# nv-tlabs/ChronoEdit

Measured on AMD Instinct MI355X. Metric: denoising-steps/sec, higher is better.
Workload: dtype bf16

## Files before the change

chronoedit_amd/csrc/ce_attn.hip:

```cpp
#include <cstdlib>

#include "ce_common.h"

namespace {

constexpr int HD = 128;
constexpr int QW = 32;
constexpr int KVB = 64;
constexpr int K_TILE_BYTES = KVB * HD * 2;
constexpr int VT_TILE_BYTES = HD * KVB * 2;
constexpr int BUF_BYTES = K_TILE_BYTES + VT_TILE_BYTES;
constexpr int OST_ROW = HD * 2 + 16;
constexpr int smem_bytes(int nwave, bool two_seg) {
  const int stage = nwave * QW * OST_ROW;
  return two_seg ? 2 * BUF_BYTES + stage : (stage > 2 * BUF_BYTES ? stage : 2 * BUF_BYTES);
}
constexpr float NEG_BIG = -1.0e30f;

__device__ __forceinline__ int vt_swz(int dv) {
  return ((((dv >> 2) & 7) << 1) | (((dv >> 1) ^ (dv >> 5)) & 1)) ^ (((dv >> 6) & 1) << 1);
}

struct KVSeg {
  const bf16* k;
  const bf16* v;
  int len;
  int ldk;
  int ldv;
};
struct BlkRows {
  int rows;
  int stride;
  uint32_t magic;
  int vt_cols;
  unsigned char* q8;
  unsigned char* s8;
  int ld8;
};

template <bool TWO_SEG, int NWAVE>
__global__ __launch_bounds__(NWAVE * 64, NWAVE == 8 ? 2 : 2) void attn_fwd_kernel(const bf16* __restrict__ Q, bf16* __restrict__ O, KVSeg seg0,
                                                       KVSeg seg1, int Nq, int H, int ldq, int ldo, int nqb,
                                                       float scale_log2e) {
  extern __shared__ __attribute__((aligned(16))) unsigned char smem[];
  {
    const size_t bz = blockIdx.y;
    Q += bz * Nq * ldq;
    O += bz * Nq * ldo;
    seg0.k += bz * seg0.len * seg0.ldk;
    seg0.v += bz * seg0.len * seg0.ldv;
    if (TWO_SEG) {
      seg1.k += bz * seg1.len * seg1.ldk;
      seg1.v += bz * seg1.len * seg1.ldv;
    }
  }
  const int tid = threadIdx.x, lane = tid & 63, wave = tid >> 6;
  const int l31 = lane & 31, hh = lane >> 5;

  int head, qb;
  if ((H & 7) == 0) {
    const int xcd = blockIdx.x & 7, local = blockIdx.x >> 3;
    head = xcd + 8 * (local / nqb);
    qb = local % nqb;
  } else {
    head = blockIdx.x / nqb;
    qb = blockIdx.x % nqb;
  }
  constexpr int QB = QW * NWAVE;
  constexpr int NT = NWAVE * 64;
  const int q0 = qb * QB + wave * QW;
  const int hoff = head * HD;

  bf16x8 qf[8];
  {
    const bf16* qrow = Q + (size_t)min(q0 + l31, Nq - 1) * ldq + hoff + 8 * hh;
#pragma unroll
    for (int ks = 0; ks < 8; ++ks) qf[ks] = *reinterpret_cast<const bf16x8*>(qrow + 16 * ks);
  }

  constexpr int KREP = 1024 / NT, KROWS = NT / 16;
  const int k_ck = tid & 15, k_row0 = tid >> 4;
  constexpr int VREP = 512 / NT, VKQ = NT / 32;
  const int v_dvq = tid & 31, v_kvq = tid >> 5;

  unsigned char* ost = smem + (TWO_SEG ? 2 * BUF_BYTES : 0) + (size_t)(wave * QW + l31) * OST_ROW;

#pragma unroll
  for (int sidx = 0; sidx < (TWO_SEG ? 2 : 1); ++sidx) {
    const KVSeg sg = sidx == 0 ? seg0 : seg1;
    const int ntiles = (sg.len + KVB - 1) / KVB;

    f32x16 oacc[4];
// ... 135 lines not shown
    const float l_tot = l_run + __shfl_xor(l_run, 32, 64);
    const float inv = 1.0f / l_tot;
#pragma unroll
    for (int m = 0; m < 4; ++m)
#pragma unroll
      for (int a = 0; a < 4; ++a) {
        uint32_t w0 = pack_bf16(oacc[m][4 * a + 0] * inv, oacc[m][4 * a + 1] * inv);
        uint32_t w1 = pack_bf16(oacc[m][4 * a + 2] * inv, oacc[m][4 * a + 3] * inv);
        u32x2* slot = reinterpret_cast<u32x2*>(ost + (32 * m + 8 * a + 4 * hh) * 2);
        if (TWO_SEG && sidx == 1) {
          const u32x2 pv = *slot;
          w0 = pack_bf16(bf16lo(pv[0]) + bf16lo(w0), bf16hi(pv[0]) + bf16hi(w0));
          w1 = pack_bf16(bf16lo(pv[1]) + bf16lo(w1), bf16hi(pv[1]) + bf16hi(w1));
        }
        u32x2 val = {w0, w1};
        *slot = val;
      }
  }

  __syncthreads();
#pragma unroll
  for (int i = 0; i < 8; ++i) {
    const int c = lane + 64 * i;
    const int rl = c >> 4, cc = c & 15;
    const int q = q0 + rl;
    if (q < Nq) {
      const u32x4 v = *reinterpret_cast<const u32x4*>(smem + (TWO_SEG ? 2 * BUF_BYTES : 0) + (size_t)(wave * QW + rl) * OST_ROW + cc * 16);
      *reinterpret_cast<u32x4*>(O + (size_t)q * ldo + hoff + cc * 8) = v;
    }
  }
}


#define CE_EPOCH_BARRIER()                          \
  asm volatile("s_waitcnt lgkmcnt(0)" ::: "memory"); \
  __builtin_amdgcn_s_barrier()
constexpr int PK_ROW = HD * 2 + 16;
constexpr int PV_ROW = KVB * 2 + 16;
constexpr int PK_TILE = KVB * PK_ROW;
constexpr int PV_TILE = HD * PV_ROW;
typedef __attribute__((ext_vector_type(4))) unsigned pp_u4;
typedef __attribute__((ext_vector_type(2))) unsigned pp_u2;

constexpr int K_GRP = 1088;
typedef __attribute__((address_space(3))) void lds_void;
#ifdef CE_DIAGNOSTICS
__device__ unsigned long long g_sp_exact_hits = 0ull;
#endif
constexpr float SP_SPEC_THR = 1024.0f;
constexpr int SP_V0 = 2 * PK_TILE;
constexpr int SP_TILE_BYTES = 2 * PK_TILE + 3 * PV_TILE;
constexpr int sp_smem_bytes(bool two_seg) { return two_seg ? SP_TILE_BYTES + 8 * QW * OST_ROW : SP_TILE_BYTES; }

template <bool TWO_SEG, bool VT = false, bool QOUT = false>
__global__ __launch_bounds__(512, 2) void attn_fwd_sp_kernel(const bf16* __restrict__ Q_, bf16* __restrict__ O_, KVSeg seg0_,
                                                              KVSeg seg1_, int Nq, int H, int ldq, int ldo, int nqb,
                                                              float scale_log2e, int batch, BlkRows blk) {
  extern __shared__ __attribute__((aligned(16))) unsigned char smem[];
  constexpr int NWAVE = 8, QB = QW * NWAVE;
  const int tid = threadIdx.x, lane = tid & 63;
  const int wave = __builtin_amdgcn_readfirstlane(tid >> 6);
  const int l31 = lane & 31, hh = lane >> 5;
  for (int item = blockIdx.x; item < nqb * H * batch; item += gridDim.x) {
  const bf16* Q = Q_;
  bf16* O = O_;
  KVSeg seg0 = seg0_, seg1 = seg1_;

  int head, qb, bz;
  {
    const int nqb_full = Nq / QB;
    if ((H & 7) == 0) {
      const int xcd = item & 7, local = item >> 3, hx_n = H >> 3;
      const int full = batch * hx_n * nqb_full;
      if (local < full) {
        bz = local / (hx_n * nqb_full);
        const int r = local % (hx_n * nqb_full);
        head = xcd + 8 * (r / nqb_full);
        qb = r % nqb_full;
      } else {
        const int l2 = local - full;
        bz = l2 / hx_n;
        head = xcd + 8 * (l2 % hx_n);
        qb = nqb_full;
      }
    } else {
      bz = item / (nqb * H);
      const int r = item % (nqb * H);
      head = r / nqb;
      qb = r % nqb;
    }
  }
  {
    if (VT && blk.rows > 0) {
      Q += (size_t)bz * blk.rows * ldq;
      O += (size_t)bz * blk.rows * ldo;
      seg0.k += (size_t)bz * blk.rows * seg0.ldk;
      seg0.v += (size_t)bz * blk.vt_cols;
    } else {
      Q += (size_t)bz * Nq * ldq;
      O += (size_t)bz * Nq * ldo;
      seg0.k += (size_t)bz * seg0.len * seg0.ldk;
      seg0.v += VT ? (size_t)bz * (TWO_SEG ? blk.vt_cols : seg0.len) : (size_t)bz * seg0.len * seg0.ldv;
    }
    if (TWO_SEG) {
      seg1.k += (size_t)bz * seg1.len * seg1.ldk;
      seg1.v += VT ? (size_t)bz * blk.stride : (size_t)bz * seg1.len * seg1.ldv;
    }
  }
  const int q0 = qb * QB + wave * QW;
  const int hoff = head * HD;
  const bool active = q0 < Nq;
  const int q0row = (VT && blk.rows > 0) ? (q0 / blk.rows) * blk.stride + q0 % blk.rows : q0;

  bf16x8 qf[8];
  {
    const bf16* qrow = Q + (size_t)(q0 + l31 < Nq ? q0row + l31 : 0) * ldq + hoff + 8 * hh;
#pragma unroll
    for (int ks = 0; ks < 8; ++ks) qf[ks] = *reinterpret_cast<const bf16x8*>(qrow + 16 * ks);
  }
  auto scale_q = [&]() __attribute__((always_inline)) {
#pragma unroll
  for (int ks = 0; ks < 8; ++ks) {
    const u32x4 w = __builtin_bit_cast(u32x4, qf[ks]);
    u32x4 o;
#pragma unroll
    for (int i = 0; i < 4; ++i) o[i] = pack_bf16(bf16lo(w[i]) * scale_log2e, bf16hi(w[i]) * scale_log2e);
    qf[ks] = __builtin_bit_cast(bf16x8, o);
  }
#pragma unroll
  for (int ks = 0; ks < 8; ++ks) asm volatile("" : "+v"(qf[ks]));

  };
  const int v_dvq = (tid & 1) | (((tid >> 4) & 15) << 1), v_kvq = ((tid >> 1) & 7) | (((tid >> 8) & 1) << 3);
  const int v_chunk = (v_kvq & ~3) | ((v_kvq & 1) << 1) | ((v_kvq >> 1) & 1);
  unsigned char* ost = smem + (TWO_SEG ? SP_TILE_BYTES : 0) + (size_t)(wave * QW + l31) * OST_ROW;
  const int k_w = l31 & 3;
  const unsigned char* k_rd = smem + (l31 >> 2) * K_GRP + k_w * 256 + ((hh ^ (k_w & 1)) << 4);
  const int k_eo[2] = {(k_w >> 1) << 5, ((k_w >> 1) ^ 1) << 5};
  const unsigned char* v_rd = smem + SP_V0 + l31 * PV_ROW + hh * 16;
  int vt_off[4];
#pragma unroll
  for (int s4 = 0; s4 < 4; ++s4) {
    const int x = (l31 >> 1) & 7;
    vt_off[s4] = l31 * 128 + ((2 * (s4 ^ (x >> 1)) + (hh ^ (x & 1))) << 4);
  }
  unsigned char* v_wr = smem + SP_V0 + (4 * v_dvq) * PV_ROW + v_chunk * 8;

#pragma unroll
  for (int sidx = 0; sidx < (TWO_SEG ? 2 : 1); ++sidx) {
    const KVSeg sg = sidx == 0 ? seg0 : seg1;
    const int ntiles = (sg.len + KVB - 1) / KVB;
    const int k_rows_span = (VT && blk.rows > 0) ? ((sg.len - 1) / blk.rows) * blk.stride + blk.rows : sg.len;
    const auto k_rsrc = __builtin_amdgcn_make_buffer_rsrc((void*)(sg.k + hoff), 0, (k_rows_span - 1) * sg.ldk * 2 + HD * 2, 0x00020000);
    const auto v_rsrc = VT ? __builtin_amdgcn_make_buffer_rsrc((void*)(sg.v + (size_t)hoff * sg.ldv), 0, ((HD - 1) * sg.ldv + ntiles * KVB) * 2, 0x00020000)
                           : __builtin_amdgcn_make_buffer_rsrc((void*)(sg.v + hoff), 0, (sg.len - 1) * sg.ldv * 2 + HD * 2, 0x00020000);
    int v_voff[4];
#pragma unroll
    for (int i = 0; i < 4; ++i) v_voff[i] = (4 * v_kvq + i) * sg.ldv * 2 + v_dvq * 8;
    const int k_tile_bytes = KVB * sg.ldk * 2, v_tile_bytes = KVB * sg.ldv * 2;

    f32x16 oacc[4];
#pragma unroll
    for (int m = 0; m < 4; ++m)
#pragma unroll
      for (int r = 0; r < 16; ++r) oacc[m][r] = 0.f;
    float l_run = 0.f, alpha_prev = 1.0f, mc = 0.f;
    f32x16 cinit;
#pragma unroll
    for (int r = 0; r < 16; ++r) cinit[r] = 0.f;
    u32x4 ppk[4];
#pragma unroll
    for (int s4 = 0; s4 < 4; ++s4) ppk[s4] = u32x4{0u, 0u, 0u, 0u};

// ... 822 lines not shown
    if (col < col_end) *reinterpret_cast<pp_u4*>(VT + (size_t)(head * HD + d) * ldvt + col) = v;
  }
}

}

#ifdef CE_DIAGNOSTICS
extern "C" int ce_diag_mx_exact_hits(unsigned long long* out, int reset);
CE_API int ce_diag_attention_exact_route_hits(unsigned long long* hits, int reset) {
  if (!hits) return CE_ERR_ARG;
  unsigned long long v = 0ull, z = 0ull;
  if (hipDeviceSynchronize() != hipSuccess) return CE_ERR_ARG;
  if (hipMemcpyFromSymbol(&v, HIP_SYMBOL(g_sp_exact_hits), sizeof(v)) != hipSuccess) return CE_ERR_ARG;
  if (reset && hipMemcpyToSymbol(HIP_SYMBOL(g_sp_exact_hits), &z, sizeof(z)) != hipSuccess) return CE_ERR_ARG;
  hits[0] = v;
  return ce_diag_mx_exact_hits(hits + 1, reset);
}
#endif
CE_KNOB g_attn_nwave = 0;
#ifdef CE_DIAGNOSTICS
CE_API int ce_set_attention_waves(int nwave) {
  const int old = g_attn_nwave;
  if (nwave == 0 || nwave == 4 || nwave == 8 || nwave == 16 || nwave == 64 || nwave == 128 || nwave == 129) g_attn_nwave = nwave;
  return old;
}
#endif

CE_API int ce_attention_batched_bf16(const void* Q, const void* K1, const void* V1, int len1, int ldk1, int ldv1,
                                         const void* K2, const void* V2, int len2, int ldk2, int ldv2, void* O, int Nq, int H,
                                         int head_dim, int ldq, int ldo, float softmax_scale, int batch, hipStream_t stream) {
  if (!Q || !K1 || !V1 || !O) return CE_ERR_ARG;
  if (head_dim != HD || Nq <= 0 || H <= 0 || len1 <= 0 || batch <= 0 || batch > 65535) return CE_ERR_SHAPE;
  if ((ldq & 7) || (ldo & 7) || (ldk1 & 7) || (ldv1 & 3)) return CE_ERR_ALIGN;
  const bool two = (K2 != nullptr && V2 != nullptr && len2 > 0);
  if (two && ((ldk2 & 7) || (ldv2 & 3))) return CE_ERR_ALIGN;
  KVSeg s0{(const bf16*)K1, (const bf16*)V1, len1, ldk1, ldv1};
  KVSeg s1{(const bf16*)K2, (const bf16*)V2, two ? len2 : 0, ldk2, ldv2};
  const float sl2 = softmax_scale * 1.4426950408889634f;
  const bool sp = g_attn_nwave == 64 || g_attn_nwave == 0 || g_attn_nwave >= 128;
  const int nwave = sp ? 8 : g_attn_nwave;
  const int nqb = (Nq + nwave * QW - 1) / (nwave * QW);
  dim3 grid(nqb * H, batch), block(nwave * 64);
  if (sp) {
#define CE_ATTN_SP(TWO)                                                                                              \
  do {                                                                                                               \
    static bool done_[CE_MAX_DEVICES] = {};                                                                          \
    bool& done = done_[ce_device_slot()];                                                                            \
    if (!done) {                                                                                                     \
      (void)hipFuncSetAttribute((const void*)attn_fwd_sp_kernel<TWO>, hipFuncAttributeMaxDynamicSharedMemorySize,    \
                                sp_smem_bytes(TWO));                                                                 \
      done = true;                                                                                                   \
    }                                                                                                                \
    hipLaunchKernelGGL((attn_fwd_sp_kernel<TWO>), dim3(nqb * H * batch), block, sp_smem_bytes(TWO), stream, (const bf16*)Q, \
                       (bf16*)O, s0, s1, Nq, H, ldq, ldo, nqb, sl2, batch, BlkRows{0, 0, 0u, 0});                    \
  } while (0)
    if (two) CE_ATTN_SP(true); else CE_ATTN_SP(false);
#undef CE_ATTN_SP
    return (int)hipGetLastError();
  }
#define CE_ATTN_LAUNCH(TWO, NW)                                                                                     \
  do {                                                                                                              \
    static bool done_[CE_MAX_DEVICES] = {};                                                                         \
    bool& done = done_[ce_device_slot()];                                                                           \
    if (!done) {                                                                                                    \
      (void)hipFuncSetAttribute((const void*)attn_fwd_kernel<TWO, NW>, hipFuncAttributeMaxDynamicSharedMemorySize,  \
                                smem_bytes(NW, TWO));                                                               \
      done = true;                                                                                                  \
    }                                                                                                               \
    hipLaunchKernelGGL((attn_fwd_kernel<TWO, NW>), grid, block, smem_bytes(NW, TWO), stream, (const bf16*)Q, (bf16*)O, \
                       s0, s1, Nq, H, ldq, ldo, nqb, sl2);                                                          \
  } while (0)
  if (two) {
    if (nwave == 8) CE_ATTN_LAUNCH(true, 8); else CE_ATTN_LAUNCH(true, 4);
  } else {
    if (nwave == 8) CE_ATTN_LAUNCH(false, 8); else CE_ATTN_LAUNCH(false, 4);
  }
#undef CE_ATTN_LAUNCH
  return (int)hipGetLastError();
}

CE_API int ce_attention_bf16(const void* Q, const void* K1, const void* V1, int len1, int ldk1, int ldv1, const void* K2,
                                 const void* V2, int len2, int ldk2, int ldv2, void* O, int Nq, int H, int head_dim, int ldq,
                                 int ldo, float softmax_scale, hipStream_t stream) {
  return ce_attention_batched_bf16(Q, K1, V1, len1, ldk1, ldv1, K2, V2, len2, ldk2, ldv2, O, Nq, H, head_dim, ldq, ldo,
                                   softmax_scale, 1, stream);
}

CE_API int ce_v_transpose_bf16(const void* v, int ldv, void* vt, int ldvt, int n_keys, int H, hipStream_t stream) {
  if (!v || !vt) return CE_ERR_ARG;
  if (n_keys <= 0 || H <= 0 || ldvt < n_keys) return CE_ERR_SHAPE;
  if ((ldv & 3) || (ldvt & 7)) return CE_ERR_ALIGN;
  hipLaunchKernelGGL(v_transpose_kernel, dim3((ldvt + KVB - 1) / KVB, H), dim3(256), 0, stream, (const bf16*)v, ldv, (bf16*)vt, ldvt, n_keys, 0, 0, 0);
  return (int)hipGetLastError();
}

CE_API int ce_v_transpose_blocked_bf16(const void* v, int ldv, void* vt, int ldvt, int n_keys, int H, int batch, int blk_rows, int blk_stride,
                                           int vt_sample_cols, hipStream_t stream) {
  if (!v || !vt) return CE_ERR_ARG;
  if (n_keys <= 0 || H <= 0 || batch <= 0 || blk_rows <= 0 || (blk_rows & 63) || blk_stride < batch * blk_rows || (vt_sample_cols & 63) ||
      vt_sample_cols < (n_keys + KVB - 1) / KVB * KVB || ldvt < batch * vt_sample_cols)
    return CE_ERR_SHAPE;
  if ((ldv & 3) || (ldvt & 7)) return CE_ERR_ALIGN;
  hipLaunchKernelGGL(v_transpose_kernel, dim3(vt_sample_cols / KVB, H, batch), dim3(256), 0, stream, (const bf16*)v, ldv, (bf16*)vt, ldvt, n_keys,
                     blk_rows, blk_stride, vt_sample_cols);
  return (int)hipGetLastError();
}

#ifdef CE_DIAGNOSTICS
extern "C" int ce_attn16_launch(const void* Q, const void* K, const void* Vt, int len, int ldk, int ldvt, void* O, int Nq, int H, int ldq, int ldo,
                                float sl2, int batch, int cus, hipStream_t stream);
#endif

static int attention_vt_launch(const void* Q, const void* K, const void* Vt, int len, int ldk, int ldvt, void* O, int Nq, int H, int head_dim,
                               int ldq, int ldo, float softmax_scale, int batch, int blk_rows, int blk_stride, int vt_sample_cols,
                               hipStream_t stream) {
  if (!Q || !K || !Vt || !O) return CE_ERR_ARG;
  if (head_dim != HD || Nq <= 0 || H <= 0 || len <= 0 || batch <= 0 || batch > 65535) return CE_ERR_SHAPE;
  const int ntiles_cols = (len + KVB - 1) / KVB * KVB;
  if (blk_rows == 0) {
    vt_sample_cols = len;
    if (ldvt < (batch - 1) * len + ntiles_cols) return CE_ERR_SHAPE;
  } else {
    if ((blk_rows & 63) || blk_stride < batch * blk_rows || (Nq % blk_rows) || vt_sample_cols < ntiles_cols ||
        ldvt < (batch - 1) * vt_sample_cols + ntiles_cols)
      return CE_ERR_SHAPE;
  }
  if ((ldq & 7) || (ldo & 7) || (ldk & 7) || (ldvt & 7) || (batch > 1 && (vt_sample_cols & 1))) return CE_ERR_ALIGN;
  KVSeg s0{(const bf16*)K, (const bf16*)Vt, len, ldk, ldvt};
  KVSeg s1{nullptr, nullptr, 0, 0, 0};
  BlkRows blk{blk_rows, blk_stride, 0u, vt_sample_cols};
  if (blk_rows > 0) {
    const uint32_t tps = (uint32_t)(blk_rows >> 6);
    blk.magic = tps == 1 ? 0u : (uint32_t)(((1ull << 32) + tps - 1) / tps);
  }
  const float sl2 = softmax_scale * 1.4426950408889634f;
  const int nqb = (Nq + 8 * QW - 1) / (8 * QW);
  static bool done_[CE_MAX_DEVICES] = {};
  bool& done = done_[ce_device_slot()];
  if (!done) {
    (void)hipFuncSetAttribute((const void*)attn_fwd_sp_kernel<false, true>, hipFuncAttributeMaxDynamicSharedMemorySize, sp_smem_bytes(false));
    done = true;
  }
  const int cus = ce_device_cus();
  const int items = nqb * H * batch;
#ifdef CE_DIAGNOSTICS
  if (g_attn_nwave == 16 && blk_rows == 0) {
    const int rc = ce_attn16_launch(Q, K, Vt, len, ldk, ldvt, O, Nq, H, ldq, ldo, sl2, batch, cus, stream);
    if (rc != CE_ERR_ALIGN) return rc;
  }
#endif
  if (g_attn_nwave == 128 || g_attn_nwave == 129) {
    static bool done4_[CE_MAX_DEVICES] = {};
    bool& done4 = done4_[ce_device_slot()];
    if (!done4) {
      (void)hipFuncSetAttribute((const void*)attn_fwd_w4_kernel, hipFuncAttributeMaxDynamicSharedMemorySize, W4_SMEM);
      done4 = true;
    }
    const int grid4 = (g_attn_nwave == 129 && items > cus) ? (cus & ~7) : items;
    hipLaunchKernelGGL(attn_fwd_w4_kernel, dim3(grid4), dim3(256), W4_SMEM, stream, (const bf16*)Q, (bf16*)O, s0, Nq, H, ldq, ldo, nqb,
                       sl2, batch, blk);
    return (int)hipGetLastError();
  }
  const int grid_vt = items <= 2 * cus ? items : ((2 * cus) & ~7);
  hipLaunchKernelGGL((attn_fwd_sp_kernel<false, true>), dim3(grid_vt), dim3(512), sp_smem_bytes(false), stream, (const bf16*)Q, (bf16*)O,
                     s0, s1, Nq, H, ldq, ldo, nqb, sl2, batch, blk);
  return (int)hipGetLastError();
}

CE_API int ce_attention_vt_bf16(const void* Q, const void* K, const void* Vt, int len, int ldk, int ldvt, void* O, int Nq, int H,
                                    int head_dim, int ldq, int ldo, float softmax_scale, int batch, hipStream_t stream) {
  return attention_vt_launch(Q, K, Vt, len, ldk, ldvt, O, Nq, H, head_dim, ldq, ldo, softmax_scale, batch, 0, 0, 0, stream);
}

CE_API int ce_attention_vt_blocked_bf16(const void* Q, const void* K, const void* Vt, int len, int ldk, int ldvt, void* O, int Nq, int H,
                                            int head_dim, int ldq, int ldo, float softmax_scale, int batch, int blk_rows, int blk_stride,
                                            int vt_sample_cols, hipStream_t stream) {
  if (blk_rows <= 0) return CE_ERR_SHAPE;
  return attention_vt_launch(Q, K, Vt, len, ldk, ldvt, O, Nq, H, head_dim, ldq, ldo, softmax_scale, batch, blk_rows, blk_stride, vt_sample_cols,
                             stream);
}


static int attention_2seg_vt_launch(const void* Q, const void* K1, const void* V1t, int len1, int ldk1, int ldv1t, int vt_cols1,
                                    const void* K2, const void* V2t, int len2, int ldk2, int ldv2t, int vt_cols2, void* O, int Nq,
                                    int H, int head_dim, int ldq, int ldo, float softmax_scale, int batch, void* O8, void* S8, int ldo8,
                                    hipStream_t stream) {
  if (!Q || !K1 || !V1t || !K2 || !V2t || (!O && !O8)) return CE_ERR_ARG;
  if (head_dim != HD || Nq <= 0 || H <= 0 || len1 <= 0 || len2 <= 0 || batch <= 0 || batch > 65535) return CE_ERR_SHAPE;
  const int c1 = (len1 + KVB - 1) / KVB * KVB, c2 = (len2 + KVB - 1) / KVB * KVB;
  if (vt_cols1 < len1 || vt_cols2 < len2 || ldv1t < (batch - 1) * vt_cols1 + c1 || ldv2t < (batch - 1) * vt_cols2 + c2) return CE_ERR_SHAPE;
  if ((ldq & 7) || (ldo & 7) || (ldk1 & 7) || (ldk2 & 7) || (ldv1t & 7) || (ldv2t & 7) || (vt_cols1 & 1) || (vt_cols2 & 1)) return CE_ERR_ALIGN;
  KVSeg s0{(const bf16*)K1, (const bf16*)V1t, len1, ldk1, ldv1t};
  KVSeg s1{(const bf16*)K2, (const bf16*)V2t, len2, ldk2, ldv2t};
  const float sl2 = softmax_scale * 1.4426950408889634f;
  const int nqb = (Nq + 8 * QW - 1) / (8 * QW);
  static bool done_[CE_MAX_DEVICES] = {};
  bool& done = done_[ce_device_slot()];
  if (!done) {
    (void)hipFuncSetAttribute((const void*)attn_fwd_sp_kernel<true, true>, hipFuncAttributeMaxDynamicSharedMemorySize, sp_smem_bytes(true));
    (void)hipFuncSetAttribute((const void*)attn_fwd_sp_kernel<true, true, true>, hipFuncAttributeMaxDynamicSharedMemorySize, sp_smem_bytes(true));
    done = true;
  }
  const BlkRows blk{0, vt_cols2, 0u, vt_cols1, (unsigned char*)O8, (unsigned char*)S8, ldo8};
  const int cus = ce_device_cus();
  const int items = nqb * H * batch;
  const int grid = items <= 2 * cus ? items : ((2 * cus) & ~7);
  if (O8)
    hipLaunchKernelGGL((attn_fwd_sp_kernel<true, true, true>), dim3(grid), dim3(512), sp_smem_bytes(true), stream, (const bf16*)Q,
                       (bf16*)O, s0, s1, Nq, H, ldq, ldo, nqb, sl2, batch, blk);
  else
    hipLaunchKernelGGL((attn_fwd_sp_kernel<true, true>), dim3(grid), dim3(512), sp_smem_bytes(true), stream, (const bf16*)Q, (bf16*)O,
                       s0, s1, Nq, H, ldq, ldo, nqb, sl2, batch, blk);
  return (int)hipGetLastError();
}

CE_API int ce_attention_2seg_vt_bf16(const void* Q, const void* K1, const void* V1t, int len1, int ldk1, int ldv1t, int vt_cols1,
                                         const void* K2, const void* V2t, int len2, int ldk2, int ldv2t, int vt_cols2, void* O, int Nq,
                                         int H, int head_dim, int ldq, int ldo, float softmax_scale, int batch, hipStream_t stream) {
  if (!O) return CE_ERR_ARG;
  return attention_2seg_vt_launch(Q, K1, V1t, len1, ldk1, ldv1t, vt_cols1, K2, V2t, len2, ldk2, ldv2t, vt_cols2, O, Nq, H, head_dim, ldq, ldo,
                                  softmax_scale, batch, nullptr, nullptr, 0, stream);
}

CE_API int ce_attention_2seg_vt_quant_bf16(const void* Q, const void* K1, const void* V1t, int len1, int ldk1, int ldv1t, int vt_cols1,
                                               const void* K2, const void* V2t, int len2, int ldk2, int ldv2t, int vt_cols2, void* o8,
                                               void* scale8, int Nq, int H, int head_dim, int ldq, int ldo8, float softmax_scale, int batch,
                                               hipStream_t stream) {
  if (!o8 || !scale8 || (ldo8 & 15) || ((H * head_dim) & 127)) return CE_ERR_ARG;
  return attention_2seg_vt_launch(Q, K1, V1t, len1, ldk1, ldv1t, vt_cols1, K2, V2t, len2, ldk2, ldv2t, vt_cols2, nullptr, Nq, H, head_dim, ldq,
                                  8, softmax_scale, batch, o8, scale8, ldo8, stream);
}
```

chronoedit_amd/csrc/ce_gemm.hip:

```cpp
#include <cmath>

#include "ce_common.h"

#define EPI_BIAS 0
#define EPI_BIAS_GELU 1
#define EPI_GATE_RES 2
#define EPI_BIAS_GELU_ERF 3
#define EPI_F32 4
#define EPI_BIAS_ROW 6
#define EPI_BIAS_T 7
#define EPI_MUL 5

namespace {

constexpr int BM = 128, BN = 128, BK = 64;
constexpr int TILE_BYTES = BM * BK * 2;
constexpr int LDC_BYTES = BN * 2 + 16;

__device__ __forceinline__ int swz_chunk(int row, int chunk) { return chunk ^ ((row >> 1) & 7); }

template <int EPI>
__global__ __launch_bounds__(256) void gemm_bf16_128(const bf16* __restrict__ A, const bf16* __restrict__ W,
                                                     bf16* __restrict__ C, const float* __restrict__ bias,
                                                     const float* __restrict__ gate, const bf16* __restrict__ res, int M,
                                                     int N, int K, int lda, int ldw, int ldc, int ldres, int gate_rows,
                                                     int tiles_m, int tiles_n, int batch0, long long sA0, long long sA1,
                                                     long long sW0, long long sW1, long long sC0, long long sC1,
                                                     int a_seg_tiles, long long a_seg_extra) {
  __shared__ __attribute__((aligned(16))) unsigned char smem[2 * 2 * TILE_BYTES];
  if (gridDim.y > 1) {
    const int z0 = blockIdx.y % batch0, z1 = blockIdx.y / batch0;
    A += z0 * sA0 + z1 * sA1;
    W += z0 * sW0 + z1 * sW1;
    const long long oc = z0 * sC0 + z1 * sC1;
    C = EPI == EPI_F32 ? reinterpret_cast<bf16*>(reinterpret_cast<float*>(C) + oc) : C + oc;
  }
  const int tid = threadIdx.x, lane = tid & 63, wave = tid >> 6;
  const int wm = wave >> 1, wn = wave & 1;

  const int nwg = tiles_m * tiles_n;
  const int wg = xcd_remap(blockIdx.x, nwg);
  constexpr int GROUP = 8;
  const int group_sz = GROUP * tiles_n;
  const int gid = wg / group_sz;
  const int first_m = gid * GROUP;
  const int gm = min(tiles_m - first_m, GROUP);
  const int tm = first_m + (wg % group_sz) % gm;
  const int tn = (wg % group_sz) / gm;
  const int m0 = tm * BM, n0 = tn * BN;

  const int st_row = tid >> 3, st_ck = tid & 7;
  const bf16* a_src[4];
  const bf16* w_src[4];
  int st_off[4];
#pragma unroll
  for (int i = 0; i < 4; ++i) {
    const int r = st_row + 32 * i;
    a_src[i] = A + (size_t)min(m0 + r, M - 1) * lda + st_ck * 8;
    w_src[i] = W + (size_t)min(n0 + r, N - 1) * ldw + st_ck * 8;
    st_off[i] = r * (BK * 2) + (swz_chunk(r, st_ck) << 4);
  }

  f32x4 acc[4][4];
#pragma unroll
// ... 39 lines not shown
        af[i] = *reinterpret_cast<const bf16x8*>(sA + r * (BK * 2) + (swz_chunk(r, fg + 4 * ks) << 4));
      }
#pragma unroll
      for (int j = 0; j < 4; ++j) {
        const int r = wn * 64 + j * 16 + fr;
        wf[j] = *reinterpret_cast<const bf16x8*>(sW + r * (BK * 2) + (swz_chunk(r, fg + 4 * ks) << 4));
      }
#pragma unroll
      for (int i = 0; i < 4; ++i)
#pragma unroll
        for (int j = 0; j < 4; ++j) acc[i][j] = __builtin_amdgcn_mfma_f32_16x16x32_bf16(af[i], wf[j], acc[i][j], 0, 0, 0);
    }
    if (kt + 1 < KT) {
      unsigned char* dA = smem + (cur ^ 1) * 2 * TILE_BYTES;
#pragma unroll
      for (int i = 0; i < 4; ++i) {
        *reinterpret_cast<u32x4*>(dA + st_off[i]) = ra[i];
        *reinterpret_cast<u32x4*>(dA + TILE_BYTES + st_off[i]) = rw[i];
      }
    }
    __syncthreads();
  }

  if (EPI == EPI_F32) {
    float* Cf = reinterpret_cast<float*>(C);
#pragma unroll
    for (int j = 0; j < 4; ++j) {
      const int n = n0 + wn * 64 + j * 16 + fr;
#pragma unroll
      for (int i = 0; i < 4; ++i)
#pragma unroll
        for (int r = 0; r < 4; ++r) {
          const int m = m0 + wm * 64 + i * 16 + fg * 4 + r;
          if (m < M && n < N) Cf[(size_t)m * ldc + n] = acc[i][j][r];
        }
    }
    return;
  }
#pragma unroll
  for (int j = 0; j < 4; ++j) {
    const int cl = wn * 64 + j * 16 + fr;
    const int n = n0 + cl;
    const float bv = (EPI != EPI_BIAS_ROW && bias != nullptr && n < N) ? bias[n] : 0.f;
#pragma unroll
    for (int i = 0; i < 4; ++i)
#pragma unroll
      for (int r = 0; r < 4; ++r) {
        const int rl = wm * 64 + i * 16 + fg * 4 + r;
        const float br = EPI == EPI_BIAS_ROW ? bias[min(m0 + rl, M - 1)] : bv;
        *reinterpret_cast<bf16*>(smem + rl * LDC_BYTES + cl * 2) = (bf16)(acc[i][j][r] + br);
      }
  }
  __syncthreads();
#pragma unroll
  for (int t = 0; t < 8; ++t) {
    const int c = tid + 256 * t;
    const int rl = c >> 4, cc = c & 15;
    const int m = m0 + rl, n = n0 + cc * 8;
    if (m < M && n < N) {
      u32x4 v = *reinterpret_cast<const u32x4*>(smem + rl * LDC_BYTES + cc * 16);
      if (EPI == EPI_BIAS_GELU) {
#pragma unroll
        for (int q = 0; q < 4; ++q) v[q] = pack_bf16(gelu_tanh(bf16lo(v[q])), gelu_tanh(bf16hi(v[q])));
      } else if (EPI == EPI_BIAS_GELU_ERF) {
#pragma unroll
        for (int q = 0; q < 4; ++q) v[q] = pack_bf16(gelu_erf(bf16lo(v[q])), gelu_erf(bf16hi(v[q])));
      } else if (EPI == EPI_MUL) {
        const u32x4 rv = *reinterpret_cast<const u32x4*>(res + (size_t)m * ldres + n);
#pragma unroll
        for (int q = 0; q < 4; ++q) v[q] = pack_bf16(bf16lo(rv[q]) * bf16lo(v[q]), bf16hi(rv[q]) * bf16hi(v[q]));
      } else if (EPI == EPI_GATE_RES) {
        const u32x4 rv = *reinterpret_cast<const u32x4*>(res + (size_t)m * ldres + n);
        float g[8];
        if (gate != nullptr) {
          const float* gp = gate + (gate_rows > 0 ? (size_t)(m / gate_rows) * N : 0) + n;
          const f32x4 g0 = *reinterpret_cast<const f32x4*>(gp), g1 = *reinterpret_cast<const f32x4*>(gp + 4);
#pragma unroll
          for (int q = 0; q < 4; ++q) {
            g[q] = g0[q];
            g[4 + q] = g1[q];
          }
        } else {
#pragma unroll
          for (int q = 0; q < 8; ++q) g[q] = 1.0f;
        }
#pragma unroll
        for (int q = 0; q < 4; ++q)
          v[q] = pack_bf16(mul_then_add(bf16lo(v[q]), g[2 * q], bf16lo(rv[q])), mul_then_add(bf16hi(v[q]), g[2 * q + 1], bf16hi(rv[q])));
      }
      *reinterpret_cast<u32x4*>(C + (size_t)m * ldc + n) = v;
    }
  }
}

}

extern "C" int ce_gemm256_supported(int M, int N, int K, int lda, int ldw);
extern "C" int ce_gemm256_launch(const void* A, const void* W, void* C, const float* bias, int epilogue, const float* gate,
                                 const void* res, int M, int N, int K, int lda, int ldw, int ldc, int ldres, int gate_rows,
                                 int a_seg_k, long long a_seg_stride, int w_seg_k, long long w_seg_stride, float* ws, size_t ws_bytes,
                                 hipStream_t stream);

extern "C" void ce_gemm256_set_staggered(int on);
extern "C" int ce_gemm384_launch(const void* A, const void* W, void* C, const float* bias, int epilogue, const float* gate,
                                 const void* res, int M, int N, int K, int lda, int ldw, int ldc, int ldres, int gate_rows,
                                 int a_seg_k, long long a_seg_stride, int w_seg_k, long long w_seg_stride, float* ws, size_t ws_bytes,
// ... 29 lines not shown
    double t = (double)full * kt * c;
    if (tail > 0) {
      const int split = ce_split_k(tail, kt, cus, bm * 256 * (long long)sizeof(float), ws_bytes);
      if (split > 1) t += (double)kt / split * c + (double)tail * split * bm * 256.0 * 8.0 / 6.0e6;
      else t += (double)kt * c * pow((double)tail / cus, 0.3);
    }
    return t;
  };
  const double c384 = cost(384), c256 = cost(256);
  if (M % 288 == 0) {
    const long long nwg = (long long)(M / 288) * ((N + 255) / 256);
    const int tail = (int)(nwg % cus);
    if (tail == 0 || tail * 10 >= cus * 9) {
      const double c288 = cost(288);
      if (c288 < 0.97 * (c384 < c256 ? c384 : c256)) return 288;
    }
  }
  return c384 <= c256 ? 384 : 256;
}

CE_API int ce_gemm_bf16(const void* A, const void* W, void* C, const float* bias, int epilogue, const float* gate,
                        const void* res, int M, int N, int K, int lda, int ldw, int ldc, int ldres, int gate_rows,
                        int a_seg_k, long long a_seg_stride, int w_seg_k, long long w_seg_stride, void* ws, size_t ws_bytes,
                        hipStream_t stream) {
  if (!A || !W || !C) return CE_ERR_ARG;
  float* const slabs = static_cast<float*>(ws);
  const long long scratch_bytes = ws ? (long long)ws_bytes : 0;
  const int cus = ce_device_cus();
  if (epilogue == EPI_BIAS_T) {
    if (!bias || M <= 0 || N <= 0 || K <= 0 || (K % BK)) return CE_ERR_ARG;
    if ((lda & 7) || (ldw & 7) || (ldc & 7)) return CE_ERR_ALIGN;
    const bool plain = (a_seg_k <= 0 || a_seg_k >= K) && (w_seg_k <= 0 || w_seg_k >= K);
    if (plain && (M & 7) == 0 && (N & 7) == 0 && (long long)M * N >= 256ll * 256 * 128 && (long long)N * ldc * 2 < (1ll << 32) &&
        ce_gemm256_supported(M, N, K, lda, ldw) && (g_gemm_variant == -1 || g_gemm_variant == 6 || g_gemm_variant == 7)) {
      const int rows = g_gemm_variant == 6 ? 384 : g_gemm_variant == 7 ? 288 : ce_gemm_bf16_tile_rows(M, N, K, cus, scratch_bytes);
      if (rows == 384 || rows == 288) {
        const long long nwg = (long long)((M + rows - 1) / rows) * ((N + 255) / 256);
        const int tail = (int)(nwg % cus);
        if (g_gemm_variant != -1 || tail == 0 || tail * 10 >= cus * 9)
          return (rows == 384 ? ce_gemm384_launch : ce_gemm288_launch)(A, W, C, bias, EPI_BIAS_T, nullptr, nullptr, M, N, K, lda, ldw, ldc, 0, 0, 0, 0, 0, 0,
                                                                      slabs, ws_bytes, stream);
      }
    }
    if (!plain) return CE_ERR_SHAPE;
    return ce_gemm_bf16(W, A, C, bias, EPI_BIAS_ROW, nullptr, nullptr, N, M, K, ldw, lda, ldc, 0, 0, 0, 0, 0, 0, ws, ws_bytes, stream);
  }
  if (w_seg_k < 0 || (w_seg_k > 0 && w_seg_k < K && ((w_seg_k % BK) || (K % w_seg_k) || (w_seg_stride & 7)))) return CE_ERR_SHAPE;
  if (w_seg_k >= K) w_seg_k = 0;
  if (a_seg_k < 0 || (a_seg_k > 0 && a_seg_k < K && ((a_seg_k % BK) || (K % a_seg_k) || (a_seg_stride & 7)))) return CE_ERR_SHAPE;
  if (a_seg_k >= K) a_seg_k = 0;
  if (M <= 0 || N <= 0 || K <= 0 || (K % BK) || (N & 7)) return CE_ERR_SHAPE;
  if ((lda & 7) || (ldw & 7) || (ldc & 7)) return CE_ERR_ALIGN;
  if ((epilogue == EPI_GATE_RES || epilogue == EPI_MUL) && (!res || (ldres & 7))) return CE_ERR_ARG;
  if (epilogue < 0 || epilogue > 6 || (epilogue == EPI_BIAS_ROW && !bias)) return CE_ERR_ARG;
  if (epilogue != EPI_F32 && epilogue != EPI_MUL) {
    const bool big = (long long)M * N >= 256ll * 256 * 128;
    const bool want = g_gemm_variant >= 1 || (g_gemm_variant == -1 && big);
    if ((want || w_seg_k) && ce_gemm256_supported(M, N, K, lda, ldw)) {
      const int rows_auto = g_gemm_variant == -1 ? ce_gemm_bf16_tile_rows(M, N, K, cus, scratch_bytes) : 0;
      if (g_gemm_variant == 6 || rows_auto == 384)
        return ce_gemm384_launch(A, W, C, bias, epilogue, gate, res, M, N, K, lda, ldw, ldc, ldres, gate_rows, a_seg_k, a_seg_stride,
                                 w_seg_k, w_seg_stride, slabs, ws_bytes, stream);
      if (g_gemm_variant == 7 || rows_auto == 288)
        return ce_gemm288_launch(A, W, C, bias, epilogue, gate, res, M, N, K, lda, ldw, ldc, ldres, gate_rows, a_seg_k, a_seg_stride,
                                 w_seg_k, w_seg_stride, slabs, ws_bytes, stream);
      if (g_gemm_variant == 1 || g_gemm_variant == 2)
        return ce_gemm256_launch(A, W, C, bias, epilogue, gate, res, M, N, K, lda, ldw, ldc, ldres, gate_rows, a_seg_k, a_seg_stride,
                                 w_seg_k, w_seg_stride, slabs, ws_bytes, stream);
      return ce_gemm256w4_launch(A, W, C, bias, epilogue, gate, res, M, N, K, lda, ldw, ldc, ldres, gate_rows, a_seg_k, a_seg_stride,
                                 w_seg_k, w_seg_stride, g_gemm_variant == 3 ? 3 : g_gemm_variant == 5 ? 1 : 2, slabs, ws_bytes, stream);
    }
  }
  if (w_seg_k) return CE_ERR_SHAPE;
  const int a_seg_tiles = a_seg_k > 0 ? a_seg_k / BK : 0;
  const long long a_seg_extra = a_seg_k > 0 ? a_seg_stride - a_seg_k : 0;
  const int tiles_m = (M + BM - 1) / BM, tiles_n = (N + BN - 1) / BN;
  dim3 grid(tiles_m * tiles_n), block(256);
#define CE_LAUNCH(E)                                                                                              \
  hipLaunchKernelGGL(gemm_bf16_128<E>, grid, block, 0, stream, (const bf16*)A, (const bf16*)W, (bf16*)C, bias, gate, \
                     (const bf16*)res, M, N, K, lda, ldw, ldc, ldres, gate_rows, tiles_m, tiles_n, 1, 0ll, 0ll, 0ll, 0ll, 0ll, 0ll, \
                     a_seg_tiles, a_seg_extra)
  switch (epilogue) {
    case EPI_BIAS: CE_LAUNCH(EPI_BIAS); break;
    case EPI_BIAS_GELU: CE_LAUNCH(EPI_BIAS_GELU); break;
    case EPI_GATE_RES: CE_LAUNCH(EPI_GATE_RES); break;
    case EPI_BIAS_GELU_ERF: CE_LAUNCH(EPI_BIAS_GELU_ERF); break;
    case EPI_F32: CE_LAUNCH(EPI_F32); break;
    case EPI_MUL: CE_LAUNCH(EPI_MUL); break;
    case EPI_BIAS_ROW: CE_LAUNCH(EPI_BIAS_ROW); break;
    default: return CE_ERR_ARG;
  }
#undef CE_LAUNCH
  return (int)hipGetLastError();
}

CE_API int ce_gemm_batched_bf16(const void* A, const void* W, void* C, const float* bias, int epilogue, int M, int N, int K,
                                    int lda, int ldw, int ldc, int batch0, int batch1, long long sA0, long long sA1, long long sW0,
                                    long long sW1, long long sC0, long long sC1, hipStream_t stream) {
  if (!A || !W || !C) return CE_ERR_ARG;
  if (M <= 0 || N <= 0 || K <= 0 || (K % BK) || (N & 7) || batch0 <= 0 || batch1 <= 0 || (long long)batch0 * batch1 > 65535)
    return CE_ERR_SHAPE;
  if ((lda & 7) || (ldw & 7) || (ldc & 7) || (sA0 & 7) || (sA1 & 7) || (sW0 & 7) || (sW1 & 7) || (sC0 & 7) || (sC1 & 7))
    return CE_ERR_ALIGN;
  if (epilogue != EPI_BIAS && epilogue != EPI_F32) return CE_ERR_ARG;
  const int tiles_m = (M + BM - 1) / BM, tiles_n = (N + BN - 1) / BN;
  dim3 grid(tiles_m * tiles_n, batch0 * batch1), block(256);
#define CE_LAUNCH(E)                                                                                                 \
  hipLaunchKernelGGL(gemm_bf16_128<E>, grid, block, 0, stream, (const bf16*)A, (const bf16*)W, (bf16*)C, bias, nullptr, \
                     nullptr, M, N, K, lda, ldw, ldc, 0, 0, tiles_m, tiles_n, batch0, sA0, sA1, sW0, sW1, sC0, sC1, 0, 0ll)
  if (epilogue == EPI_BIAS) CE_LAUNCH(EPI_BIAS); else CE_LAUNCH(EPI_F32);
#undef CE_LAUNCH
  return (int)hipGetLastError();
}
```

chronoedit_amd/csrc/ce_gemm256w4.hip:

```cpp
#include "ce_common.h"
#include "ce_gemm_epi.h"

namespace {

constexpr int BM = 256, BN = 256, BK = 64;
constexpr int TILE = 256 * BK * 2;
constexpr int CROW = BN * 2 + 16;
constexpr int QROW = 128 * 2 + 16;

typedef __attribute__((address_space(3))) void lds_void;

#define W4_VM(N) asm volatile("s_waitcnt vmcnt(" #N ")" ::: "memory")
#define W4_LGKM0() asm volatile("s_waitcnt lgkmcnt(0)" ::: "memory")
#define W4_BAR() __builtin_amdgcn_s_barrier()
#define W4_PIN() __builtin_amdgcn_sched_barrier(0)

__device__ __forceinline__ void tile_origin_w4(int wg, int tiles_m, int tiles_n, int bn, int& m0, int& n0) {
  constexpr int GROUP = 4;
  const int group_sz = GROUP * tiles_n;
  const int gid = wg / group_sz;
  const int first_m = gid * GROUP;
  const int gm = min(tiles_m - first_m, GROUP);
  m0 = (first_m + (wg % group_sz) % gm) * BM;
  n0 = ((wg % group_sz) / gm) * bn;
// ... 191 lines not shown
            *reinterpret_cast<f32x4*>(slab + (((wave * 64 + f * 8 + (fr >> 1)) * 64) + lane_o) * 4) = o;
          }
      }
      return;
    }
    f32x4 bvv[2];
#pragma unroll
    for (int h = 0; h < 2; ++h)
      bvv[h] = (EPI != EPI_BIAS_ROW && bias != nullptr) ? *reinterpret_cast<const f32x4*>(bias + colc + 4 * h) : f32x4{0.f, 0.f, 0.f, 0.f};
    const auto c_rsrc = __builtin_amdgcn_make_buffer_rsrc((void*)C, 0, (uint32_t)(M - 1) * (uint32_t)(ldc * 2) + (uint32_t)N * 2u, 0x00020000);
    f32x4 gA[2], gB[2];
    int g_switch = 0x7fffffff;
    u32x4 rv[8][4];
    if (EPI == EPI_GATE_RES) {
      gA[0] = gA[1] = gB[0] = gB[1] = f32x4{1.f, 1.f, 1.f, 1.f};
      if (gate != nullptr) {
        const int s0 = gate_rows > 0 ? m0 / gate_rows : 0;
        const int s1 = gate_rows > 0 ? min(M - 1, m0 + BM - 1) / gate_rows : 0;
        const float* ga = gate + (size_t)s0 * N + colc;
        const float* gb = gate + (size_t)s1 * N + colc;
        gA[0] = *reinterpret_cast<const f32x4*>(ga);
        gA[1] = *reinterpret_cast<const f32x4*>(ga + 4);
        gB[0] = *reinterpret_cast<const f32x4*>(gb);
        gB[1] = *reinterpret_cast<const f32x4*>(gb + 4);
        if (s1 != s0) g_switch = s1 * gate_rows;
      }
#pragma unroll
      for (int f = 0; f < 8; ++f)
#pragma unroll
        for (int jj = 0; jj < 4; ++jj)
          rv[f][jj] = *reinterpret_cast<const u32x4*>(res + (size_t)min(row_base + f * 16 + jj, M - 1) * ldres + colc);
    }
#pragma unroll
    for (int f = 0; f < 8; ++f) {
      f32x4 av[8];
#pragma unroll
      for (int g = 0; g < 8; ++g) {
        asm volatile("" : "+a"(acc[f][g]));
        av[g] = acc[f][g];
      }
      f32x4 brow4 = {0.f, 0.f, 0.f, 0.f};
      if (EPI == EPI_BIAS_ROW) brow4 = *reinterpret_cast<const f32x4*>(bias + min(row_base + f * 16, M - 4));
#pragma unroll
      for (int jj = 0; jj < 4; ++jj) {
        const int m = row_base + f * 16 + jj;
        u32x4 y;
#pragma unroll
        for (int q = 0; q < 4; ++q) {
          const int h = q >> 1, e = 2 * (q & 1);
          const float b0 = EPI == EPI_BIAS_ROW ? brow4[jj] : bvv[h][e], b1 = EPI == EPI_BIAS_ROW ? brow4[jj] : bvv[h][e + 1];
          y[q] = pack_bf16(av[2 * q][jj] + b0, av[2 * q + 1][jj] + b1);
        }
        u32x4 o = y;
        if (EPI == EPI_BIAS_GELU) {
#pragma unroll
          for (int q = 0; q < 4; ++q) o[q] = pack_bf16(gelu_tanh(bf16lo(y[q])), gelu_tanh(bf16hi(y[q])));
        } else if (EPI == EPI_BIAS_GELU_ERF) {
#pragma unroll
          for (int q = 0; q < 4; ++q) o[q] = pack_bf16(gelu_erf(bf16lo(y[q])), gelu_erf(bf16hi(y[q])));
        } else if (EPI == EPI_GATE_RES) {
          const u32x4 r = rv[f][jj];
          const bool second = m >= g_switch;
          const f32x4 g0 = second ? gB[0] : gA[0], g1 = second ? gB[1] : gA[1];
#pragma unroll
          for (int q = 0; q < 4; ++q) {
            const float ga = q < 2 ? g0[2 * q] : g1[2 * q - 4], gb = q < 2 ? g0[2 * q + 1] : g1[2 * q - 3];
            o[q] = pack_bf16(mul_then_add(bf16lo(y[q]), ga, bf16lo(r[q])), mul_then_add(bf16hi(y[q]), gb, bf16hi(r[q])));
          }
        }
        const uint32_t coff = (m < M && col_ok) ? (uint32_t)m * (uint32_t)(ldc * 2) + (uint32_t)col0 * 2u : 0xffffffffu;
        __builtin_amdgcn_raw_buffer_store_b128(o, c_rsrc, coff, 0, 0);
      }
    }
    return;
  }
  W4_BAR();

  if (partial) {
    float* slab = ws + (size_t)(blockIdx.x - t_full) * (BM * BN);
#pragma unroll
    for (int f = 0; f < 8; ++f)
#pragma unroll
      for (int g = 0; g < NG; ++g)
        *reinterpret_cast<f32x4*>(slab + (((wave * 64 + f * 8 + g) * 64) + lane) * 4) = acc[f][g];
    return;
  }
  constexpr int CPR = BN / 8;
  constexpr bool CPOW2 = (CPR & (CPR - 1)) == 0;
  constexpr int RPT = 256 / CPR;
  constexpr int CH = CPOW2 ? 64 * CPR / 256 : (64 + RPT - 1) / RPT;
  const int my_cc = CPOW2 ? (tid & (CPR - 1)) : tid % CPR;
  auto chunk_row = [&](int tt, bool& ok) __attribute__((always_inline)) -> int {
    if (CPOW2) {
      ok = true;
      return (tid + 256 * tt) / CPR;
    }
    const int rl = tid / CPR + RPT * tt;
    ok = tid < RPT * CPR && rl < 64;
    return min(rl, 63);
  };

  f32x4 bcol[NG];
#pragma unroll
  for (int g = 0; g < NG; ++g) {
    const int n = n0 + wn * (BN / 2) + g * 16 + fg * 4;
    bcol[g] = (EPI != EPI_BIAS_ROW && bias != nullptr) ? *reinterpret_cast<const f32x4*>(bias + min(n, N - 4)) : f32x4{0.f, 0.f, 0.f, 0.f};
// ... 63 lines not shown
          const float ga = q < 2 ? g0[2 * q] : g1[2 * q - 4], gb = q < 2 ? g0[2 * q + 1] : g1[2 * q - 3];
          o[q] = pack_bf16(mul_then_add(bf16lo(y[q]), ga, bf16lo(r[q])), mul_then_add(bf16hi(y[q]), gb, bf16hi(r[q])));
        }
        const uint32_t coff = (m < M && my_n < N) ? (uint32_t)m * (uint32_t)(ldc * 2) + (uint32_t)my_n * 2u : 0xffffffffu;
        __builtin_amdgcn_raw_buffer_store_b128(o, c_rsrc, coff, 0, 0);
      }
    } else if (EPI != EPI_GATE_RES) {
      epi_chunks<EPI, CH>(smem, CROW,
                         [&](int tt, int& rl, int& cc, int& mr) {
                           bool ok;
                           rl = chunk_row(tt, ok);
                           cc = my_cc;
                           mr = ok ? (rl >> 5) * 128 + p * 32 + (rl & 31) : (1 << 28);
                         },
                         m0, n0, C, gate, res, M, N, ldc, ldres, gate_rows);
    }
  }
}

template <int EPI>
__global__ __launch_bounds__(256) void gemm256w4_reduce(bf16* __restrict__ C, const float* __restrict__ bias, const float* __restrict__ gate,
                                                        const bf16* __restrict__ res, int M, int N, int ldc, int ldres, int gate_rows,
                                                        int tiles_m, int tiles_n, int t_full, int split, const float* __restrict__ ws) {
  extern __shared__ __attribute__((aligned(16))) unsigned char smem[];
  const int tid = threadIdx.x, lane = tid & 63, w = tid >> 6;
  const int fr = lane & 15, fg = lane >> 4;
  const int tile = blockIdx.x >> 2, q = blockIdx.x & 3;
  int m0, n0;
  tile_origin_w4(t_full + tile, tiles_m, tiles_n, BN, m0, n0);
  m0 += (q >> 1) * 128;
  n0 += (q & 1) * 128;
  const float* slab = ws + (size_t)tile * split * (BM * BN);
#pragma unroll
  for (int ff = 0; ff < 2; ++ff) {
    const int f = 2 * w + ff;
    const int rl = f * 16 + fr;
    float brow = 0.f;
    if (EPI == EPI_BIAS_ROW) brow = bias[min(m0 + rl, M - 1)];
#pragma unroll
    for (int g = 0; g < 8; ++g) {
      const int cl = g * 16 + fg * 4;
      f32x4 bv = (EPI != EPI_BIAS_ROW && bias != nullptr) ? *reinterpret_cast<const f32x4*>(bias + min(n0 + cl, N - 4)) : f32x4{0.f, 0.f, 0.f, 0.f};
      if (EPI == EPI_BIAS_ROW) bv[0] = bv[1] = bv[2] = bv[3] = brow;
      const int e = (((q * 64 + f * 8 + g) * 64) + lane) * 4;
      f32x4 v = *reinterpret_cast<const f32x4*>(slab + e);
      for (int sidx = 1; sidx < split; ++sidx) v += *reinterpret_cast<const f32x4*>(slab + (size_t)sidx * (BM * BN) + e);
      const u32x2 pk = {pack_bf16(v[0] + bv[0], v[1] + bv[1]), pack_bf16(v[2] + bv[2], v[3] + bv[3])};
      *reinterpret_cast<u32x2*>(smem + rl * QROW + cl * 2) = pk;
    }
  }
  __syncthreads();
  epi_chunks<EPI, 8>(smem, QROW, [&](int tt, int& rl, int& cc, int& mr) { const int c = tid + 256 * tt; rl = mr = c >> 4; cc = c & 15; }, m0, n0,
                     C, gate, res, M, N, ldc, ldres, gate_rows);
}

}

extern "C" int ce_gemm256_launch(const void* A, const void* W, void* C, const float* bias, int epilogue, const float* gate,
                                 const void* res, int M, int N, int K, int lda, int ldw, int ldc, int ldres, int gate_rows,
                                 int a_seg_k, long long a_seg_stride, int w_seg_k, long long w_seg_stride, float* ws, size_t ws_bytes,
                                 hipStream_t stream);

static int w4_launch(const void* A, const void* W, void* C, const float* bias, int epilogue, const float* gate, const void* res, int M, int N,
                     int K, int lda, int ldw, int ldc, int ldres, int gate_rows, int a_seg_k, long long a_seg_stride, int w_seg_k,
                     long long w_seg_stride, int a_seg2_k, long long a_seg2_stride, int nsa, int ng, float* ws, size_t ws_bytes,
                     hipStream_t stream) {
  const bool seg2 = a_seg2_k > 0;
  if ((ng != 8 && ng != 4 && ng != 3) || (ng != 8 && !seg2)) return CE_ERR_ARG;
  if (seg2 && (a_seg_k <= 0 || a_seg2_k % a_seg_k || (epilogue != EPI_BIAS && epilogue != EPI_GATE_RES) || nsa != 2 ||
               (epilogue == EPI_GATE_RES && gate != nullptr)))
    return CE_ERR_ARG;
  if (epilogue == EPI_GATE_RES && ((gate != nullptr && gate_rows > 0 && gate_rows < BM) || (long long)M * ldc * 2 >= (1ll << 32)))
    return ce_gemm256_launch(A, W, C, bias, epilogue, gate, res, M, N, K, lda, ldw, ldc, ldres, gate_rows, a_seg_k, a_seg_stride, w_seg_k,
                             w_seg_stride, ws, ws_bytes, stream);
  if (ng == 8 && ((long long)M * ldc * 2 >= (1ll << 32) || (epilogue == EPI_BIAS_ROW && (M & 3))))
    return ce_gemm256_launch(A, W, C, bias, epilogue, gate, res, M, N, K, lda, ldw, ldc, ldres, gate_rows, a_seg_k, a_seg_stride, w_seg_k,
                             w_seg_stride, ws, ws_bytes, stream);
  const int bn = 32 * ng;
  const int tiles_m = (M + BM - 1) / BM, tiles_n = (N + bn - 1) / bn;
  const int nwg = tiles_m * tiles_n, kt = K / BK;
  uint32_t a_seg_magic = 0, a_seg_extra = 0, w_seg_magic = 0, w_seg_extra = 0;
  auto seg = [&](int seg_k, long long seg_stride, uint32_t& magic, uint32_t& extra_out) -> int {
    if (seg_k <= 0 || seg_k >= K) return CE_OK;
    magic = ce_seg_magic(seg_k, BK, kt);
    const long long extra = (seg_stride - seg_k) * 2;
    if (!magic || extra < 0 || extra * ((K + seg_k - 1) / seg_k) + (long long)K * 2 >= (1ll << 31)) return CE_ERR_SHAPE;
    extra_out = (uint32_t)extra;
    return CE_OK;
  };
  if (int rc = seg(a_seg_k, a_seg_stride, a_seg_magic, a_seg_extra)) return rc;
  if (int rc = seg(w_seg_k, w_seg_stride, w_seg_magic, w_seg_extra)) return rc;
  uint32_t a_seg2_magic = 0, a_seg2_extra = 0;
  if (seg2 && a_seg2_k < K) {
    a_seg2_magic = ce_seg_magic(a_seg2_k, BK, kt);
    if (!a_seg2_magic) return CE_ERR_SHAPE;
    const long long extra = (a_seg2_stride - (long long)(a_seg2_k / a_seg_k) * a_seg_stride) * 2;
    const long long reach = ((long long)(K - 1) / a_seg2_k) * a_seg2_stride * 2 + (long long)(a_seg2_k / a_seg_k) * a_seg_stride * 2 + (long long)a_seg_k * 2;
    if (extra < 0 || reach >= (1ll << 31)) return CE_ERR_SHAPE;
    a_seg2_extra = (uint32_t)extra;
  }
  const int cus = ce_device_cus();
  int tail = nwg % cus;
  const int split = seg2 ? 1 : ce_split_k(tail, kt, cus, BM * BN * sizeof(float), ws ? (long long)ws_bytes : 0);
  if (split == 1) tail = 0;
  const int t_full2 = nwg - tail;
  dim3 grid(t_full2 + tail * split), block(256);
  const int lds3 = 5 * TILE, lds2 = 4 * TILE;
  if (seg2) {
    const int lds2n = 2 * TILE + 2 * (128 * BK * 2);
    const int lds2m = 2 * TILE + 2 * (96 * BK * 2);
    static bool seg2_done_[CE_MAX_DEVICES] = {};
    bool& seg2_done = seg2_done_[ce_device_slot()];
    if (!seg2_done) {
      if (hipFuncSetAttribute((const void*)gemm_bf16_w4<EPI_BIAS, 2, false, true>, hipFuncAttributeMaxDynamicSharedMemorySize, lds2) != hipSuccess ||
          hipFuncSetAttribute((const void*)gemm_bf16_w4<EPI_GATE_RES, 2, false, true>, hipFuncAttributeMaxDynamicSharedMemorySize, lds2) != hipSuccess ||
          hipFuncSetAttribute((const void*)gemm_bf16_w4<EPI_BIAS, 2, false, true, 4>, hipFuncAttributeMaxDynamicSharedMemorySize, lds2n) != hipSuccess ||
          hipFuncSetAttribute((const void*)gemm_bf16_w4<EPI_GATE_RES, 2, false, true, 4>, hipFuncAttributeMaxDynamicSharedMemorySize, lds2n) != hipSuccess ||
          hipFuncSetAttribute((const void*)gemm_bf16_w4<EPI_BIAS, 2, false, true, 3>, hipFuncAttributeMaxDynamicSharedMemorySize, lds2m) != hipSuccess ||
          hipFuncSetAttribute((const void*)gemm_bf16_w4<EPI_GATE_RES, 2, false, true, 3>, hipFuncAttributeMaxDynamicSharedMemorySize, lds2m) != hipSuccess)
        return CE_ERR_ARG;
      seg2_done = true;
    }
#define CE_LAUNCH_SEG2(E, NGV, LDS)                                                                                                     \
  hipLaunchKernelGGL((gemm_bf16_w4<E, 2, false, true, NGV>), grid, block, LDS, stream, (const bf16*)A, (const bf16*)W, (bf16*)C, bias, gate, \
                     (const bf16*)res, M, N, K, lda, ldw, ldc, ldres, gate_rows, tiles_m, tiles_n, t_full2, split, ws, a_seg_magic,   \
                     a_seg_extra, w_seg_magic, w_seg_extra, a_seg2_magic, a_seg2_extra)
    if (epilogue == EPI_BIAS) {
      if (ng == 8) CE_LAUNCH_SEG2(EPI_BIAS, 8, lds2); else if (ng == 4) CE_LAUNCH_SEG2(EPI_BIAS, 4, lds2n); else CE_LAUNCH_SEG2(EPI_BIAS, 3, lds2m);
    } else {
      if (ng == 8) CE_LAUNCH_SEG2(EPI_GATE_RES, 8, lds2); else if (ng == 4) CE_LAUNCH_SEG2(EPI_GATE_RES, 4, lds2n); else CE_LAUNCH_SEG2(EPI_GATE_RES, 3, lds2m);
// ... 8 lines not shown
    if (!attr_done[E]) {                                                                                                   \
      if (hipFuncSetAttribute((const void*)gemm_bf16_w4<E, 3, false>, hipFuncAttributeMaxDynamicSharedMemorySize, lds3) != hipSuccess) return CE_ERR_ARG; \
      if (hipFuncSetAttribute((const void*)gemm_bf16_w4<E, 3, true>, hipFuncAttributeMaxDynamicSharedMemorySize, lds3) != hipSuccess) return CE_ERR_ARG; \
      if (hipFuncSetAttribute((const void*)gemm_bf16_w4<E, 2, false>, hipFuncAttributeMaxDynamicSharedMemorySize, lds2) != hipSuccess) return CE_ERR_ARG; \
      (void)hipFuncSetAttribute((const void*)gemm256w4_reduce<E>, hipFuncAttributeMaxDynamicSharedMemorySize, 128 * QROW); \
      attr_done[E] = true;                                                                                                 \
    }                                                                                                                      \
    if (nsa == 1)                                                                                                          \
      hipLaunchKernelGGL((gemm_bf16_w4<E, 3, true>), grid, block, lds3, stream, (const bf16*)A, (const bf16*)W, (bf16*)C, bias, gate, \
                         (const bf16*)res, M, N, K, lda, ldw, ldc, ldres, gate_rows, tiles_m, tiles_n, t_full2, split, ws, \
                         a_seg_magic, a_seg_extra, w_seg_magic, w_seg_extra, 0u, 0u);                                      \
    else if (nsa == 3)                                                                                                     \
      hipLaunchKernelGGL((gemm_bf16_w4<E, 3, false>), grid, block, lds3, stream, (const bf16*)A, (const bf16*)W, (bf16*)C, bias, gate, \
                         (const bf16*)res, M, N, K, lda, ldw, ldc, ldres, gate_rows, tiles_m, tiles_n, t_full2, split, ws, \
                         a_seg_magic, a_seg_extra, w_seg_magic, w_seg_extra, 0u, 0u);                                      \
    else                                                                                                                   \
      hipLaunchKernelGGL((gemm_bf16_w4<E, 2, false>), grid, block, lds2, stream, (const bf16*)A, (const bf16*)W, (bf16*)C, bias, gate, \
                         (const bf16*)res, M, N, K, lda, ldw, ldc, ldres, gate_rows, tiles_m, tiles_n, t_full2, split, ws, \
                         a_seg_magic, a_seg_extra, w_seg_magic, w_seg_extra, 0u, 0u);                                      \
    if (tail)                                                                                                              \
      hipLaunchKernelGGL((gemm256w4_reduce<E>), dim3(4 * tail), block, 128 * QROW, stream, (bf16*)C, bias, gate,           \
                         (const bf16*)res, M, N, ldc, ldres, gate_rows, tiles_m, tiles_n, t_full2, split, ws);           \
  } while (0)
  switch (epilogue) {
    case EPI_BIAS: CE_LAUNCH(EPI_BIAS); break;
    case EPI_BIAS_GELU: CE_LAUNCH(EPI_BIAS_GELU); break;
    case EPI_GATE_RES: CE_LAUNCH(EPI_GATE_RES); break;
    case EPI_BIAS_GELU_ERF: CE_LAUNCH(EPI_BIAS_GELU_ERF); break;
    case EPI_BIAS_ROW: CE_LAUNCH(EPI_BIAS_ROW); break;
    default: return CE_ERR_ARG;
  }
#undef CE_LAUNCH
  return (int)hipGetLastError();
}

extern "C" int ce_gemm256w4_launch(const void* A, const void* W, void* C, const float* bias, int epilogue, const float* gate,
                                   const void* res, int M, int N, int K, int lda, int ldw, int ldc, int ldres, int gate_rows,
                                   int a_seg_k, long long a_seg_stride, int w_seg_k, long long w_seg_stride, int nsa, float* ws,
                                   size_t ws_bytes, hipStream_t stream) {
  return w4_launch(A, W, C, bias, epilogue, gate, res, M, N, K, lda, ldw, ldc, ldres, gate_rows, a_seg_k, a_seg_stride, w_seg_k, w_seg_stride,
                   0, 0, nsa, 8, ws, ws_bytes, stream);
}

extern "C" int ce_gemm256w4_seg2_launch(const void* A, const void* W, void* C, const float* bias, int epilogue, const void* res, int M, int N,
                                        int K, int lda, int ldw, int ldc, int ldres, int a_seg_k, long long a_seg_stride, int a_seg2_k,
                                        long long a_seg2_stride, int n_tile, hipStream_t stream) {
  return w4_launch(A, W, C, bias, epilogue, nullptr, res, M, N, K, lda, ldw, ldc, ldres, 0, a_seg_k, a_seg_stride, 0, 0, a_seg2_k, a_seg2_stride,
                   2, n_tile / 32, nullptr, 0, stream);
}

extern "C" int ce_gemm256w4_reduce_launch(int epilogue, void* C, const float* bias, const float* gate, const void* res, int M, int N, int ldc,
                                          int ldres, int gate_rows, int tiles_m, int tiles_n, int t_full, int split, const float* ws, int tail,
                                          hipStream_t stream) {
  static bool done_[CE_MAX_DEVICES][8] = {};
  bool* done = done_[ce_device_slot()];
#define CE_RED(E)                                                                                                            \
  do {                                                                                                                       \
    if (!done[E]) {                                                                                                          \
      (void)hipFuncSetAttribute((const void*)gemm256w4_reduce<E>, hipFuncAttributeMaxDynamicSharedMemorySize, 128 * QROW);    \
      done[E] = true;                                                                                                        \
    }                                                                                                                        \
    hipLaunchKernelGGL((gemm256w4_reduce<E>), dim3(4 * tail), dim3(256), 128 * QROW, stream, (bf16*)C, bias, gate, (const bf16*)res, M, N, \
                       ldc, ldres, gate_rows, tiles_m, tiles_n, t_full, split, ws);                                          \
  } while (0)
  switch (epilogue) {
    case EPI_BIAS: CE_RED(EPI_BIAS); break;
    case EPI_BIAS_GELU: CE_RED(EPI_BIAS_GELU); break;
    case EPI_GATE_RES: CE_RED(EPI_GATE_RES); break;
    default: return CE_ERR_ARG;
  }
#undef CE_RED
  return (int)hipGetLastError();
}
```

chronoedit_amd/csrc/ce_gemm384.hip:

```cpp
#include "ce_common.h"
#include "ce_gemm_epi.h"

namespace {

constexpr int BN = 256, BK = 64;
constexpr int W_TILE = BN * BK * 2;
template <int NF> struct T384 {
  static constexpr int BM = 32 * NF;
  static constexpr int A_TILE = BM * BK * 2;
  static constexpr int STAGE = A_TILE + W_TILE;
  static constexpr int NG = 2 * NF;
  static constexpr int NP = NF + 8;
};
constexpr int CROW = BN * 2 + 16;
constexpr int QROW = 128 * 2 + 16;

typedef __attribute__((address_space(3))) void lds_void;

#define X_BAR() __builtin_amdgcn_s_barrier()
#define X_PIN() __builtin_amdgcn_sched_barrier(0)

template <int BM>
__device__ __forceinline__ void tile_origin_384(int wg, int tiles_m, int tiles_n, int& m0, int& n0) {
  constexpr int GROUP = 4;
// ... 258 lines not shown
        const uint32_t toff = (m < M && col_ok) ? (uint32_t)(col0 + g) * (uint32_t)(ldc * 2) + (uint32_t)m * 2u : 0xffffffffu;
        __builtin_amdgcn_raw_buffer_store_b64(y, t_rsrc, toff, 0, 0);
      }
    }
    return;
  }
  const auto c_rsrc = __builtin_amdgcn_make_buffer_rsrc((void*)C, 0, (uint32_t)(M - 1) * (uint32_t)(ldc * 2) + (uint32_t)N * 2u, 0x00020000);
  f32x4 gA[2], gB[2];
  int g_switch = 0x7fffffff;
  constexpr int RA = 2;
  u32x4 rv[RA + 1][4];
  auto res_load = [&](int f, u32x4* dst) __attribute__((always_inline)) {
#pragma unroll
    for (int jj = 0; jj < 4; ++jj) dst[jj] = *reinterpret_cast<const u32x4*>(res + (size_t)min(row_base + f * 16 + jj, M - 1) * ldres + colc);
  };
  if (EPI == EPI_GATE_RES) {
    gA[0] = gA[1] = gB[0] = gB[1] = f32x4{1.f, 1.f, 1.f, 1.f};
    if (gate != nullptr) {
      const int s0 = gate_rows > 0 ? m0 / gate_rows : 0;
      const int s1 = gate_rows > 0 ? min(M - 1, m0 + BM - 1) / gate_rows : 0;
      const float* ga = gate + (size_t)s0 * N + colc;
      const float* gb = gate + (size_t)s1 * N + colc;
      gA[0] = *reinterpret_cast<const f32x4*>(ga);
      gA[1] = *reinterpret_cast<const f32x4*>(ga + 4);
      gB[0] = *reinterpret_cast<const f32x4*>(gb);
      gB[1] = *reinterpret_cast<const f32x4*>(gb + 4);
      if (s1 != s0) g_switch = s1 * gate_rows;
    }
#pragma unroll
    for (int f = 0; f < RA; ++f) res_load(f, rv[f % (RA + 1)]);
  }
#pragma unroll
  for (int f = 0; f < NF; ++f) {
    if (EPI == EPI_GATE_RES && f + RA < NF) res_load(f + RA, rv[(f + RA) % (RA + 1)]);
    f32x4 av[8];
#pragma unroll
    for (int g = 0; g < 8; ++g) {
      if (f < 8) asm volatile("" : "+a"(acc[f][g])); else asm volatile("" : "+v"(acc[f][g]));
      av[g] = acc[f][g];
    }
    f32x4 brow4 = {0.f, 0.f, 0.f, 0.f};
    if (EPI == EPI_BIAS_ROW) brow4 = *reinterpret_cast<const f32x4*>(bias + min(row_base + f * 16, M - 4));
#pragma unroll
    for (int jj = 0; jj < 4; ++jj) {
      const int m = row_base + f * 16 + jj;
      u32x4 y;
#pragma unroll
      for (int q = 0; q < 4; ++q) {
        const int h = q >> 1, e = 2 * (q & 1);
        const float b0 = EPI == EPI_BIAS_ROW ? brow4[jj] : bvv[h][e], b1 = EPI == EPI_BIAS_ROW ? brow4[jj] : bvv[h][e + 1];
        y[q] = pack_bf16(av[2 * q][jj] + b0, av[2 * q + 1][jj] + b1);
      }
      u32x4 o = y;
      if (EPI == EPI_BIAS_GELU) {
#pragma unroll
        for (int q = 0; q < 4; ++q) o[q] = pack_bf16(gelu_tanh(bf16lo(y[q])), gelu_tanh(bf16hi(y[q])));
      } else if (EPI == EPI_BIAS_GELU_ERF) {
#pragma unroll
        for (int q = 0; q < 4; ++q) o[q] = pack_bf16(gelu_erf(bf16lo(y[q])), gelu_erf(bf16hi(y[q])));
      } else if (EPI == EPI_GATE_RES) {
        const u32x4 r = rv[f % (RA + 1)][jj];
        const bool second = m >= g_switch;
        const f32x4 g0 = second ? gB[0] : gA[0], g1 = second ? gB[1] : gA[1];
#pragma unroll
        for (int q = 0; q < 4; ++q) {
          const float ga = q < 2 ? g0[2 * q] : g1[2 * q - 4], gb = q < 2 ? g0[2 * q + 1] : g1[2 * q - 3];
          o[q] = pack_bf16(mul_then_add(bf16lo(y[q]), ga, bf16lo(r[q])), mul_then_add(bf16hi(y[q]), gb, bf16hi(r[q])));
        }
      }
      const uint32_t coff = (m < M && col_ok) ? (uint32_t)m * (uint32_t)(ldc * 2) + (uint32_t)col0 * 2u : 0xffffffffu;
      __builtin_amdgcn_raw_buffer_store_b128(o, c_rsrc, coff, 0, 0);
    }
  }
}

template <int EPI, int NF = 12>
__global__ __launch_bounds__(256) void gemm384_reduce(bf16* __restrict__ C, const float* __restrict__ bias, const float* __restrict__ gate,
                                                      const bf16* __restrict__ res, int M, int N, int ldc, int ldres, int gate_rows,
                                                      int tiles_m, int tiles_n, int t_full, int split, const float* __restrict__ ws) {
  extern __shared__ __attribute__((aligned(16))) unsigned char smem[];
  const int tid = threadIdx.x, lane = tid & 63, w = tid >> 6;
  const int fr = lane & 15, fg = lane >> 4;
  const int tile = blockIdx.x >> 2, q = blockIdx.x & 3;
  constexpr int BM = T384<NF>::BM;
  int m0, n0;
  tile_origin_384<BM>(t_full + tile, tiles_m, tiles_n, m0, n0);
  m0 += (q >> 1) * (16 * NF);
  n0 += (q & 1) * 128;
  const float* slab = ws + (size_t)tile * split * (BM * BN);
#pragma unroll
  for (int ff = 0; ff < 3; ++ff) {
    const int f = 3 * w + ff;
    if (f >= NF) break;
    const int rl = f * 16 + fr;
    float brow = 0.f;
    if (EPI == EPI_BIAS_ROW) brow = bias[min(m0 + rl, M - 1)];
#pragma unroll
    for (int g = 0; g < 8; ++g) {
      const int cl = g * 16 + fg * 4;
      f32x4 bv = (EPI != EPI_BIAS_ROW && bias != nullptr) ? *reinterpret_cast<const f32x4*>(bias + min(n0 + cl, N - 4)) : f32x4{0.f, 0.f, 0.f, 0.f};
      if (EPI == EPI_BIAS_ROW) bv[0] = bv[1] = bv[2] = bv[3] = brow;
      const int e = (((q * (8 * NF) + f * 8 + g) * 64) + lane) * 4;
      f32x4 v = *reinterpret_cast<const f32x4*>(slab + e);
      for (int sidx = 1; sidx < split; ++sidx) v += *reinterpret_cast<const f32x4*>(slab + (size_t)sidx * (BM * BN) + e);
      const u32x2 pk = {pack_bf16(v[0] + bv[0], v[1] + bv[1]), pack_bf16(v[2] + bv[2], v[3] + bv[3])};
      *reinterpret_cast<u32x2*>(smem + rl * QROW + cl * 2) = pk;
    }
  }
  __syncthreads();
  epi_chunks<EPI, NF>(smem, QROW, [&](int tt, int& rl, int& cc, int& mr) { const int c = tid + 256 * tt; rl = mr = c >> 4; cc = c & 15; }, m0, n0,
                      C, gate, res, M, N, ldc, ldres, gate_rows);
}

}

extern "C" int ce_gemm256_launch(const void* A, const void* W, void* C, const float* bias, int epilogue, const float* gate,
                                 const void* res, int M, int N, int K, int lda, int ldw, int ldc, int ldres, int gate_rows,
                                 int a_seg_k, long long a_seg_stride, int w_seg_k, long long w_seg_stride, float* ws, size_t ws_bytes,
                                 hipStream_t stream);

template <int NF>
static int gemm384_launch_impl(const void* A, const void* W, void* C, const float* bias, int epilogue, const float* gate, const void* res, int M, int N,
                               int K, int lda, int ldw, int ldc, int ldres, int gate_rows, int a_seg_k, long long a_seg_stride, int w_seg_k,
                               long long w_seg_stride, float* ws, size_t ws_bytes, hipStream_t stream) {
  constexpr int BM = T384<NF>::BM, STAGE = T384<NF>::STAGE;
  if (epilogue == EPI_BIAS_T) {
    if ((M & 7) || (long long)N * ldc * 2 >= (1ll << 32) || !bias) return CE_ERR_SHAPE;
  } else
  if ((epilogue == EPI_GATE_RES && gate != nullptr && gate_rows > 0 && gate_rows < BM) || (long long)M * ldc * 2 >= (1ll << 32) ||
      (epilogue == EPI_BIAS_ROW && (M & 3)))
    return ce_gemm256_launch(A, W, C, bias, epilogue, gate, res, M, N, K, lda, ldw, ldc, ldres, gate_rows, a_seg_k, a_seg_stride, w_seg_k,
                             w_seg_stride, ws, ws_bytes, stream);
  const int tiles_m = (M + BM - 1) / BM, tiles_n = (N + BN - 1) / BN;
  const int nwg = tiles_m * tiles_n, kt = K / BK;
  uint32_t a_seg_magic = 0, a_seg_extra = 0, w_seg_magic = 0, w_seg_extra = 0;
  auto seg = [&](int seg_k, long long seg_stride, uint32_t& magic, uint32_t& extra_out) -> int {
    if (seg_k <= 0 || seg_k >= K) return CE_OK;
    magic = ce_seg_magic(seg_k, BK, kt);
    const long long extra = (seg_stride - seg_k) * 2;
    if (!magic || extra < 0 || extra * (K / seg_k) + (long long)K * 2 >= (1ll << 31)) return CE_ERR_SHAPE;
    extra_out = (uint32_t)extra;
    return CE_OK;
  };
  if (int rc = seg(a_seg_k, a_seg_stride, a_seg_magic, a_seg_extra)) return rc;
  if (int rc = seg(w_seg_k, w_seg_stride, w_seg_magic, w_seg_extra)) return rc;
  const int cus = ce_device_cus();
  int tail = nwg % cus;
  const int split = epilogue == EPI_BIAS_T ? 1 : ce_split_k(tail, kt, cus, BM * BN * sizeof(float), ws ? (long long)ws_bytes : 0);
  if (split == 1) tail = 0;
  const int t_full2 = nwg - tail;
  dim3 grid(t_full2 + tail * split), block(256);
  const int lds = 2 * STAGE;
  static bool attr_done_[CE_MAX_DEVICES][8] = {};
  bool* attr_done = attr_done_[ce_device_slot()];
#define CE_LAUNCH(E)                                                                                                       \
  do {                                                                                                                     \
    if (!attr_done[E]) {                                                                                                   \
      if (hipFuncSetAttribute((const void*)gemm_bf16_384<E, NF>, hipFuncAttributeMaxDynamicSharedMemorySize, lds) != hipSuccess) return CE_ERR_ARG; \
      (void)hipFuncSetAttribute((const void*)gemm384_reduce<E, NF>, hipFuncAttributeMaxDynamicSharedMemorySize, 16 * NF * QROW); \
      attr_done[E] = true;                                                                                                 \
    }                                                                                                                      \
    hipLaunchKernelGGL((gemm_bf16_384<E, NF>), grid, block, lds, stream, (const bf16*)A, (const bf16*)W, (bf16*)C, bias, gate, \
                       (const bf16*)res, M, N, K, lda, ldw, ldc, ldres, gate_rows, tiles_m, tiles_n, t_full2, split, ws, \
                       a_seg_magic, a_seg_extra, w_seg_magic, w_seg_extra);                                                \
    if (tail)                                                                                                              \
      hipLaunchKernelGGL((gemm384_reduce<E, NF>), dim3(4 * tail), block, 16 * NF * QROW, stream, (bf16*)C, bias, gate,     \
                         (const bf16*)res, M, N, ldc, ldres, gate_rows, tiles_m, tiles_n, t_full2, split, ws);           \
  } while (0)
  switch (epilogue) {
    case EPI_BIAS: CE_LAUNCH(EPI_BIAS); break;
    case EPI_BIAS_GELU: CE_LAUNCH(EPI_BIAS_GELU); break;
    case EPI_GATE_RES: CE_LAUNCH(EPI_GATE_RES); break;
    case EPI_BIAS_GELU_ERF: CE_LAUNCH(EPI_BIAS_GELU_ERF); break;
    case EPI_BIAS_ROW: CE_LAUNCH(EPI_BIAS_ROW); break;
    case EPI_BIAS_T: {
      static bool t_done_[CE_MAX_DEVICES] = {};
      bool& t_done = t_done_[ce_device_slot()];
      if (!t_done) {
        if (hipFuncSetAttribute((const void*)gemm_bf16_384<EPI_BIAS_T, NF>, hipFuncAttributeMaxDynamicSharedMemorySize, lds) != hipSuccess) return CE_ERR_ARG;
        t_done = true;
      }
      hipLaunchKernelGGL((gemm_bf16_384<EPI_BIAS_T, NF>), grid, block, lds, stream, (const bf16*)A, (const bf16*)W, (bf16*)C, bias, gate, (const bf16*)res,
                         M, N, K, lda, ldw, ldc, ldres, gate_rows, tiles_m, tiles_n, t_full2, split, ws, a_seg_magic, a_seg_extra, w_seg_magic,
                         w_seg_extra);
      break;
// ... 23 lines not shown
```

chronoedit_amd/csrc/ce_gemm_epi.h:

```cpp
#pragma once
#include "ce_common.h"

#ifndef EPI_BIAS
#define EPI_BIAS 0
#define EPI_BIAS_GELU 1
#define EPI_GATE_RES 2
#define EPI_BIAS_GELU_ERF 3
#endif
#ifndef EPI_BIAS_ROW
#define EPI_BIAS_ROW 6
#endif
#ifndef EPI_BIAS_T
#define EPI_BIAS_T 7
#endif

namespace {

template <int EPI, int NCH, bool HAS_GATE, typename RowCol>
__device__ __forceinline__ void epi_chunks_impl(const unsigned char* smem, int row_bytes, RowCol rowcol, int m0, int n0,
                                                bf16* __restrict__ C, const float* __restrict__ gate, const bf16* __restrict__ res,
                                                int M, int N, int ldc, int ldres, int gate_rows) {
  u32x4 v[NCH], rv[NCH];
  f32x4 g0[NCH], g1[NCH];
  int ms[NCH], ns[NCH];
#pragma unroll
  for (int t = 0; t < NCH; ++t) {
    int rl, cc, mr;
    rowcol(t, rl, cc, mr);
    ms[t] = m0 + mr;
    ns[t] = n0 + cc * 8;
    v[t] = *reinterpret_cast<const u32x4*>(smem + rl * row_bytes + cc * 16);
    if (EPI == EPI_GATE_RES) {
      const int mc = min(ms[t], M - 1), nc = min(ns[t], N - 8);
      rv[t] = *reinterpret_cast<const u32x4*>(res + (size_t)mc * ldres + nc);
      if (HAS_GATE) {
        const float* gp = gate + (gate_rows > 0 ? (size_t)(mc / gate_rows) * N : 0) + nc;
        g0[t] = *reinterpret_cast<const f32x4*>(gp);
        g1[t] = *reinterpret_cast<const f32x4*>(gp + 4);
      }
    }
  }
#pragma unroll
  for (int t = 0; t < NCH; ++t) {
    u32x4 o = v[t];
    if (EPI == EPI_BIAS_GELU) {
#pragma unroll
      for (int q = 0; q < 4; ++q) o[q] = pack_bf16(gelu_tanh(bf16lo(o[q])), gelu_tanh(bf16hi(o[q])));
    } else if (EPI == EPI_BIAS_GELU_ERF) {
#pragma unroll
      for (int q = 0; q < 4; ++q) o[q] = pack_bf16(gelu_erf(bf16lo(o[q])), gelu_erf(bf16hi(o[q])));
    } else if (EPI == EPI_GATE_RES) {
#pragma unroll
      for (int q = 0; q < 4; ++q) {
        const float ga = !HAS_GATE ? 1.0f : q < 2 ? g0[t][2 * q] : g1[t][2 * q - 4];
        const float gb = !HAS_GATE ? 1.0f : q < 2 ? g0[t][2 * q + 1] : g1[t][2 * q - 3];
        o[q] = pack_bf16(mul_then_add(bf16lo(o[q]), ga, bf16lo(rv[t][q])), mul_then_add(bf16hi(o[q]), gb, bf16hi(rv[t][q])));
      }
    }
    if (ms[t] < M && ns[t] < N) *reinterpret_cast<u32x4*>(C + (size_t)ms[t] * ldc + ns[t]) = o;
  }
}
template <int EPI, int NCH, typename RowCol>
__device__ __forceinline__ void epi_chunks(const unsigned char* smem, int row_bytes, RowCol rowcol, int m0, int n0,
                                           bf16* __restrict__ C, const float* __restrict__ gate, const bf16* __restrict__ res,
                                           int M, int N, int ldc, int ldres, int gate_rows) {
  if (EPI == EPI_GATE_RES && gate != nullptr)
    epi_chunks_impl<EPI, NCH, true>(smem, row_bytes, rowcol, m0, n0, C, gate, res, M, N, ldc, ldres, gate_rows);
  else
    epi_chunks_impl<EPI, NCH, false>(smem, row_bytes, rowcol, m0, n0, C, gate, res, M, N, ldc, ldres, gate_rows);
// ... 4 lines not shown
```

chronoedit_amd/hiplib.py:

```python
from __future__ import annotations

import ctypes
import os
import re
import subprocess
from typing import Dict, List

PKG_DIR = os.path.dirname(os.path.abspath(__file__))
ROOT = os.path.dirname(PKG_DIR)
CSRC = os.path.join(PKG_DIR, "csrc")
LIB_DIR = os.path.join(PKG_DIR, "lib")
LIB_PATH = os.path.join(LIB_DIR, "libchronoedit_hip.so")
DIAG_LIB_PATH = os.path.join(LIB_DIR, "libchronoedit_hip_diag.so")
OBJ_DIR = os.path.join(LIB_DIR, "obj")
HEADER = os.path.join(ROOT, "include", "chronoedit_hip.h")
DIAG_HEADER = os.path.join(ROOT, "include", "chronoedit_hip_diag.h")

DIAG_SOURCES = ["ce_gemm.hip", "ce_gemm256.hip", "ce_attn.hip", "ce_attn_fp8.hip", "ce_gemm_fp8.hip", "ce_gemm_fp8w4.hip"]
DIAG_ONLY_SOURCES = ["ce_attn16.hip"]
SOURCES = ["ce_rowops.hip", "ce_gemm.hip", "ce_gemm256.hip", "ce_gemm256w4.hip", "ce_gemm384.hip", "ce_attn.hip", "ce_attn16.hip", "ce_attn_fp8.hip", "ce_sched.hip", "ce_conv.hip", "ce_enc.hip", "ce_gemm_fp8.hip", "ce_gemm_fp8w4.hip", "ce_comm.hip", "ce_lora.hip", "ce_tea.hip"]

_c = ctypes
_P, _I, _F = _c.c_void_p, _c.c_int, _c.c_float

SIGNATURES: Dict[str, List] = {
    "ce_ln_affine_bf16": [_P, _P, _P, _P, _I, _I, _I, _I, _F, _I, _I, _P],
    "ce_rmsnorm_rope_bf16": [_P, _P, _P, _P, _P, _I, _I, _I, _I, _F, _I, _P],
    "ce_gemm_bf16": [_P, _P, _P, _P, _I, _P, _P, _I, _I, _I, _I, _I, _I, _I, _I, _I, _c.c_longlong, _I, _c.c_longlong, _P, _c.c_size_t, _P],
    "ce_rmsnorm_rope_mxfp8": [_P, _P, _P, _P, _P, _I, _I, _I, _I, _I, _F, _I, _F, _P],
    "ce_v_mxfp8_transpose": [_P, _I, _P, _P, _I, _I, _I, _I, _P],
    "ce_attention_mxfp8": [_P, _P, _P, _P, _P, _P, _P, _I, _I, _I, _I, _I, _I, _I, _I, _I, _P],
    "ce_attention_mxfp8_quant": [_P, _P, _P, _P, _P, _P, _P, _P, _I, _I, _I, _I, _I, _I, _I, _I, _I, _P],
    "ce_attention_mxfp8_add": [_P, _P, _P, _P, _P, _P, _P, _I, _P, _I, _P, _P, _I, _I, _I, _I, _I, _I, _I, _I, _I, _P],
    "ce_rope_scatter_bf16": [_P, _I, _P, _I, _I, _I, _I, _I, _P, _I, _P, _I, _P, _P, _I, _F, _I, _P],
    "ce_patchify_rows_bf16": [_P, _P, _I, _I, _I, _I, _I, _I, _I, _P],
    "ce_comm_load": [ctypes.c_char_p],
    "ce_comm_unique_id": [_P],
    "ce_comm_init": [ctypes.POINTER(ctypes.c_void_p), _P, _I, _I],
    "ce_comm_destroy": [_P],
    "ce_comm_all_to_all": [_P, _P, _P, ctypes.c_size_t, _P],
    "ce_comm_all_gather": [_P, _P, _P, ctypes.c_size_t, _P],
    "ce_ln_affine_fp8": [_P, _P, _P, _P, _P, _I, _I, _I, _I, _F, _I, _I, _P],
    "ce_quant_rows_fp8": [_P, _P, _P, _I, _I, _I, _I, _P],
    "ce_gemm_fp8": [_P, _P, _P, _P, _P, _P, _I, _P, _P, _I, _I, _I, _I, _I, _I, _I, _I, _P, _c.c_size_t, _P],
    "ce_quant_rows_mxfp8": [_P, _P, _P, _I, _I, _I, _I, _P],
    "ce_quant_rows_mxfp8_w": [_P, _P, _P, _I, _I, _I, _I, _P],
    "ce_ln_affine_mxfp8": [_P, _P, _P, _P, _P, _I, _I, _I, _I, _F, _I, _I, _P],
    "ce_gemm_mxfp8": [_P, _P, _P, _P, _P, _P, _I, _P, _P, _I, _I, _I, _I, _I, _I, _I, _I, _P, _c.c_size_t, _P],
    "ce_gemm_mxfp8_gelu_quant": [_P, _P, _P, _P, _P, _P, _P, _I, _I, _I, _I, _I, _I, _P, _c.c_size_t, _P],
    "ce_gemm_batched_bf16": [_P, _P, _P, _P, _I, _I, _I, _I, _I, _I, _I, _I, _I] + [ctypes.c_longlong] * 6 + [_P],
    "ce_im2col_patch2d_bf16": [_P, _P, _I, _I, _I, _I, _I, _I, _P],
    "ce_gather_rows_bf16": [_P, _P, _P, _I, _I, _I, _I, _I, _P],
    "ce_rmsnorm_bf16": [_P, _P, _P, _I, _I, _I, _I, _F, _P],
    "ce_softmax_t5_bf16": [_P, _P, _I, _I, _I, _I, _I, _I, _P, _P, _P, _P],
    "ce_attention_bf16": [_P, _P, _P, _I, _I, _I, _P, _P, _I, _I, _I, _P, _I, _I, _I, _I, _I, _F, _P],
    "ce_attention_batched_bf16": [_P, _P, _P, _I, _I, _I, _P, _P, _I, _I, _I, _P, _I, _I, _I, _I, _I, _F, _I, _P],
    "ce_attention_vt_bf16": [_P, _P, _P, _I, _I, _I, _P, _I, _I, _I, _I, _I, _F, _I, _P],
    "ce_attention_2seg_vt_bf16": [_P, _P, _P, _I, _I, _I, _I, _P, _P, _I, _I, _I, _I, _P, _I, _I, _I, _I, _I, _F, _I, _P],
    "ce_attention_2seg_vt_quant_bf16": [_P, _P, _P, _I, _I, _I, _I, _P, _P, _I, _I, _I, _I, _P, _P, _I, _I, _I, _I, _I, _F, _I, _P],
    "ce_v_transpose_bf16": [_P, _I, _P, _I, _I, _I, _P],
    "ce_attention_vt_blocked_bf16": [_P, _P, _P, _I, _I, _I, _P, _I, _I, _I, _I, _I, _F, _I, _I, _I, _I, _P],
    "ce_v_transpose_blocked_bf16": [_P, _I, _P, _I, _I, _I, _I, _I, _I, _I, _P],
    "ce_timestep_sinusoid": [_P, _P, _I, _P],
    "ce_timestep_sinusoid_f32": [_P, _P, _I, _P],
    "ce_gemv": [_P, _I, _P, _P, _P, _I, _I, _I, _P],
    "ce_modulation": [_P, _P, _P, _I, _I, _I, _I, _I, _P],
    "ce_patchify_bf16": [_P, _P, _I, _I, _I, _I, _I, _P],
    "ce_unpatchify_bf16": [_P, _P, _I, _I, _I, _I, _I, _P],
    "ce_conv_igemm_bf16": [_P, _I, _P, _P, _P, _I, _P] + [_I] * 16 + [_P],
    "ce_conv3d_head_bf16": [_P, _I, _P, _P, _P, _I] + [_I] * 10 + [_P],
    "ce_gemm_bf16_tile_rows": [_I, _I, _I, _I, _c.c_longlong],
    "ce_zero_border_bf16": [_P, _I, _I, _I, _I, _I, _P],
    "ce_conv3d_gemm_bf16": [_P, _P, _I, _P, _P, _P, _I, _I, _I, _I, _I, _I, _I, _I, _P],
    "ce_conv3d_gemm_rms_silu_bf16": [_P, _P, _I, _P, _P, _P, _P, _I, _I, _I, _I, _I, _I, _I, _P, _I, _P],
    "ce_rms_silu_bf16": [_P, _P, _P, _c.c_longlong, _I, _I, _I, _I, _I, _I, _P],
    "ce_upsample2x_bf16": [_P, _P, _I, _I, _I, _I, _P],
    "ce_softmax_rows_f32_bf16": [_P, _P, _I, _I, _I, _I, _I, _F, _P],
    "ce_attention_1head_bf16": [_P, _P, _P, _P, _I, _I, _I, _I, _I, _I, _I, _F, _P, _c.c_longlong, _P],
    "ce_cfg_unipc_step": [_P, _P, _P, _P, _P, _P, _P, _P, _P, _c.c_longlong, _I, _P],
    "ce_lora_merge_bf16": [_P, _I, _P, _I, _I, _I, _I, _P, _P, _P, _P, _P],
    "ce_tea_rel_l1_bf16": [_P, _I, _I, _P, _P],
    "ce_tea_store_bf16": [_P, _P, _c.c_longlong, _P],
    "ce_tea_apply_bf16": [_P, _P, _c.c_longlong, _P],
    "ce_build_info": [],
}
DIAG_SIGNATURES: Dict[str, List] = {
    "ce_set_gemm_variant": [_I],
    "ce_set_attention_waves": [_I],
    "ce_set_gemm_fp8_variant": [_I],
    "ce_set_attention_mxfp8_variant": [_I],
    "ce_set_attention_mxfp8_persistent": [_I],
    "ce_diag_attention_exact_route_hits": [_P, _I],
}


def header_symbols(diag: bool = False) -> List[str]:
    txt = open(DIAG_HEADER if diag else HEADER).read()
    return re.findall(r"^int (ce_\w+)\(", txt, flags=re.M)


def exported_symbols(path: str) -> List[str]:
    nm = "/opt/rocm/lib/llvm/bin/llvm-nm" if os.path.exists("/opt/rocm/lib/llvm/bin/llvm-nm") else "nm"
    out = subprocess.run([nm, "-D", "--defined-only", path], check=True, capture_output=True, text=True).stdout
    return sorted(l.split()[-1] for l in out.splitlines() if l.split() and l.split()[-2] in ("T", "t", "W", "D", "B"))


HIPCC_FLAGS = ["--offload-arch=gfx950", "-O3", "-std=c++17", "-fPIC", "-fvisibility=hidden"]


def build(force: bool = False, verbose: bool = False, jobs: int = 0) -> str:
    import glob
# ... 93 lines not shown
```

chronoedit_amd/ops.py:

```python
from __future__ import annotations

import ctypes
from typing import Optional

import torch

from . import hiplib

EPI_BIAS, EPI_BIAS_GELU, EPI_GATE_RES, EPI_BIAS_GELU_ERF = 0, 1, 2, 3
EPI_F32, EPI_MUL, EPI_BIAS_ROW, EPI_BIAS_T = 4, 5, 6, 7

_lib = None
_product = None

_KNOB_DEFAULTS = {"ce_set_gemm_variant": -1, "ce_set_attention_waves": 0, "ce_set_gemm_fp8_variant": 1,
                  "ce_set_attention_mxfp8_variant": 1, "ce_set_attention_mxfp8_persistent": 512}
_knobs = dict(_KNOB_DEFAULTS)


def lib():
    global _lib, _product
    if _lib is None:
        _lib = _product = hiplib.load()
        import os
        v8 = os.environ.get("CE_GEMM_FP8_VARIANT")
        if v8 is not None:
            _set_knob("ce_set_gemm_fp8_variant", int(v8))
        v = os.environ.get("CE_GEMM_VARIANT")
        if v is not None:
            _set_knob("ce_set_gemm_variant", int(v))
    return _lib


_force_diag = False


def force_diagnostics(on: bool = True) -> None:
    global _lib, _force_diag
    lib()
    _force_diag = bool(on)
    want = hiplib.load_diagnostics() if (_force_diag or any(_knobs[k] != _KNOB_DEFAULTS[k] for k in _knobs)) else _product
    if want is not _lib:
        _lib = want


def attention_exact_route_hits(reset: bool = True):
    buf = (ctypes.c_ulonglong * 2)()
    _check(hiplib.load_diagnostics().ce_diag_attention_exact_route_hits(buf, 1 if reset else 0), "ce_diag_attention_exact_route_hits")
    return int(buf[0]), int(buf[1])


def _set_knob(symbol: str, v: int) -> int:
    global _lib
    lib()
    diag = hiplib.load_diagnostics()
    prev = getattr(diag, symbol)(int(v))
    _knobs[symbol] = getattr(diag, symbol)(int(v))
    want = diag if (_force_diag or any(_knobs[k] != _KNOB_DEFAULTS[k] for k in _knobs)) else _product
    if want is not _lib:
        _lib = want
    return prev


# ... 54 lines not shown


def _ptr(t: Optional[torch.Tensor]) -> ctypes.c_void_p:
    return ctypes.c_void_p(0 if t is None else t.data_ptr())


def _dev(t: torch.Tensor, dtype, name: str):
    if not t.is_cuda:
        raise HipKernelError(f"{name}: tensor must live on the GPU (the HIP path has no CPU fallback)")
    if t.dtype != dtype:
        raise TypeError(f"{name}: expected {dtype}, got {t.dtype}")


def _rows(t: torch.Tensor, name: str):
    if t.dim() != 2 or t.stride(1) != 1:
        raise ValueError(f"{name}: need a 2-D tensor with contiguous rows, got shape {tuple(t.shape)} stride {t.stride()}")
    return t.shape[0], t.shape[1], t.stride(0)


def ln_affine(x: torch.Tensor, a: torch.Tensor, b: torch.Tensor, eps: float, out: Optional[torch.Tensor] = None,
              ab_rows: int = 0, ab_stride: int = 0):
    _dev(x, torch.bfloat16, "x"), _dev(a, torch.float32, "a"), _dev(b, torch.float32, "b")
    M, D, ldx = _rows(x, "x")
    if out is None:
        out = torch.empty((M, D), dtype=torch.bfloat16, device=x.device)
    _, _, ldy = _rows(out, "out")
    st = _prof_begin()
    _check(lib().ce_ln_affine_bf16(_ptr(x), _ptr(out), _ptr(a), _ptr(b), M, D, ldx, ldy, float(eps), int(ab_rows), int(ab_stride),
                                   _stream()), "ce_ln_affine_bf16")
    _prof_end(st, f"ln_affine_{M}x{D}", 4.0 * M * D)
    return out


def rmsnorm_rope_(x: torch.Tensor, w: torch.Tensor, cos_sin: Optional[torch.Tensor], head_dim: int, eps: float,
                  x2: Optional[torch.Tensor] = None, w2: Optional[torch.Tensor] = None):
    _dev(x, torch.bfloat16, "x"), _dev(w, torch.float32, "w")
    M, D, ld = _rows(x, "x")
    rope_rows = 0
    if cos_sin is not None:
        _dev(cos_sin, torch.float32, "cos_sin")
        assert cos_sin.is_contiguous() and cos_sin.shape[1:] == (head_dim // 2, 2) and M % cos_sin.shape[0] == 0, (cos_sin.shape, M)
        rope_rows = cos_sin.shape[0]
    if x2 is not None:
        _dev(x2, torch.bfloat16, "x2"), _dev(w2, torch.float32, "w2")
        assert _rows(x2, "x2") == (M, D, ld)
    st = _prof_begin()
    _check(lib().ce_rmsnorm_rope_bf16(_ptr(x), _ptr(w), _ptr(x2), _ptr(w2), _ptr(cos_sin), M, D, ld, head_dim, float(eps), rope_rows,
                                      _stream()), "ce_rmsnorm_rope_bf16")
    _prof_end(st, f"rmsnorm_rope_{M}x{D}" + ("x2" if x2 is not None else ""), (8.0 if x2 is not None else 4.0) * M * D)
    return x


def gemm(a: torch.Tensor, w: torch.Tensor, bias: Optional[torch.Tensor], out: Optional[torch.Tensor] = None,
         epilogue: int = EPI_BIAS, gate: Optional[torch.Tensor] = None, res: Optional[torch.Tensor] = None, gate_rows: int = 0):
    _dev(a, torch.bfloat16, "a"), _dev(w, torch.bfloat16, "w")
    a_seg_k, a_seg_stride = 0, 0
    if a.dim() == 3:
        S, M, Ks = a.shape
        if a.stride(2) != 1 or a.stride(1) < Ks:
            raise ValueError(f"gemm: segmented a needs unit inner stride, got {a.stride()}")
        K, lda, a_seg_k, a_seg_stride = S * Ks, a.stride(1), Ks, a.stride(0)
    else:
        M, K, lda = _rows(a, "a")
    N, K2, ldw = _rows(w, "w")
    if K != K2:
        raise ValueError(f"gemm: K mismatch {K} vs {K2}")
    if bias is not None:
        _dev(bias, torch.float32, "bias")
        assert bias.numel() == (M if epilogue == EPI_BIAS_ROW else N) and bias.is_contiguous()
    oshape = (N, M) if epilogue == EPI_BIAS_T else (M, N)
    if out is None:
        out = torch.empty(oshape, dtype=torch.bfloat16, device=a.device)
    _dev(out, torch.bfloat16, "out")
    Mo, No, ldc = _rows(out, "out")
    assert (Mo, No) == oshape, ((Mo, No), oshape)
    ldres = 0
    if epilogue in (EPI_GATE_RES, EPI_MUL):
        if res is None:
            raise ValueError("EPI_GATE_RES / EPI_MUL need res")
        _dev(res, torch.bfloat16, "res")
        _, _, ldres = _rows(res, "res")
        if gate is not None:
            _dev(gate, torch.float32, "gate")
            assert gate.is_contiguous() and gate.numel() == (N if gate_rows <= 0 else (M + gate_rows - 1) // gate_rows * N)
    ws, ws_bytes = _gemm_scratch(a.device)
    st = _prof_begin()
    _check(lib().ce_gemm_bf16(_ptr(a), _ptr(w), _ptr(out), _ptr(bias), epilogue, _ptr(gate), _ptr(res), M, N, K, lda, ldw, ldc, ldres,
                              int(gate_rows), int(a_seg_k), int(a_seg_stride), 0, 0, ws, ws_bytes, _stream()), "ce_gemm_bf16")
    _prof_end(st, f"gemm_{M}x{N}x{K}_epi{epilogue}", 2.0 * M * N * K)
    return out


def rope_scatter(x: torch.Tensor, cols, weights, D: int, world: int, cos_sin: Optional[torch.Tensor], head_dim: int, eps: float,
                 out: Optional[torch.Tensor] = None):
    _dev(x, torch.bfloat16, "x")
    M, _, ldx = _rows(x, "x")
    nt = len(cols)
    assert 1 <= nt <= 3 and len(weights) == nt
    for w in weights:
        if w is not None:
            _dev(w, torch.float32, "w")
            assert w.is_contiguous() and w.numel() == D
    rope_rows = 0
    if cos_sin is not None:
        _dev(cos_sin, torch.float32, "cos_sin")
        assert cos_sin.is_contiguous() and cos_sin.shape[1:] == (head_dim // 2, 2) and M % cos_sin.shape[0] == 0
        rope_rows = cos_sin.shape[0]
    if out is None:
        out = torch.empty((world, M, nt, D // world), dtype=torch.bfloat16, device=x.device)
    _dev(out, torch.bfloat16, "out")
    assert out.is_contiguous() and out.numel() == M * nt * D
    c = list(cols) + [0] * (3 - nt)
    w = list(weights) + [None] * (3 - nt)
    st = _prof_begin()
    _check(lib().ce_rope_scatter_bf16(_ptr(x), ldx, _ptr(out), M, D, world, nt, c[0], _ptr(w[0]), c[1], _ptr(w[1]), c[2], _ptr(w[2]),
                                      _ptr(cos_sin), head_dim, float(eps), rope_rows, _stream()), "ce_rope_scatter_bf16")
    _prof_end(st, f"rope_scatter_{M}x{D}x{nt}", 4.0 * M * D * nt)
    return out


_gemm_split = True
GEMM_WS_BYTES = 256 * 384 * 256 * 4


GEMM_WS_STREAMS = 8
_gemm_default = {}
_gemm_own = {}


def _gemm_scratch(device: torch.device):
    if not _gemm_split:
        return None, 0
    dev = device.index if device.index is not None else torch.cuda.current_device()
    stream = torch.cuda.current_stream(dev).cuda_stream
    first = _gemm_default.get(dev)
    if first is not None and first[0] == stream:
        buf = first[1]
# ... 30 lines not shown
def set_attention_waves(n: int) -> int:
    return _set_knob("ce_set_attention_waves", n)


def attention(q: torch.Tensor, k: torch.Tensor, v: torch.Tensor, heads: int, out: Optional[torch.Tensor] = None,
              k2: Optional[torch.Tensor] = None, v2: Optional[torch.Tensor] = None, scale: Optional[float] = None,
              batch: int = 1):
    for n, t in (("q", q), ("k", k), ("v", v)):
        _dev(t, torch.bfloat16, n)
    Nq, Dq, ldq = _rows(q, "q")
    head_dim = Dq // heads
    L1, _, ldk = _rows(k, "k")
    L1v, _, ldv = _rows(v, "v")
    assert L1 == L1v
    if batch < 1 or Nq % batch or L1 % batch or (k2 is not None and k2.shape[0] % batch):
        raise ValueError(f"attention: row counts must be multiples of batch={batch}")
    if out is None:
        out = torch.empty((Nq, Dq), dtype=torch.bfloat16, device=q.device)
    _, _, ldo = _rows(out, "out")
    L2 = ldk2 = ldv2 = 0
    if k2 is not None:
        _dev(k2, torch.bfloat16, "k2"), _dev(v2, torch.bfloat16, "v2")
        L2, _, ldk2 = _rows(k2, "k2")
        _, _, ldv2 = _rows(v2, "v2")
    if scale is None:
        scale = head_dim ** -0.5
    st = _prof_begin()
    nq, l1, l2 = Nq // batch, L1 // batch, L2 // batch
    _check(lib().ce_attention_batched_bf16(_ptr(q), _ptr(k), _ptr(v), l1, ldk, ldv, _ptr(k2), _ptr(v2), l2, ldk2, ldv2, _ptr(out),
                                           nq, heads, head_dim, ldq, ldo, float(scale), batch, _stream()), "ce_attention_bf16")
    _prof_end(st, f"attention_{nq}x{l1}+{l2}_h{heads}" + (f"_b{batch}" if batch > 1 else ""),
              4.0 * nq * (l1 + l2) * head_dim * heads * batch)
    return out


def vt_columns(n_keys_total: int) -> int:
    return (n_keys_total + 63) // 64 * 64 + 64


def v_transpose(v: torch.Tensor, heads: int, out: Optional[torch.Tensor] = None):
    _dev(v, torch.bfloat16, "v")
    n, D, ldv = _rows(v, "v")
    assert D == heads * 128
    if out is None:
        out = torch.empty((D, vt_columns(n)), dtype=torch.bfloat16, device=v.device)
    _dev(out, torch.bfloat16, "vt")
    assert out.shape[0] == D and out.is_contiguous() and out.shape[1] >= n
    st = _prof_begin()
    _check(lib().ce_v_transpose_bf16(_ptr(v), ldv, _ptr(out), out.shape[1], n, heads, _stream()), "ce_v_transpose_bf16")
    _prof_end(st, f"v_transpose_{n}x{D}", 4.0 * n * D)
    return out


def attention_vt(q: torch.Tensor, k: torch.Tensor, vt: torch.Tensor, heads: int, out: Optional[torch.Tensor] = None,
                 scale: Optional[float] = None, batch: int = 1):
    for n, t in (("q", q), ("k", k), ("vt", vt)):
        _dev(t, torch.bfloat16, n)
    Nq, Dq, ldq = _rows(q, "q")
    L1, _, ldk = _rows(k, "k")
    assert Dq == heads * 128 and vt.shape[0] == Dq and vt.stride(1) == 1
    if batch < 1 or Nq % batch or L1 % batch:
        raise ValueError(f"attention_vt: row counts must be multiples of batch={batch}")
    if out is None:
        out = torch.empty((Nq, Dq), dtype=torch.bfloat16, device=q.device)
    _, _, ldo = _rows(out, "out")
    if scale is None:
        scale = 128 ** -0.5
    st = _prof_begin()
    nq, l1 = Nq // batch, L1 // batch
    _check(lib().ce_attention_vt_bf16(_ptr(q), _ptr(k), _ptr(vt), l1, ldk, vt.stride(0), _ptr(out), nq, heads, 128, ldq, ldo, float(scale),
                                      batch, _stream()), "ce_attention_vt_bf16")
    _prof_end(st, f"attention_{nq}x{l1}+0_h{heads}" + (f"_b{batch}" if batch > 1 else ""), 4.0 * nq * l1 * 128 * heads * batch)
    return out


def attention_2seg_vt(q: torch.Tensor, k1: torch.Tensor, v1t: torch.Tensor, len1: int, k2: torch.Tensor, v2t: torch.Tensor, len2: int,
                      heads: int, out: Optional[torch.Tensor] = None, scale: Optional[float] = None, batch: int = 1,
                      cols1: Optional[int] = None, cols2: Optional[int] = None, out8: Optional[torch.Tensor] = None,
                      scale8: Optional[torch.Tensor] = None):
    for n, t in (("q", q), ("k1", k1), ("v1t", v1t), ("k2", k2), ("v2t", v2t)):
        _dev(t, torch.bfloat16, n)
    Nq, Dq, ldq = _rows(q, "q")
    _, _, ldk1 = _rows(k1, "k1")
    _, _, ldk2 = _rows(k2, "k2")
    assert Dq == heads * 128 and v1t.shape[0] == Dq and v2t.shape[0] == Dq and v1t.stride(1) == 1 and v2t.stride(1) == 1
    assert Nq % batch == 0 and k1.shape[0] == batch * len1 and k2.shape[0] == batch * len2
    if cols1 is None:
        assert v1t.shape[1] % batch == 0
        cols1 = v1t.shape[1] // batch
    if cols2 is None:
        assert v2t.shape[1] % batch == 0
        cols2 = v2t.shape[1] // batch
    if scale is None:
        scale = 128 ** -0.5
    nq = Nq // batch
    if out8 is not None:
        _dev(out8, torch.uint8, "out8"), _dev(scale8, torch.uint8, "scale8")
        _, D8, ld8 = _rows(out8, "out8")
        assert out8.shape[0] == Nq and D8 == Dq and scale8.is_contiguous() and scale8.numel() >= mx_scale_bytes(Nq, Dq)
        st = _prof_begin()
        _check(lib().ce_attention_2seg_vt_quant_bf16(_ptr(q), _ptr(k1), _ptr(v1t), len1, ldk1, v1t.stride(0), int(cols1), _ptr(k2), _ptr(v2t),
                                                     len2, ldk2, v2t.stride(0), int(cols2), _ptr(out8), _ptr(scale8), nq, heads, 128, ldq, ld8,
                                                     float(scale), batch, _stream()), "ce_attention_2seg_vt_quant_bf16")
        _prof_end(st, f"attention_{nq}x{len1}+{len2}_h{heads}" + (f"_b{batch}" if batch > 1 else "") + "_mxq",
                  4.0 * nq * (len1 + len2) * 128 * heads * batch)
        return out8
    if out is None:
        out = torch.empty((Nq, Dq), dtype=torch.bfloat16, device=q.device)
    _, _, ldo = _rows(out, "out")
    st = _prof_begin()
    _check(lib().ce_attention_2seg_vt_bf16(_ptr(q), _ptr(k1), _ptr(v1t), len1, ldk1, v1t.stride(0), int(cols1), _ptr(k2), _ptr(v2t),
                                           len2, ldk2, v2t.stride(0), int(cols2), _ptr(out), nq, heads, 128, ldq, ldo,
                                           float(scale), batch, _stream()), "ce_attention_2seg_vt_bf16")
    _prof_end(st, f"attention_{nq}x{len1}+{len2}_h{heads}" + (f"_b{batch}" if batch > 1 else ""), 4.0 * nq * (len1 + len2) * 128 * heads * batch)
    return out


def v_transpose_blocked(v: torch.Tensor, heads: int, batch: int, blk_rows: int, n_keys: int, out: Optional[torch.Tensor] = None):
    _dev(v, torch.bfloat16, "v")
    rows, D, ldv = _rows(v, "v")
    assert D == heads * 128 and blk_rows % 64 == 0 and rows % (batch * blk_rows) == 0
    cols = (n_keys + 63) // 64 * 64 + 64
    if out is None:
        out = torch.empty((D, batch * cols), dtype=torch.bfloat16, device=v.device)
    assert out.shape == (D, batch * cols) and out.is_contiguous()
    st = _prof_begin()
    _check(lib().ce_v_transpose_blocked_bf16(_ptr(v), ldv, _ptr(out), out.shape[1], n_keys, heads, batch, blk_rows, batch * blk_rows, cols,
                                             _stream()), "ce_v_transpose_blocked_bf16")
    _prof_end(st, f"v_transpose_{batch * n_keys}x{D}", 4.0 * batch * n_keys * D)
    return out


def attention_vt_blocked(q: torch.Tensor, k: torch.Tensor, vt: torch.Tensor, heads: int, batch: int, blk_rows: int, n_keys: int,
                         out: Optional[torch.Tensor] = None, scale: Optional[float] = None):
    for n, t in (("q", q), ("k", k), ("vt", vt)):
        _dev(t, torch.bfloat16, n)
    rows, Dq, ldq = _rows(q, "q")
    rk, _, ldk = _rows(k, "k")
    assert Dq == heads * 128 and vt.shape[0] == Dq and vt.stride(1) == 1 and rows == rk and rows % (batch * blk_rows) == 0
    nq = rows // batch
    cols = vt.shape[1] // batch
    if out is None:
        out = torch.empty((rows, Dq), dtype=torch.bfloat16, device=q.device)
    _, _, ldo = _rows(out, "out")
    if scale is None:
        scale = 128 ** -0.5
    st = _prof_begin()
    _check(lib().ce_attention_vt_blocked_bf16(_ptr(q), _ptr(k), _ptr(vt), n_keys, ldk, vt.stride(0), _ptr(out), nq, heads, 128, ldq, ldo,
                                              float(scale), batch, blk_rows, batch * blk_rows, cols, _stream()), "ce_attention_vt_blocked_bf16")
    _prof_end(st, f"attention_{nq}x{n_keys}+0_h{heads}" + (f"_b{batch}" if batch > 1 else ""), 4.0 * nq * n_keys * 128 * heads * batch)
    return out


def timestep_sinusoid(t: torch.Tensor, dim: int, out: Optional[torch.Tensor] = None):
    if t.dtype == torch.float32:
        _dev(t, torch.float32, "timestep")
    else:
        _dev(t, torch.int64, "timestep")
    if out is None:
        out = torch.empty((dim,), dtype=torch.float32, device=t.device)
    if t.dtype == torch.float32:
        _check(lib().ce_timestep_sinusoid_f32(_ptr(t), _ptr(out), dim, _stream()), "ce_timestep_sinusoid_f32")
    else:
        _check(lib().ce_timestep_sinusoid(_ptr(t), _ptr(out), dim, _stream()), "ce_timestep_sinusoid")
    return out

# ... 630 lines not shown
```

chronoedit_amd/transformer.py:

```python
from __future__ import annotations

import inspect
import math
import re
from dataclasses import dataclass
from types import SimpleNamespace
from typing import Any, Dict, Optional, Tuple, Union

import torch
import torch.nn as nn

from . import ops, weights
from .weights import LoraMixin


_VT_GEMM_SWAPPED = __import__("os").environ.get("CE_VT_GEMM") == "row"


@dataclass
class Transformer2DModelOutput:
    sample: torch.Tensor


class _Config(SimpleNamespace):
    def __getitem__(self, k):
        return getattr(self, k)

    def get(self, k, d=None):
        return getattr(self, k, d)


class RMSNormParams(nn.Module):

    def __init__(self, dim: int, eps: float, device=None, dtype=None):
        super().__init__()
        self.eps = eps
        self.weight = nn.Parameter(torch.ones(dim, device=device, dtype=dtype))


class AttentionParams(nn.Module):

    def __init__(self, dim: int, heads: int, eps: float, added_kv_proj_dim: Optional[int], device=None, dtype=None):
        super().__init__()
        kw = dict(device=device, dtype=dtype)
        self.heads = heads
        self.to_q = nn.Linear(dim, dim, **kw)
        self.to_k = nn.Linear(dim, dim, **kw)
        self.to_v = nn.Linear(dim, dim, **kw)
        self.to_out = nn.ModuleList([nn.Linear(dim, dim, **kw), nn.Dropout(0.0)])
        self.norm_q = RMSNormParams(dim, eps, **kw)
        self.norm_k = RMSNormParams(dim, eps, **kw)
        self.add_k_proj = self.add_v_proj = self.norm_added_k = None
        if added_kv_proj_dim is not None:
            self.add_k_proj = nn.Linear(added_kv_proj_dim, dim, **kw)
            self.add_v_proj = nn.Linear(added_kv_proj_dim, dim, **kw)
            self.norm_added_k = RMSNormParams(dim, eps, **kw)


class _GELUProj(nn.Module):
    def __init__(self, din, dout, device=None, dtype=None):
        super().__init__()
        self.proj = nn.Linear(din, dout, device=device, dtype=dtype)


class FeedForwardParams(nn.Module):

    def __init__(self, dim, inner, dim_out=None, device=None, dtype=None):
        super().__init__()
        self.net = nn.ModuleList([
# ... 61 lines not shown
    _keys_to_ignore_on_load_unexpected = ["norm_added_q"]

    def __init__(
        self,
        patch_size: Tuple[int, int, int] = (1, 2, 2),
        num_attention_heads: int = 40,
        attention_head_dim: int = 128,
        in_channels: int = 16,
        out_channels: int = 16,
        text_dim: int = 4096,
        freq_dim: int = 256,
        ffn_dim: int = 13824,
        num_layers: int = 40,
        cross_attn_norm: bool = True,
        qk_norm: Optional[str] = "rms_norm_across_heads",
        eps: float = 1e-6,
        image_dim: Optional[int] = None,
        added_kv_proj_dim: Optional[int] = None,
        rope_max_seq_len: int = 1024,
        rope_temporal_skip_len: int = 8,
        device=None,
        dtype: torch.dtype = torch.bfloat16,
    ) -> None:
        super().__init__()
        if qk_norm != "rms_norm_across_heads":
            raise NotImplementedError("only qk_norm='rms_norm_across_heads' (the ChronoEdit/Wan setting) is supported")
        if tuple(patch_size) != (1, 2, 2):
            raise NotImplementedError("patch_size must be (1, 2, 2)")
        if attention_head_dim != 128:
            raise NotImplementedError("the gfx950 attention kernel is specialised for head_dim 128")
        self.config = _Config(
            patch_size=tuple(patch_size), num_attention_heads=num_attention_heads, attention_head_dim=attention_head_dim,
            in_channels=in_channels, out_channels=out_channels or in_channels, text_dim=text_dim, freq_dim=freq_dim,
            ffn_dim=ffn_dim, num_layers=num_layers, cross_attn_norm=cross_attn_norm, qk_norm=qk_norm, eps=eps,
            image_dim=image_dim, added_kv_proj_dim=added_kv_proj_dim, rope_max_seq_len=rope_max_seq_len,
            rope_temporal_skip_len=rope_temporal_skip_len,
        )
        inner = num_attention_heads * attention_head_dim
        kw = dict(device=device, dtype=dtype)
        self.patch_embedding = nn.Conv3d(in_channels, inner, kernel_size=patch_size, stride=patch_size, **kw)
        self.condition_embedder = ConditionEmbedderParams(inner, freq_dim, inner * 6, text_dim, image_dim, **kw)
        self.blocks = nn.ModuleList(
            [BlockParams(inner, ffn_dim, num_attention_heads, cross_attn_norm, eps, added_kv_proj_dim, **kw) for _ in range(num_layers)]
        )
        self.proj_out = nn.Linear(inner, self.config.out_channels * math.prod(patch_size), **kw)
        self.scale_shift_table = nn.Parameter(torch.randn(1, 2, inner, device=device, dtype=torch.float32) / inner**0.5)
        self._engine: Optional["DiTEngine"] = None
        self._gen = next(_GENERATION)
        self.cache_context = False
        self.gemm_dtype = "bf16"
        self.fp8_linears = self.FP8_LINEARS
        self.attn_dtype = "bf16"
        self.v_transposed = True
        self.sp_batch_cfg = True
        self.fp8_fuse_quant = True
        self.fp8_fuse_attn_quant = True
        self.cross_vt = True
        self._sp = None
        self._cfgp = None
        self._teacache = None
        self._tea_mode = None
        self.teacache_report = None

    @property
    def dtype(self) -> torch.dtype:
        return self.proj_out.weight.dtype

    @property
    def device(self) -> torch.device:
        return self.proj_out.weight.device

    @classmethod
    def from_pretrained(cls, path: str, subfolder: Optional[str] = None, torch_dtype: torch.dtype = torch.bfloat16,
                        device=None, **unused) -> "ChronoEditTransformer3DModel":
        cfg = weights.read_config(path, subfolder)
        known = set(inspect.signature(cls.__init__).parameters) - {"self", "device", "dtype"}
        model = cls(**{k: v for k, v in cfg.items() if k in known}, device=device, dtype=torch_dtype)
        sd = weights.load_state_dict_files(weights.shard_files(path, subfolder))
        weights.assign_state_dict(model, sd, ignore_unexpected=cls._keys_to_ignore_on_load_unexpected)
        model.invalidate()
        return model

    def load_wan_native_state_dict(self, sd: Dict[str, torch.Tensor]):
        renamed = weights.wan_native_to_diffusers(sd, [k for k, _ in self.named_parameters()])
        weights.assign_state_dict(self, renamed, ignore_unexpected=self._keys_to_ignore_on_load_unexpected)
        self.invalidate()
        return self

    def wan_native_state_dict(self) -> Dict[str, torch.Tensor]:
        return {weights.diffusers_to_wan_native_key(k): p.detach() for k, p in self.named_parameters()}

    def save_pretrained(self, path: str, max_shard_bytes: int = 5 << 30):
        return weights.save_pretrained(self, path, dict(vars(self.config)), max_shard_bytes, "ChronoEditTransformer3DModel")

    def load_synthetic_(self, params: Dict[str, torch.Tensor]):
        own = dict(self.named_parameters())
        missing = set(own) - set(params)
        extra = set(params) - set(own)
        if missing or extra:
            raise KeyError(f"state mismatch: missing {sorted(missing)[:4]} unexpected {sorted(extra)[:4]}")
        with torch.no_grad():
            for k, p in own.items():
                p.copy_(params[k].to(p.dtype))
        self.invalidate()
        return self

# ... 5 lines not shown
        if self._engine is not None:
            self._engine._ws = {}
            self._engine.ws_generation += 1
        return self

    def enable_cfg_parallel(self):
        from .parallel import CFGParallel, Ulysses
        self._cfgp = CFGParallel()
        self._sp = Ulysses(self._cfgp.sp_group)
        if self.config.num_attention_heads % self._sp.world:
            raise ValueError(f"{self.config.num_attention_heads} heads do not divide over {self._sp.world} ranks")
        if self._engine is not None:
            self._engine._ws = {}
            self._engine.ws_generation += 1
        return self

    def clear_context_cache(self):
        if self._engine is not None:
            self._engine.clear_context_cache()

    @torch.no_grad()
    def prime_context(self, encoder_hidden_states: torch.Tensor, encoder_hidden_states_image: Optional[torch.Tensor]):
        if self.cache_context:
            self.engine()._context(encoder_hidden_states, encoder_hidden_states_image)

    def invalidate(self):
        self._engine = None

    FP8_LINEARS = ("qkv", "o1", "q2", "o2", "f1", "f2")
    FP8_POLICIES = {"fast": ("qkv", "o1", "q2", "o2", "f1", "f2"), "accurate": ("qkv", "o1", "q2", "f1", "f2")}

    def enable_fp8_gemms(self, on: bool = True, mx: bool = True, linears=None, policy: Optional[str] = None):
        if policy is not None:
            if linears is not None:
                raise ValueError("enable_fp8_gemms: give `linears` or `policy`, not both")
            if policy not in self.FP8_POLICIES:
                raise ValueError(f"enable_fp8_gemms: unknown policy {policy!r} (one of {sorted(self.FP8_POLICIES)})")
            linears = self.FP8_POLICIES[policy]
        linears = tuple(self.FP8_LINEARS if linears is None else linears)
        bad = [n for n in linears if n not in self.FP8_LINEARS]
        if bad:
            raise ValueError(f"enable_fp8_gemms: unknown Linear name(s) {bad} (of {self.FP8_LINEARS})")
        self.fp8_linears = tuple(n for n in self.FP8_LINEARS if n in linears)
        self.gemm_dtype = ("mxfp8" if mx else "fp8") if (on and self.fp8_linears) else "bf16"
        self._engine = None
        return self

    def enable_transposed_v(self, on: bool = True):
        self.v_transposed = bool(on)
        if self._engine is not None:
            self._engine.v_transposed = self.v_transposed
            self._engine._ws = {}
            self._engine.ws_generation += 1
        return self

    def enable_cross_vt(self, on: bool = True):
        self.cross_vt = bool(on)
        self._engine = None
        return self

    def enable_fp8_attention(self, on: bool = True, cross: bool = False):
        self.attn_dtype = "mxfp8" if on else "bf16"
        self.fp8_cross = bool(on and cross)
        self._engine = None
        return self

    def enable_teacache(self, rel_l1_thresh: float, coefficients=(1.0, 0.0)):
        from .teacache import TeaCacheConfig
        coefficients = tuple(float(c) for c in coefficients)
        if not coefficients:
            raise ValueError("enable_teacache: `coefficients` is empty")
        self._teacache = TeaCacheConfig(float(rel_l1_thresh), coefficients)
        return self

    def disable_teacache(self):
        self._teacache = None
        self._tea_mode = None
        if self._engine is not None:
            self._engine.tea_release()
        return self

    @torch.no_grad()
    def teacache_ratios(self, timesteps: torch.Tensor):
        from .teacache import ratios_from_sums
        rows = self.engine().tea_tproj_rows(timesteps)
        return ratios_from_sums(ops.tea_rel_l1(rows).cpu().numpy(), rows.shape[1])

    def teacache_plan(self, timesteps: torch.Tensor, forced=()):
        from .teacache import plan_from_ratios
        if self._teacache is None:
            raise RuntimeError("teacache_plan: call enable_teacache(rel_l1_thresh) first")
        return plan_from_ratios(self.teacache_ratios(timesteps), int(timesteps.numel()), self._teacache.rel_l1_thresh,
                                self._teacache.coefficients, forced)

    def attention_path(self) -> str:
        sharded = self._sp is not None and self._sp.sharded
        return "mxfp8" if (self.attn_dtype == "mxfp8" and not sharded) else "bf16"

    def _apply(self, fn, *a, **kw):
        self._engine = None
        out = super()._apply(fn, *a, **kw)
        self._lora_moved(fn)
        return out

    def load_state_dict(self, *a, **kw):
        self._engine = None
        return super().load_state_dict(*a, **kw)

    _LORA_SLOTS = {"attn1.to_q": "qkv", "attn1.to_k": "qkv", "attn1.to_v": "qkv", "attn1.to_out.0": "o1", "attn2.to_q": "q2", "attn2.to_out.0": "o2",
                   "ffn.net.0.proj": "f1", "ffn.net.2": "f2", "attn2.to_k": "k_t", "attn2.to_v": "v_t", "attn2.add_k_proj": "k_i", "attn2.add_v_proj": "v_i"}
    _LORA_CONTEXT_SLOTS = ("k_t", "v_t", "k_i", "v_i")

    def _lora_weights_changed(self, modules):
        eng = self._engine
        if eng is None:
            return
        own = dict(self.named_modules())
        requant, context = set(), False
        for m in modules:
            mt = re.match(r"^blocks\.(\d+)\.(.+)$", m)
            slot = self._LORA_SLOTS.get(mt.group(2)) if mt else None
            if slot is None:
                return self.invalidate()
            li = int(mt.group(1))
            op = getattr(eng, f"w_{slot}_all", None) if slot in self._LORA_CONTEXT_SLOTS else getattr(eng.blk[li], "w_" + slot, None)
            if op is None or op.untyped_storage().data_ptr() != own[m].weight.untyped_storage().data_ptr():
                return self.invalidate()
            context |= slot in self._LORA_CONTEXT_SLOTS
            if slot in eng.fp8_set:
                requant.add((li, slot))
        for li, slot in sorted(requant):
            p = eng.blk[li]
            q, s = getattr(p, "q_" + slot)
            (ops.quant_rows_mxfp8(getattr(p, "w_" + slot), out=q, scale=s, w_order=True) if eng.mx else
             ops.quant_rows_fp8(getattr(p, "w_" + slot), out=q, scale=s))
        if context:
            eng.clear_context_cache()

    def engine(self) -> "DiTEngine":
        rt = getattr(self, "_lora_rt", None)
        if rt is not None and rt.dirty:
            self._lora_apply()
        if self._engine is None:
            self._engine = DiTEngine(self)
            self._gen = next(_GENERATION)
        return self._engine

    def engine_generation(self):
        eng = self._engine
        sp = self._sp
        return (self._gen, None if eng is None else eng.ws_generation, self.gemm_dtype, self.fp8_linears, self.attn_dtype, self.v_transposed, self.cross_vt,
                self.sp_batch_cfg, bool(getattr(self, "rope_plain_temporal", False)), self.cache_context,
                None if sp is None else (sp.world, sp.rank), self._cfgp is not None)

    @torch.no_grad()
    def forward(
        self,
        hidden_states: torch.Tensor,
        timestep: torch.LongTensor,
        encoder_hidden_states: torch.Tensor,
        encoder_hidden_states_image: Optional[torch.Tensor] = None,
        return_dict: bool = True,
        attention_kwargs: Optional[Dict[str, Any]] = None,
    ) -> Union[Transformer2DModelOutput, Tuple[torch.Tensor]]:
        if not hidden_states.is_cuda:
            raise ops.HipKernelError("ChronoEditTransformer3DModel (chronoedit_amd) runs only on an MI355X device: "
                                     "there is no CPU fallback (use oracle/ for CPU reference numbers)")
        B = hidden_states.shape[0]
        ts = timestep.reshape(-1)
        if ts.numel() == 1 and B > 1:
            ts = ts.expand(B)
        output = self.engine().forward(hidden_states, ts, encoder_hidden_states, encoder_hidden_states_image).to(hidden_states.dtype)
        if not return_dict:
            return (output,)
        return Transformer2DModelOutput(sample=output)


def rope_cos_sin(head_dim: int, max_len: int, skip_len: int, T: int, Hp: int, Wp: int, theta: float = 10000.0,
                 plain_temporal: bool = False) -> torch.Tensor:
    assert plain_temporal or T == 2 or T == skip_len, f"num_frames must be 2 or {skip_len}, but got {T}"
    h_dim = w_dim = 2 * (head_dim // 6)
    t_dim = head_dim - h_dim - w_dim

    def ang(dim, idx):
        f = 1.0 / (theta ** (torch.arange(0, dim, 2, dtype=torch.float64)[: dim // 2] / dim))
        return torch.outer(idx.to(torch.float64), f)

    t_idx = torch.tensor([0, skip_len - 1]) if (T == 2 and not plain_temporal) else torch.arange(T)
    assert max(T, Hp, Wp, skip_len) <= max_len
    a_t = ang(t_dim, t_idx).view(T, 1, 1, -1).expand(T, Hp, Wp, -1)
    a_h = ang(h_dim, torch.arange(Hp)).view(1, Hp, 1, -1).expand(T, Hp, Wp, -1)
    a_w = ang(w_dim, torch.arange(Wp)).view(1, 1, Wp, -1).expand(T, Hp, Wp, -1)
    a = torch.cat([a_t, a_h, a_w], dim=-1).reshape(T * Hp * Wp, head_dim // 2)
    return torch.stack([torch.cos(a), torch.sin(a)], dim=-1).to(torch.float32).contiguous()


def _pad_k(w: torch.Tensor, mult: int = 64) -> torch.Tensor:
    K = w.shape[1]
    Kp = (K + mult - 1) // mult * mult
    if Kp == K:
        return w.contiguous()
    out = torch.zeros((w.shape[0], Kp), dtype=w.dtype, device=w.device)
    out[:, :K] = w
    return out

# ... 31 lines not shown
        self.L = cfg.num_layers
        f32 = lambda t: t.detach().to(torch.float32).contiguous()
        ce = model.condition_embedder

        self.kpatch = (cfg.in_channels * 4 + 63) // 64 * 64
        self.w_patch = _pad_k(model.patch_embedding.weight.detach().reshape(self.D, -1))
        self.b_patch = f32(model.patch_embedding.bias)

        self.te_w1, self.te_b1 = ce.time_embedder.linear_1.weight.detach().contiguous(), f32(ce.time_embedder.linear_1.bias)
        self.te_w2, self.te_b2 = ce.time_embedder.linear_2.weight.detach().contiguous(), f32(ce.time_embedder.linear_2.bias)
        self.tp_w, self.tp_b = ce.time_proj.weight.detach().contiguous(), f32(ce.time_proj.bias)

        self.tx_w1, self.tx_b1 = _pad_k(ce.text_embedder.linear_1.weight.detach()), f32(ce.text_embedder.linear_1.bias)
        self.tx_w2, self.tx_b2 = ce.text_embedder.linear_2.weight.detach().contiguous(), f32(ce.text_embedder.linear_2.bias)
        self.has_image = ce.image_embedder is not None
        if self.has_image:
            ie = ce.image_embedder
            self.im_n1 = (f32(ie.norm1.weight), f32(ie.norm1.bias), ie.norm1.eps)
            self.im_w1, self.im_b1 = _pad_k(ie.ff.net[0].proj.weight.detach()), f32(ie.ff.net[0].proj.bias)
            self.im_w2, self.im_b2 = _pad_k(ie.ff.net[2].weight.detach()), f32(ie.ff.net[2].bias)
            self.im_n2 = (f32(ie.norm2.weight), f32(ie.norm2.bias), ie.norm2.eps)

        self.blk = []
        tables = []
        for blk in model.blocks:
            p = SimpleNamespace()
            a1, a2 = blk.attn1, blk.attn2
            p.w_qkv = self._fuse([a1.to_q, a1.to_k, a1.to_v])
            p.b_qkv = torch.cat([f32(a1.to_q.bias), f32(a1.to_k.bias), f32(a1.to_v.bias)])
            p.nq1, p.nk1 = f32(a1.norm_q.weight), f32(a1.norm_k.weight)
            p.w_o1, p.b_o1 = a1.to_out[0].weight.detach().contiguous(), f32(a1.to_out[0].bias)
            p.w_q2, p.b_q2 = a2.to_q.weight.detach().contiguous(), f32(a2.to_q.bias)
            p.nq2, p.nk2 = f32(a2.norm_q.weight), f32(a2.norm_k.weight)
            p.has_img = a2.add_k_proj is not None
            if p.has_img:
                p.nk_i = f32(a2.norm_added_k.weight)
            p.w_o2, p.b_o2 = a2.to_out[0].weight.detach().contiguous(), f32(a2.to_out[0].bias)
            if cfg.cross_attn_norm:
                p.n2w, p.n2b = f32(blk.norm2.weight), f32(blk.norm2.bias)
            else:
                p.n2w = p.n2b = None
            p.w_f1, p.b_f1 = blk.ffn.net[0].proj.weight.detach().contiguous(), f32(blk.ffn.net[0].proj.bias)
            p.w_f2, p.b_f2 = blk.ffn.net[2].weight.detach().contiguous(), f32(blk.ffn.net[2].bias)
            tables.append(f32(blk.scale_shift_table).reshape(6, self.D))
            self.blk.append(p)
        self.fp8_attn = model.attn_dtype == "mxfp8"
        self.fp8_cross = self.fp8_attn and bool(getattr(model, "fp8_cross", False))
        self.fp8 = model.gemm_dtype in ("fp8", "mxfp8")
        self.mx = model.gemm_dtype == "mxfp8"
        self.fp8_set = frozenset(getattr(model, "fp8_linears", model.FP8_LINEARS)) if self.fp8 else frozenset()
        self.fuse_quant = bool(getattr(model, "fp8_fuse_quant", True)) and self.F % 128 == 0
        self.fuse_attn_quant = self.fuse_quant and bool(getattr(model, "fp8_fuse_attn_quant", True))
        self.v_transposed = bool(getattr(model, "v_transposed", True))
        if self.fp8:
            if self.D % 256 or self.F % 256:
                raise NotImplementedError("fp8 GEMMs need inner and ffn dims that are multiples of 256")
            for p in self.blk:
                for name in sorted(self.fp8_set):
                    w = getattr(p, "w_" + name)
                    setattr(p, "q_" + name, ops.quant_rows_mxfp8(w, w_order=True) if self.mx else ops.quant_rows_fp8(w))
        self.w_k_t_all = self._fuse([blk.attn2.to_k for blk in model.blocks])
        self.b_k_t_all = torch.cat([f32(blk.attn2.to_k.bias) for blk in model.blocks])
        self.w_v_t_all = self._fuse([blk.attn2.to_v for blk in model.blocks])
        self.b_v_t_all = torch.cat([f32(blk.attn2.to_v.bias) for blk in model.blocks])
        self.all_img = all(p.has_img for p in self.blk)
        if self.all_img:
            self.w_k_i_all = self._fuse([blk.attn2.add_k_proj for blk in model.blocks])
            self.b_k_i_all = torch.cat([f32(blk.attn2.add_k_proj.bias) for blk in model.blocks])
            self.w_v_i_all = self._fuse([blk.attn2.add_v_proj for blk in model.blocks])
            self.b_v_i_all = torch.cat([f32(blk.attn2.add_v_proj.bias) for blk in model.blocks])
        self.cross_vt = bool(getattr(model, "cross_vt", True))
        self._ctx_bufs = {}
        self.tables = torch.stack(tables, 0).contiguous()
        self.table_out = f32(model.scale_shift_table).reshape(1, 2, self.D)
        self.w_out, self.b_out = _pad_n(model.proj_out.weight.detach().contiguous(), f32(model.proj_out.bias))
        self.ones = torch.ones(self.D, dtype=torch.float32, device=dev)
        self.zeros = torch.zeros(self.D, dtype=torch.float32, device=dev)
        self._rope = {}
        self._ws = {}
        self.ws_generation = 0
        self._ctx_key = None
        self._ctx = None
        self._ctx_refs = None
        self._tea_res = None
        self._tea_valid = False

    def _fuse(self, linears) -> torch.Tensor:
        w = torch.cat([l.weight.detach() for l in linears], dim=0).contiguous()
        o = 0
        for l in linears:
            n = l.weight.shape[0]
            l.weight.data = w[o : o + n]
            o += n
        return w

    def _ln_linear(self, ws, x: torch.Tensor, a_row, b_row, p, name: str, out: torch.Tensor, ab_rows: int = 0, ab_stride: int = 0, **kw):
        eps = self.cfg.eps
        if name not in self.fp8_set:
            ops.ln_affine(x, a_row, b_row, eps, out=ws.h, ab_rows=ab_rows, ab_stride=ab_stride)
            return ops.gemm(ws.h, getattr(p, "w_" + name), getattr(p, "b_" + name), out=out, **kw)
        aq = ws.a8[:, : x.shape[1]]
        wq, sw = getattr(p, "q_" + name)
        if self.mx:
            ops.ln_affine_mxfp8(x, a_row, b_row, eps, out=aq, scale=ws.s8, ab_rows=ab_rows, ab_stride=ab_stride)
            return ops.gemm_mxfp8(aq, ws.s8, wq, sw, getattr(p, "b_" + name), out=out, **kw)
        ops.ln_affine_fp8(x, a_row, b_row, eps, out=aq, scale=ws.s8, ab_rows=ab_rows, ab_stride=ab_stride)
# ... 13 lines not shown
            return ops.gemm_mxfp8(aq, ws.s8, wq, sw, b, out=out, **kw)
        ops.quant_rows_fp8(a, out=aq, scale=ws.s8)
        return ops.gemm_fp8(aq, ws.s8, wq, sw, b, out=out, **kw)

    def _self_attention_ulysses(self, ws, sp, x, a_row, b_row, p, cs, N: int, Nl: int, B: int = 1):
        D, H, hd, eps, W = self.D, self.H, self.cfg.attention_head_dim, self.cfg.eps, sp.world
        Dl = D // W
        if "qkv" not in self.fp8_set:
            ops.ln_affine(x, a_row, b_row, eps, out=ws.h, ab_rows=Nl, ab_stride=6 * D)
            lin = lambda lo, hi, out: ops.gemm(ws.h, p.w_qkv[lo:hi], p.b_qkv[lo:hi], out=out)
        else:
            aq = ws.a8[:, :D]
            wq, sw = p.q_qkv
            if self.mx:
                ops.ln_affine_mxfp8(x, a_row, b_row, eps, out=aq, scale=ws.s8, ab_rows=Nl, ab_stride=6 * D)
                sblk = (D // 128) * 512
                lin = lambda lo, hi, out: ops.gemm_mxfp8(aq, ws.s8, wq[lo:hi], sw[lo // 128 * sblk: hi // 128 * sblk], p.b_qkv[lo:hi], out=out)
            else:
                ops.ln_affine_fp8(x, a_row, b_row, eps, out=aq, scale=ws.s8, ab_rows=Nl, ab_stride=6 * D)
                lin = lambda lo, hi, out: ops.gemm_fp8(aq, ws.s8, wq[lo:hi], sw[lo:hi], p.b_qkv[lo:hi], out=out)
        lin(D, 3 * D, ws.qkv[:, D:])
        ops.rope_scatter(ws.qkv, (D, 2 * D), (p.nk1, None), D, W, cs, hd, eps, out=ws.send_kv)
        _, wait_kv = sp.all_to_all(ws.send_kv, ws.recv_kv, async_op=True)
        lin(0, D, ws.qkv[:, :D])
        ops.rope_scatter(ws.qkv, (0,), (p.nq1,), D, W, cs, hd, eps, out=ws.send_q)
        _, wait_q = sp.all_to_all(ws.send_q, ws.recv_q, async_op=True)
        wait_kv.wait()
        wait_q.wait()
        kv = sp.gathered_view(ws.recv_kv)
        if B > 1:
            vt_shape = (Dl, B * ops.vt_columns(N))
            ws.vt_sp = ops.v_transpose_blocked(kv[:, Dl:], H // W, B, Nl, N, out=ws.vt_sp if getattr(ws, "vt_sp", torch.empty(0)).shape == vt_shape else None)
            ops.attention_vt_blocked(sp.gathered_view(ws.recv_q), kv[:, :Dl], ws.vt_sp, H // W, B, Nl, N, out=ws.att_g)
        elif self.v_transposed:
            if getattr(ws, "vt_sp", None) is None or ws.vt_sp.shape != (Dl, ops.vt_columns(N)):
                ws.vt_sp = torch.zeros((Dl, ops.vt_columns(N)), dtype=torch.bfloat16, device=self.dev)
            ops.v_transpose(kv[:N, Dl:], H // W, out=ws.vt_sp)
            ops.attention_vt(sp.gathered_view(ws.recv_q), kv[:N, :Dl], ws.vt_sp, H // W, out=ws.att_g)
        else:
            ops.attention(sp.gathered_view(ws.recv_q), kv[:N, :Dl], kv[:N, Dl:], H // W, out=ws.att_g)
        y, _ = sp.all_to_all(ws.att_g.view(W, B * Nl, Dl), ws.att_seg)
        if "o1" in self.fp8_set:
            ws.att.copy_(sp.merge_heads_reference(y))
            return ws.att
        return y

    def _workspace(self, N: int):
        ws = self._ws.get(N)
        if ws is None:
            D, F, dev = self.D, self.F, self.dev
            e = lambda *s: torch.empty(s, dtype=torch.bfloat16, device=dev)
            ws = SimpleNamespace(x=e(N, D), h=e(N, D), qkv=e(N, 3 * D), att=e(N, D), q2=e(N, D), ffn=e(N, F),
                                 cols=e(N, self.kpatch), head=e(N, self.w_out.shape[0]))
            if self.fp8:
                ws.a8 = torch.empty((N, max(D, F)), dtype=torch.uint8, device=dev)
                ws.s8 = (torch.empty((ops.mx_scale_bytes(N, max(D, F)),), dtype=torch.uint8, device=dev) if self.mx else
                         torch.empty((N,), dtype=torch.float32, device=dev))
                if self.mx and self.fuse_quant and F % 128 == 0:
                    ws.a8b = torch.empty((N, F), dtype=torch.uint8, device=dev)
                    ws.s8b = torch.empty((ops.mx_scale_bytes(N, F),), dtype=torch.uint8, device=dev)
            if self.fp8_attn:
                u8 = lambda *s: torch.empty(s, dtype=torch.uint8, device=dev)
                ws.q8, ws.k8, ws.sq, ws.sk = u8(N, D), u8(N, D), u8(N, D // 32), u8(N, D // 32)
                ws.v8t = ws.sv = None
            sp = self.model._sp
            if sp is not None and sp.sharded:
                W, Dl = sp.world, D // sp.world
                ws.send_kv, ws.recv_kv = e(W, N, 2, Dl), e(W, N, 2, Dl)
                ws.send_q, ws.recv_q = e(W, N, 1, Dl), e(W, N, 1, Dl)
                ws.att_g, ws.att_seg = e(W * N, Dl), e(W, N, Dl)
            if len(self._ws) > 1:
                self.ws_generation += 1
            keep = list(self._ws.items())[-1:]
            self._ws = dict(keep + [(N, ws)])
        return ws

    def _rope_table(self, T, Hp, Wp):
        plain = bool(getattr(self.model, "rope_plain_temporal", False))
        key = (T, Hp, Wp, plain)
        if key not in self._rope:
            c = self.cfg
            if len(self._rope) >= 4:
                self._rope.pop(next(iter(self._rope)))
            self._rope[key] = rope_cos_sin(c.attention_head_dim, c.rope_max_seq_len, c.rope_temporal_skip_len, T, Hp, Wp,
                                           plain_temporal=plain).to(self.dev)
        return self._rope[key]

    def is_warm(self, B: int, T: int, Hh: int, Ww: int) -> bool:
        plain = bool(getattr(self.model, "rope_plain_temporal", False))
        N = T * (Hh // 2) * (Ww // 2)
        return (B * N) in self._ws and (T, Hh // 2, Ww // 2, plain) in self._rope

    def _context(self, text: torch.Tensor, image: Optional[torch.Tensor]):
        key = None
        if self.model.cache_context:
            key = (text.data_ptr(), text._version, tuple(text.shape), text.dtype,
                   None if image is None else (image.data_ptr(), image._version, tuple(image.shape), image.dtype))
            if key == self._ctx_key:
                return self._ctx
        keyed = (text, image)
        D = self.D
        B, Tt = text.shape[0], text.shape[1]
        text = text.to(torch.bfloat16).reshape(B * Tt, -1)
        if text.shape[1] != self.tx_w1.shape[1]:
            tp = torch.zeros((text.shape[0], self.tx_w1.shape[1]), dtype=torch.bfloat16, device=self.dev)
            tp[:, : text.shape[1]] = text
# ... 158 lines not shown
                if self._tea_res is None or self._tea_res.shape[0] != B * Nl or not self._tea_valid:
                    raise RuntimeError(f"TeaCache: a skipped step needs the residual of a computed step with the same {B * Nl} token rows")
                ops.tea_apply_(ws.x, self._tea_res)
            else:
                self.tea_reserve(B * Nl).copy_(ws.x)
        skip = tea == "skip"

        mods, gates1, gates2, mods_out = [], [], [], []
        for b in range(B):
            sin = ops.timestep_sinusoid(timestep[b : b + 1], cfg.freq_dim)
            h1 = ops.gemv(self.te_w1, sin, self.te_b1, flags=2)
            temb = ops.gemv(self.te_w2, h1, self.te_b2, flags=4)
            if not skip:
                tproj = ops.gemv(self.tp_w, temb, self.tp_b, flags=1 | 4)
                mods.append(ops.modulation(self.tables, tproj.view(6, D), one_mask=0b010010))
            mods_out.append(ops.modulation(self.table_out, temb.view(1, D), one_mask=0b10))
        if not skip:
            mod = torch.stack(mods, dim=1).contiguous()
        mod_out = torch.stack(mods_out, dim=0).contiguous()
        x = ws.x
        if skip:
            return self._head(ws, x, mod_out, sp, B, T, Hh, Ww, N, Nl, rows)
        if B > 1:
            gate_msa = mod[:, :, 2].contiguous()
            gate_ffn = mod[:, :, 5].contiguous()

        if text.shape[0] != B or (image is not None and image.shape[0] != B):
            raise ValueError("encoder_hidden_states / encoder_hidden_states_image batch size must match hidden_states")
        ctx = self._context(text, image)
        Tt, Ti = ctx.Tt, ctx.Ti
        grow = Nl if B > 1 else 0

        fuse_o = self.mx and self.fuse_attn_quant and D % 128 == 0
        fuse_o1, fuse_o2 = fuse_o and "o1" in self.fp8_set, fuse_o and "o2" in self.fp8_set
        for li, p in enumerate(self.blk):
            q_o1 = False
            if sp is None and self.fp8_attn:
                self._ln_linear(ws, x, mod[li, 0, 1], mod[li, 0, 0], p, "qkv", ws.qkv, ab_rows=Nl, ab_stride=6 * D)
                ops.rmsnorm_rope_mxfp8(ws.qkv[:, :D], p.nq1, cs, hd, eps, out=ws.q8, scale=ws.sq, post_scale=ops.MXFP8_Q_SCALE)
                ops.rmsnorm_rope_mxfp8(ws.qkv[:, D : 2 * D], p.nk1, cs, hd, eps, out=ws.k8, scale=ws.sk)
                if ws.v8t is None or ws.v8t.shape[0] != B:
                    ws.v8t = ws.sv = None
                ws.v8t, ws.sv = ops.v_mxfp8_transpose(ws.qkv[:, 2 * D :], Nl, B, H, out=ws.v8t, scale=ws.sv)
                if fuse_o1:
                    ops.attention_mxfp8(ws.q8, ws.sq, ws.k8, ws.sk, ws.v8t, ws.sv, H, batch=B, out8=ws.a8[:, :D], scale8=ws.s8)
                    q_o1 = True
                else:
                    ops.attention_mxfp8(ws.q8, ws.sq, ws.k8, ws.sk, ws.v8t, ws.sv, H, out=ws.att, batch=B)
                att = ws.att
            elif sp is None and self.v_transposed and "qkv" not in self.fp8_set and (B * Nl) % 8 == 0 and (B == 1 or Nl % 2 == 0):
                if getattr(ws, "vt", None) is None:
                    ws.vt = torch.zeros((D, ops.vt_columns(B * Nl)), dtype=torch.bfloat16, device=self.dev)
                ops.ln_affine(x, mod[li, 0, 1], mod[li, 0, 0], eps, out=ws.h, ab_rows=Nl, ab_stride=6 * D)
                ops.gemm(ws.h, p.w_qkv[: 2 * D], p.b_qkv[: 2 * D], out=ws.qkv[:, : 2 * D])
                if _VT_GEMM_SWAPPED:
                    ops.gemm(p.w_qkv[2 * D :], ws.h, p.b_qkv[2 * D :], out=ws.vt[:, : B * Nl], epilogue=ops.EPI_BIAS_ROW)
                else:
                    ops.gemm(ws.h, p.w_qkv[2 * D :], p.b_qkv[2 * D :], out=ws.vt[:, : B * Nl], epilogue=ops.EPI_BIAS_T)
                ops.rmsnorm_rope_(ws.qkv[:, :D], p.nq1, cs, hd, eps, x2=ws.qkv[:, D : 2 * D], w2=p.nk1)
                ops.attention_vt(ws.qkv[:, :D], ws.qkv[:, D : 2 * D], ws.vt, H, out=ws.att, batch=B)
                att = ws.att
            elif sp is None:
                self._ln_linear(ws, x, mod[li, 0, 1], mod[li, 0, 0], p, "qkv", ws.qkv, ab_rows=Nl, ab_stride=6 * D)
                ops.rmsnorm_rope_(ws.qkv[:, :D], p.nq1, cs, hd, eps, x2=ws.qkv[:, D : 2 * D], w2=p.nk1)
                ops.attention(ws.qkv[:, :D], ws.qkv[:, D : 2 * D], ws.qkv[:, 2 * D :], H, out=ws.att, batch=B)
                att = ws.att
            else:
                att = self._self_attention_ulysses(ws, sp, x, mod[li, 0, 1], mod[li, 0, 0], p, cs, N, Nl, B)
            self._linear(ws, att, p, "o1", x, quantised=q_o1, epilogue=ops.EPI_GATE_RES, gate=gate_msa[li] if B > 1 else mods[0][li, 2],
                         res=x, gate_rows=grow)
            if p.n2w is not None:
                self._ln_linear(ws, x, p.n2w, p.n2b, p, "q2", ws.q2)
            else:
                self._linear(ws, x, p, "q2", ws.q2)
            q_o2 = bool(ctx.vt and fuse_o2)
            if ctx.f8:
                seg_t, seg_i = ctx.kv[li]
                ops.rmsnorm_rope_mxfp8(ws.q2, p.nq2, None, hd, eps, out=ws.q8, scale=ws.sq, post_scale=ops.MXFP8_Q_SCALE)
                if seg_i is None and fuse_o2:
                    ops.attention_mxfp8(ws.q8, ws.sq, *seg_t, H, batch=B, out8=ws.a8[:, :D], scale8=ws.s8)
                else:
                    ops.attention_mxfp8(ws.q8, ws.sq, *seg_t, H, out=ws.att, batch=B)
                    if seg_i is not None and fuse_o2:
                        ops.attention_mxfp8(ws.q8, ws.sq, *seg_i, H, batch=B, out8=ws.a8[:, :D], scale8=ws.s8, add=ws.att)
                    elif seg_i is not None:
                        ops.attention_mxfp8(ws.q8, ws.sq, *seg_i, H, out=ws.att, batch=B, add=ws.att)
                q_o2 = fuse_o2
                self._linear(ws, ws.att, p, "o2", x, quantised=q_o2, epilogue=ops.EPI_GATE_RES, gate=None, res=x)
                k_t = None
            else:
                ops.rmsnorm_rope_(ws.q2, p.nq2, None, hd, eps)
                k_t, v_t, k_i, v_i = ctx.kv[li]
            if k_t is None:
                pass
            elif ctx.vt and fuse_o2:
                ops.attention_2seg_vt(ws.q2, k_t, v_t, Tt, k_i, v_i, Ti, H, batch=B, cols1=ctx.c1, cols2=ctx.c2, out8=ws.a8[:, :D], scale8=ws.s8)
            elif ctx.vt:
                ops.attention_2seg_vt(ws.q2, k_t, v_t, Tt, k_i, v_i, Ti, H, out=ws.att, batch=B, cols1=ctx.c1, cols2=ctx.c2)
            elif k_i is not None:
                ops.attention(ws.q2, k_t, v_t, H, out=ws.att, k2=k_i, v2=v_i, batch=B)
            else:
                ops.attention(ws.q2, k_t, v_t, H, out=ws.att, batch=B)
            if k_t is not None:
                self._linear(ws, ws.att, p, "o2", x, quantised=q_o2, epilogue=ops.EPI_GATE_RES, gate=None, res=x)
            if self.mx and self.fuse_quant and "f1" in self.fp8_set and "f2" in self.fp8_set:
                aq = ws.a8[:, :D]
                ops.ln_affine_mxfp8(x, mod[li, 0, 4], mod[li, 0, 3], eps, out=aq, scale=ws.s8, ab_rows=Nl, ab_stride=6 * D)
                ops.gemm_mxfp8_gelu_quant(aq, ws.s8, *p.q_f1, p.b_f1, out=ws.a8b, scale=ws.s8b)
                ops.gemm_mxfp8(ws.a8b, ws.s8b, *p.q_f2, p.b_f2, out=x, epilogue=ops.EPI_GATE_RES,
                               gate=gate_ffn[li] if B > 1 else mods[0][li, 5], res=x, gate_rows=grow)
            else:
                self._ln_linear(ws, x, mod[li, 0, 4], mod[li, 0, 3], p, "f1", ws.ffn, ab_rows=Nl, ab_stride=6 * D, epilogue=ops.EPI_BIAS_GELU)
                self._linear(ws, ws.ffn, p, "f2", x, epilogue=ops.EPI_GATE_RES, gate=gate_ffn[li] if B > 1 else mods[0][li, 5],
                             res=x, gate_rows=grow)

        if tea is not None:
            ops.tea_store_(x, self._tea_res)
            self._tea_valid = True
        return self._head(ws, x, mod_out, sp, B, T, Hh, Ww, N, Nl, rows)

    def _head(self, ws, x, mod_out, sp, B, T, Hh, Ww, N, Nl, rows):
        cfg, D, eps = self.cfg, self.D, self.cfg.eps
        ops.ln_affine(x, mod_out[0, 0, 1], mod_out[0, 0, 0], eps, out=ws.h, ab_rows=Nl, ab_stride=2 * D)
        ops.gemm(ws.h, self.w_out, self.b_out, out=ws.head)
        out = torch.empty((B, cfg.out_channels, T, Hh, Ww), dtype=torch.bfloat16, device=self.dev)
        if sp is None:
            for b in range(B):
                ops.unpatchify(ws.head[rows[b]], cfg.out_channels, T, Hh, Ww, out=out[b])
        else:
            full = sp.all_gather_rows(ws.head).view(sp.world, B, Nl, -1)
            for b in range(B):
                ops.unpatchify(full[:, b].reshape(sp.world * Nl, -1)[:N].contiguous(), cfg.out_channels, T, Hh, Ww, out=out[b])
        return out
```

include/chronoedit_hip.h:

```cpp
#ifndef CHRONOEDIT_HIP_H
#define CHRONOEDIT_HIP_H

#include <stddef.h>
#include <stdint.h>

#ifdef __cplusplus
extern "C" {
#endif

#ifndef __HIP_PLATFORM_AMD__
typedef struct ihipStream_t* hipStream_t;
#endif

#define CE_OK 0
#define CE_ERR_ARG (-1)
#define CE_ERR_SHAPE (-2)
#define CE_ERR_ALIGN (-3)

#define CE_EPI_BIAS 0
#define CE_EPI_BIAS_GELU 1
#define CE_EPI_GATE_RES 2
#define CE_EPI_BIAS_GELU_ERF 3
#define CE_EPI_BIAS_ROW 6
#define CE_EPI_BIAS_T 7
#define CE_EPI_F32 4

int ce_ln_affine_bf16(const void* x, void* y, const float* a, const float* b, int M, int D, int ldx, int ldy, float eps,
                      int ab_rows, int ab_stride, hipStream_t stream);

int ce_rmsnorm_rope_bf16(void* x, const float* w, void* x2, const float* w2, const float* cos_sin, int M, int D, int ld,
                         int head_dim, float eps, int rope_rows, hipStream_t stream);

int ce_gemm_bf16(const void* A, const void* W, void* C, const float* bias, int epilogue, const float* gate, const void* res,
                 int M, int N, int K, int lda, int ldw, int ldc, int ldres, int gate_rows, int a_seg_k, long long a_seg_stride,
                 int w_seg_k, long long w_seg_stride, void* ws, size_t ws_bytes, hipStream_t stream);



int ce_gemm_bf16_tile_rows(int M, int N, int K, int cus, long long ws_bytes);

int ce_attention_bf16(const void* Q, const void* K1, const void* V1, int len1, int ldk1, int ldv1, const void* K2,
                      const void* V2, int len2, int ldk2, int ldv2, void* O, int Nq, int H, int head_dim, int ldq, int ldo,
                      float softmax_scale, hipStream_t stream);

int ce_attention_batched_bf16(const void* Q, const void* K1, const void* V1, int len1, int ldk1, int ldv1, const void* K2,
                              const void* V2, int len2, int ldk2, int ldv2, void* O, int Nq, int H, int head_dim, int ldq,
                              int ldo, float softmax_scale, int batch, hipStream_t stream);

int ce_attention_vt_bf16(const void* Q, const void* K, const void* Vt, int len, int ldk, int ldvt, void* O, int Nq, int H, int head_dim,
                         int ldq, int ldo, float softmax_scale, int batch, hipStream_t stream);

int ce_attention_2seg_vt_bf16(const void* Q, const void* K1, const void* V1t, int len1, int ldk1, int ldv1t, int vt_cols1, const void* K2,
                              const void* V2t, int len2, int ldk2, int ldv2t, int vt_cols2, void* O, int Nq, int H, int head_dim, int ldq,
                              int ldo, float softmax_scale, int batch, hipStream_t stream);

int ce_attention_2seg_vt_quant_bf16(const void* Q, const void* K1, const void* V1t, int len1, int ldk1, int ldv1t, int vt_cols1, const void* K2,
                                    const void* V2t, int len2, int ldk2, int ldv2t, int vt_cols2, void* o8, void* scale8, int Nq, int H,
                                    int head_dim, int ldq, int ldo8, float softmax_scale, int batch, hipStream_t stream);

int ce_attention_vt_blocked_bf16(const void* Q, const void* K, const void* Vt, int len, int ldk, int ldvt, void* O, int Nq, int H, int head_dim,
                                 int ldq, int ldo, float softmax_scale, int batch, int blk_rows, int blk_stride, int vt_sample_cols,
                                 hipStream_t stream);

int ce_v_transpose_blocked_bf16(const void* v, int ldv, void* vt, int ldvt, int n_keys, int H, int batch, int blk_rows, int blk_stride,
                                int vt_sample_cols, hipStream_t stream);

int ce_v_transpose_bf16(const void* v, int ldv, void* vt, int ldvt, int n_keys, int H, hipStream_t stream);


int ce_timestep_sinusoid(const int64_t* t, float* out, int dim, hipStream_t stream);

int ce_timestep_sinusoid_f32(const float* t, float* out, int dim, hipStream_t stream);

int ce_gemv(const void* W, int w_is_bf16, const float* x, const float* bias, float* y, int N, int K, int flags,
            hipStream_t stream);

int ce_modulation(const float* table, const float* v, float* mod, int L, int J, int D, int v_rows, int one_mask,
                  hipStream_t stream);

int ce_patchify_bf16(const void* x, void* cols, int C, int T, int H, int W, int Kpad, hipStream_t stream);

int ce_patchify_rows_bf16(const void* x, void* cols, int C, int T, int H, int W, int Kpad, int row0, int nrows, hipStream_t stream);

int ce_rope_scatter_bf16(const void* x, int ldx, void* send, int M, int D, int W, int nt, int col0, const float* w0, int col1,
                         const float* w1, int col2, const float* w2, const float* cos_sin, int head_dim, float eps,
                         int rope_rows, hipStream_t stream);

int ce_unpatchify_bf16(const void* y, void* out, int Cout, int T, int H, int W, int ldy, hipStream_t stream);

int ce_cfg_unipc_step(const void* v_cond, const void* v_uncond, float* x, float* x_last, float* m0, float* m1,
                      float* x0_out, const float* coef, const void* reserved, long long n, int flags, hipStream_t stream);


int ce_conv_igemm_bf16(const void* const* in_frames, int n_in_frames, const void* weight, const float* bias,
                       void* const* out_frames, int n_out_frames, const void* const* res_frames, int Cin, int Cout, int KT,
                       int KH, int KW, int st, int ss, int H_out, int W_out, int in_Wp, int in_off_h, int in_off_w, int out_Wp,
                       int out_border, int out_cstride, int out_coff, hipStream_t stream);

int ce_conv3d_head_bf16(const void* const* in_frames, int n_in_frames, const void* weight, const float* bias, void* const* out_frames,
                        int n_out_frames, int Cin, int Cout, int KT, int H_out, int W_out, int in_Wp, int out_Wp, int out_border,
                        int out_cstride, int out_coff, hipStream_t stream);

int ce_conv3d_gemm_bf16(const void* in_stack, const void* weight, int ldw, const float* bias, void* out_stack, const void* res_stack,
                        int T_out, int H, int W, int Cin, int Cout, int KT, int out_cstride, int n_tile, hipStream_t stream);

int ce_conv3d_gemm_rms_silu_bf16(const void* in_stack, const void* weight, int ldw, const float* bias, void* out_stack, const void* res_stack,
                                 void* normed_stack, int T_out, int H, int W, int Cin, int Cout, int KT, int out_cstride, const float* gamma,
// ... 96 lines not shown
```

Measured before the change: 3.043.

## Fuse query RMSNorm and RoPE into attention via GEMM sum-of-squares epilogue

Adds a GEMM epilogue (EPI_BIAS_SS) that writes per-row, per-128-column-strip sums of squares alongside the Q projection output. The attention kernel then rebuilds the RMS statistic from those partial sums and applies the norm weight and RoPE to Q in registers. This replaces the separate rmsnorm_rope pass over Q for both self- and cross-attention. It is on by default. The cost is extra epilogue reductions in the GEMM, an extra float workspace, and some redundant per-head work when loading Q.

Measured after the change: 3.005. 1.3% lower.

```diff
diff --git a/chronoedit_amd/csrc/ce_attn.hip b/chronoedit_amd/csrc/ce_attn.hip
--- a/chronoedit_amd/csrc/ce_attn.hip
+++ b/chronoedit_amd/csrc/ce_attn.hip
@@ -38,6 +38,15 @@
   int ld8;
 };
 
+struct QNorm {
+  const float* sums;
+  const float* w;
+  const float* cs;
+  int ld_sums;
+  int rope_rows;
+  float eps;
+};
+
 template <bool TWO_SEG, int NWAVE>
 __global__ __launch_bounds__(NWAVE * 64, NWAVE == 8 ? 2 : 2) void attn_fwd_kernel(const bf16* __restrict__ Q, bf16* __restrict__ O, KVSeg seg0,
                                                        KVSeg seg1, int Nq, int H, int ldq, int ldo, int nqb,
@@ -279,10 +288,10 @@
 constexpr int SP_TILE_BYTES = 2 * PK_TILE + 3 * PV_TILE;
 constexpr int sp_smem_bytes(bool two_seg) { return two_seg ? SP_TILE_BYTES + 8 * QW * OST_ROW : SP_TILE_BYTES; }
 
-template <bool TWO_SEG, bool VT = false, bool QOUT = false>
+template <bool TWO_SEG, bool VT = false, bool QOUT = false, bool QNORM = false>
 __global__ __launch_bounds__(512, 2) void attn_fwd_sp_kernel(const bf16* __restrict__ Q_, bf16* __restrict__ O_, KVSeg seg0_,
                                                               KVSeg seg1_, int Nq, int H, int ldq, int ldo, int nqb,
-                                                              float scale_log2e, int batch, BlkRows blk) {
+                                                              float scale_log2e, int batch, BlkRows blk, QNorm qn) {
   extern __shared__ __attribute__((aligned(16))) unsigned char smem[];
   constexpr int NWAVE = 8, QB = QW * NWAVE;
   const int tid = threadIdx.x, lane = tid & 63;
@@ -340,12 +349,53 @@
   const int q0row = (VT && blk.rows > 0) ? (q0 / blk.rows) * blk.stride + q0 % blk.rows : q0;
 
   bf16x8 qf[8];
+  float q_ss = 0.f;
+  int q_row_abs = 0;
   {
-    const bf16* qrow = Q + (size_t)(q0 + l31 < Nq ? q0row + l31 : 0) * ldq + hoff + 8 * hh;
+    const int qr = q0 + l31 < Nq ? q0row + l31 : 0;
+    const bf16* qrow = Q + (size_t)qr * ldq + hoff + 8 * hh;
 #pragma unroll
     for (int ks = 0; ks < 8; ++ks) qf[ks] = *reinterpret_cast<const bf16x8*>(qrow + 16 * ks);
+    if constexpr (QNORM) {
+      q_row_abs = bz * Nq + qr;
+      const float* sp = qn.sums + (size_t)q_row_abs * qn.ld_sums;
+      for (int i = 0; i < H; i += 4) {
+        const f32x4 v = *reinterpret_cast<const f32x4*>(sp + i);
+        q_ss = (((q_ss + v[0]) + (i + 1 < H ? v[1] : 0.f)) + (i + 2 < H ? v[2] : 0.f)) + (i + 3 < H ? v[3] : 0.f);
+      }
+    }
   }
   auto scale_q = [&]() __attribute__((always_inline)) {
+  if constexpr (QNORM) {
+    const float rstd = 1.0f / sqrtf(q_ss / (float)(H * HD) + qn.eps);
+    const float* wp = qn.w + hoff + 8 * hh;
+    const float* cp = qn.cs ? qn.cs + ((size_t)(qn.rope_rows > 0 ? q_row_abs % qn.rope_rows : q_row_abs) * (HD / 2) + 4 * hh) * 2 : nullptr;
+#pragma unroll
+    for (int ks = 0; ks < 8; ++ks) {
+      const f32x4 w0 = *reinterpret_cast<const f32x4*>(wp + 16 * ks), w1 = *reinterpret_cast<const f32x4*>(wp + 16 * ks + 4);
+      f32x4 cs0 = {1.f, 0.f, 1.f, 0.f}, cs1 = {1.f, 0.f, 1.f, 0.f};
+      if (cp != nullptr) {
+        cs0 = *reinterpret_cast<const f32x4*>(cp + 16 * ks);
+        cs1 = *reinterpret_cast<const f32x4*>(cp + 16 * ks + 4);
+      }
+      const u32x4 x = __builtin_bit_cast(u32x4, qf[ks]);
+      u32x4 o;
+#pragma unroll
+      for (int j = 0; j < 4; ++j) {
+        const float ww0 = j < 2 ? w0[2 * j] : w1[2 * j - 4], ww1 = j < 2 ? w0[2 * j + 1] : w1[2 * j - 3];
+        float v0 = round_bf16(round_bf16(bf16lo(x[j]) * rstd) * ww0);
+        float v1 = round_bf16(round_bf16(bf16hi(x[j]) * rstd) * ww1);
+        if (cp != nullptr) {
+          const float co = j < 2 ? cs0[2 * j] : cs1[2 * j - 4], si = j < 2 ? cs0[2 * j + 1] : cs1[2 * j - 3];
+          const float r0 = v0 * co - v1 * si, r1 = v0 * si + v1 * co;
+          v0 = r0;
+          v1 = r1;
+        }
+        o[j] = pack_bf16(v0, v1);
+      }
+      qf[ks] = __builtin_bit_cast(bf16x8, o);
+    }
+  }
 #pragma unroll
   for (int ks = 0; ks < 8; ++ks) {
     const u32x4 w = __builtin_bit_cast(u32x4, qf[ks]);
@@ -1274,7 +1324,7 @@
       done = true;                                                                                                   \
     }                                                                                                                \
     hipLaunchKernelGGL((attn_fwd_sp_kernel<TWO>), dim3(nqb * H * batch), block, sp_smem_bytes(TWO), stream, (const bf16*)Q, \
-                       (bf16*)O, s0, s1, Nq, H, ldq, ldo, nqb, sl2, batch, BlkRows{0, 0, 0u, 0});                    \
+                       (bf16*)O, s0, s1, Nq, H, ldq, ldo, nqb, sl2, batch, BlkRows{0, 0, 0u, 0}, QNorm{});                    \
   } while (0)
     if (two) CE_ATTN_SP(true); else CE_ATTN_SP(false);
 #undef CE_ATTN_SP
@@ -1335,8 +1385,12 @@
 
 static int attention_vt_launch(const void* Q, const void* K, const void* Vt, int len, int ldk, int ldvt, void* O, int Nq, int H, int head_dim,
                                int ldq, int ldo, float softmax_scale, int batch, int blk_rows, int blk_stride, int vt_sample_cols,
-                               hipStream_t stream) {
+                               hipStream_t stream, const QNorm* qn = nullptr) {
   if (!Q || !K || !Vt || !O) return CE_ERR_ARG;
+  if (qn) {
+    if (!qn->sums || !qn->w || blk_rows != 0 || qn->ld_sums < H || qn->rope_rows < 0) return CE_ERR_ARG;
+    if ((qn->ld_sums & 3) || ((uintptr_t)qn->sums & 15) || ((uintptr_t)qn->w & 15) || ((uintptr_t)qn->cs & 15)) return CE_ERR_ALIGN;
+  }
   if (head_dim != HD || Nq <= 0 || H <= 0 || len <= 0 || batch <= 0 || batch > 65535) return CE_ERR_SHAPE;
   const int ntiles_cols = (len + KVB - 1) / KVB * KVB;
   if (blk_rows == 0) {
@@ -1365,6 +1419,18 @@
   }
   const int cus = ce_device_cus();
   const int items = nqb * H * batch;
+  if (qn) {
+    static bool doneq_[CE_MAX_DEVICES] = {};
+    bool& doneq = doneq_[ce_device_slot()];
+    if (!doneq) {
+      (void)hipFuncSetAttribute((const void*)attn_fwd_sp_kernel<false, true, false, true>, hipFuncAttributeMaxDynamicSharedMemorySize, sp_smem_bytes(false));
+      doneq = true;
+    }
+    const int grid_q = items <= 2 * cus ? items : ((2 * cus) & ~7);
+    hipLaunchKernelGGL((attn_fwd_sp_kernel<false, true, false, true>), dim3(grid_q), dim3(512), sp_smem_bytes(false), stream, (const bf16*)Q, (bf16*)O,
+                       s0, s1, Nq, H, ldq, ldo, nqb, sl2, batch, blk, *qn);
+    return (int)hipGetLastError();
+  }
 #ifdef CE_DIAGNOSTICS
   if (g_attn_nwave == 16 && blk_rows == 0) {
     const int rc = ce_attn16_launch(Q, K, Vt, len, ldk, ldvt, O, Nq, H, ldq, ldo, sl2, batch, cus, stream);
@@ -1385,8 +1451,15 @@
   }
   const int grid_vt = items <= 2 * cus ? items : ((2 * cus) & ~7);
   hipLaunchKernelGGL((attn_fwd_sp_kernel<false, true>), dim3(grid_vt), dim3(512), sp_smem_bytes(false), stream, (const bf16*)Q, (bf16*)O,
-                     s0, s1, Nq, H, ldq, ldo, nqb, sl2, batch, blk);
+                     s0, s1, Nq, H, ldq, ldo, nqb, sl2, batch, blk, QNorm{});
   return (int)hipGetLastError();
+}
+
+CE_API int ce_attention_vt_qnorm_bf16(const void* Q, const void* K, const void* Vt, int len, int ldk, int ldvt, void* O, int Nq, int H,
+                                      int head_dim, int ldq, int ldo, float softmax_scale, int batch, const float* q_sums, int ld_sums,
+                                      const float* q_weight, const float* cos_sin, int rope_rows, float eps, hipStream_t stream) {
+  const QNorm qn{q_sums, q_weight, cos_sin, ld_sums, rope_rows, eps};
+  return attention_vt_launch(Q, K, Vt, len, ldk, ldvt, O, Nq, H, head_dim, ldq, ldo, softmax_scale, batch, 0, 0, 0, stream, &qn);
 }
 
 CE_API int ce_attention_vt_bf16(const void* Q, const void* K, const void* Vt, int len, int ldk, int ldvt, void* O, int Nq, int H,
@@ -1406,8 +1479,12 @@
 static int attention_2seg_vt_launch(const void* Q, const void* K1, const void* V1t, int len1, int ldk1, int ldv1t, int vt_cols1,
                                     const void* K2, const void* V2t, int len2, int ldk2, int ldv2t, int vt_cols2, void* O, int Nq,
                                     int H, int head_dim, int ldq, int ldo, float softmax_scale, int batch, void* O8, void* S8, int ldo8,
-                                    hipStream_t stream) {
+                                    hipStream_t stream, const QNorm* qn = nullptr) {
   if (!Q || !K1 || !V1t || !K2 || !V2t || (!O && !O8)) return CE_ERR_ARG;
+  if (qn) {
+    if (!qn->sums || !qn->w || O8 || qn->ld_sums < H || qn->rope_rows < 0) return CE_ERR_ARG;
+    if ((qn->ld_sums & 3) || ((uintptr_t)qn->sums & 15) || ((uintptr_t)qn->w & 15) || ((uintptr_t)qn->cs & 15)) return CE_ERR_ALIGN;
+  }
   if (head_dim != HD || Nq <= 0 || H <= 0 || len1 <= 0 || len2 <= 0 || batch <= 0 || batch > 65535) return CE_ERR_SHAPE;
   const int c1 = (len1 + KVB - 1) / KVB * KVB, c2 = (len2 + KVB - 1) / KVB * KVB;
   if (vt_cols1 < len1 || vt_cols2 < len2 || ldv1t < (batch - 1) * vt_cols1 + c1 || ldv2t < (batch - 1) * vt_cols2 + c2) return CE_ERR_SHAPE;
@@ -1427,13 +1504,33 @@
   const int cus = ce_device_cus();
   const int items = nqb * H * batch;
   const int grid = items <= 2 * cus ? items : ((2 * cus) & ~7);
-  if (O8)
+  if (qn) {
+    static bool doneq_[CE_MAX_DEVICES] = {};
+    bool& doneq = doneq_[ce_device_slot()];
+    if (!doneq) {
+      (void)hipFuncSetAttribute((const void*)attn_fwd_sp_kernel<true, true, false, true>, hipFuncAttributeMaxDynamicSharedMemorySize, sp_smem_bytes(true));
+      doneq = true;
+    }
+    hipLaunchKernelGGL((attn_fwd_sp_kernel<true, true, false, true>), dim3(grid), dim3(512), sp_smem_bytes(true), stream, (const bf16*)Q, (bf16*)O,
+                       s0, s1, Nq, H, ldq, ldo, nqb, sl2, batch, blk, *qn);
+  } else if (O8)
     hipLaunchKernelGGL((attn_fwd_sp_kernel<true, true, true>), dim3(grid), dim3(512), sp_smem_bytes(true), stream, (const bf16*)Q,
-                       (bf16*)O, s0, s1, Nq, H, ldq, ldo, nqb, sl2, batch, blk);
+                       (bf16*)O, s0, s1, Nq, H, ldq, ldo, nqb, sl2, batch, blk, QNorm{});
   else
     hipLaunchKernelGGL((attn_fwd_sp_kernel<true, true>), dim3(grid), dim3(512), sp_smem_bytes(true), stream, (const bf16*)Q, (bf16*)O,
-                       s0, s1, Nq, H, ldq, ldo, nqb, sl2, batch, blk);
+                       s0, s1, Nq, H, ldq, ldo, nqb, sl2, batch, blk, QNorm{});
   return (int)hipGetLastError();
+}
+
+CE_API int ce_attention_2seg_vt_qnorm_bf16(const void* Q, const void* K1, const void* V1t, int len1, int ldk1, int ldv1t, int vt_cols1,
+                                           const void* K2, const void* V2t, int len2, int ldk2, int ldv2t, int vt_cols2, void* O, int Nq,
+                                           int H, int head_dim, int ldq, int ldo, float softmax_scale, int batch, const float* q_sums,
+                                           int ld_sums, const float* q_weight, const float* cos_sin, int rope_rows, float eps,
+                                           hipStream_t stream) {
+  if (!O) return CE_ERR_ARG;
+  const QNorm qn{q_sums, q_weight, cos_sin, ld_sums, rope_rows, eps};
+  return attention_2seg_vt_launch(Q, K1, V1t, len1, ldk1, ldv1t, vt_cols1, K2, V2t, len2, ldk2, ldv2t, vt_cols2, O, Nq, H, head_dim, ldq, ldo,
+                                  softmax_scale, batch, nullptr, nullptr, 0, stream, &qn);
 }
 
 CE_API int ce_attention_2seg_vt_bf16(const void* Q, const void* K1, const void* V1t, int len1, int ldk1, int ldv1t, int vt_cols1,
diff --git a/chronoedit_amd/csrc/ce_gemm.hip b/chronoedit_amd/csrc/ce_gemm.hip
--- a/chronoedit_amd/csrc/ce_gemm.hip
+++ b/chronoedit_amd/csrc/ce_gemm.hip
@@ -10,6 +10,8 @@
 #define EPI_BIAS_ROW 6
 #define EPI_BIAS_T 7
 #define EPI_MUL 5
+#define EPI_BIAS_SS 8
+#include "ce_gemm_epi.h"
 
 namespace {
 
@@ -155,6 +157,7 @@
       }
   }
   __syncthreads();
+  if (EPI == EPI_BIAS && gate != nullptr) epi_strip_sums<8>(smem, LDC_BYTES, m0, n0, const_cast<float*>(gate), M, N);
 #pragma unroll
   for (int t = 0; t < 8; ++t) {
     const int c = tid + 256 * t;
@@ -290,8 +293,10 @@
   if (M <= 0 || N <= 0 || K <= 0 || (K % BK) || (N & 7)) return CE_ERR_SHAPE;
   if ((lda & 7) || (ldw & 7) || (ldc & 7)) return CE_ERR_ALIGN;
   if ((epilogue == EPI_GATE_RES || epilogue == EPI_MUL) && (!res || (ldres & 7))) return CE_ERR_ARG;
-  if (epilogue < 0 || epilogue > 6 || (epilogue == EPI_BIAS_ROW && !bias)) return CE_ERR_ARG;
-  if (epilogue != EPI_F32 && epilogue != EPI_MUL) {
+  if (epilogue < 0 || (epilogue > 6 && epilogue != EPI_BIAS_SS) || (epilogue == EPI_BIAS_ROW && !bias)) return CE_ERR_ARG;
+  if (epilogue == EPI_BIAS_SS && !gate) return CE_ERR_ARG;
+  const bool ss_small = epilogue == EPI_BIAS_SS && (long long)M * ldc * 2 >= (1ll << 32);
+  if (epilogue != EPI_F32 && epilogue != EPI_MUL && !ss_small) {
     const bool big = (long long)M * N >= 256ll * 256 * 128;
     const bool want = g_gemm_variant >= 1 || (g_gemm_variant == -1 && big);
     if ((want || w_seg_k) && ce_gemm256_supported(M, N, K, lda, ldw)) {
@@ -302,7 +307,7 @@
       if (g_gemm_variant == 7 || rows_auto == 288)
         return ce_gemm288_launch(A, W, C, bias, epilogue, gate, res, M, N, K, lda, ldw, ldc, ldres, gate_rows, a_seg_k, a_seg_stride,
                                  w_seg_k, w_seg_stride, slabs, ws_bytes, stream);
-      if (g_gemm_variant == 1 || g_gemm_variant == 2)
+      if ((g_gemm_variant == 1 || g_gemm_variant == 2) && epilogue != EPI_BIAS_SS)
         return ce_gemm256_launch(A, W, C, bias, epilogue, gate, res, M, N, K, lda, ldw, ldc, ldres, gate_rows, a_seg_k, a_seg_stride,
                                  w_seg_k, w_seg_stride, slabs, ws_bytes, stream);
       return ce_gemm256w4_launch(A, W, C, bias, epilogue, gate, res, M, N, K, lda, ldw, ldc, ldres, gate_rows, a_seg_k, a_seg_stride,
@@ -310,6 +315,8 @@
     }
   }
   if (w_seg_k) return CE_ERR_SHAPE;
+  if (epilogue == EPI_BIAS) gate = nullptr;
+  if (epilogue == EPI_BIAS_SS) epilogue = EPI_BIAS;
   const int a_seg_tiles = a_seg_k > 0 ? a_seg_k / BK : 0;
   const long long a_seg_extra = a_seg_k > 0 ? a_seg_stride - a_seg_k : 0;
   const int tiles_m = (M + BM - 1) / BM, tiles_n = (N + BN - 1) / BN;
diff --git a/chronoedit_amd/csrc/ce_gemm256w4.hip b/chronoedit_amd/csrc/ce_gemm256w4.hip
--- a/chronoedit_amd/csrc/ce_gemm256w4.hip
+++ b/chronoedit_amd/csrc/ce_gemm256w4.hip
@@ -267,6 +267,11 @@
           y[q] = pack_bf16(av[2 * q][jj] + b0, av[2 * q + 1][jj] + b1);
         }
         u32x4 o = y;
+        if (EPI == EPI_BIAS && gate != nullptr) {
+          const float ss = strip_sum16(col_ok ? sumsq8_bf16(y) : 0.f);
+          const int n_strip = n0 + wn * 128;
+          if (fr == 0 && m < M && n_strip < N) const_cast<float*>(gate)[(size_t)m * ((N + 127) >> 7) + (n_strip >> 7)] = ss;
+        }
         if (EPI == EPI_BIAS_GELU) {
 #pragma unroll
           for (int q = 0; q < 4; ++q) o[q] = pack_bf16(gelu_tanh(bf16lo(y[q])), gelu_tanh(bf16hi(y[q])));
@@ -436,6 +441,7 @@
   __syncthreads();
   epi_chunks<EPI, 8>(smem, QROW, [&](int tt, int& rl, int& cc, int& mr) { const int c = tid + 256 * tt; rl = mr = c >> 4; cc = c & 15; }, m0, n0,
                      C, gate, res, M, N, ldc, ldres, gate_rows);
+  if (EPI == EPI_BIAS && gate != nullptr) epi_strip_sums<8>(smem, QROW, m0, n0, const_cast<float*>(gate), M, N);
 }
 
 }
@@ -457,9 +463,12 @@
   if (epilogue == EPI_GATE_RES && ((gate != nullptr && gate_rows > 0 && gate_rows < BM) || (long long)M * ldc * 2 >= (1ll << 32)))
     return ce_gemm256_launch(A, W, C, bias, epilogue, gate, res, M, N, K, lda, ldw, ldc, ldres, gate_rows, a_seg_k, a_seg_stride, w_seg_k,
                              w_seg_stride, ws, ws_bytes, stream);
+  if (epilogue == EPI_BIAS_SS && (!gate || seg2 || (long long)M * ldc * 2 >= (1ll << 32))) return CE_ERR_SHAPE;
   if (ng == 8 && ((long long)M * ldc * 2 >= (1ll << 32) || (epilogue == EPI_BIAS_ROW && (M & 3))))
     return ce_gemm256_launch(A, W, C, bias, epilogue, gate, res, M, N, K, lda, ldw, ldc, ldres, gate_rows, a_seg_k, a_seg_stride, w_seg_k,
                              w_seg_stride, ws, ws_bytes, stream);
+  if (epilogue == EPI_BIAS) gate = nullptr;
+  if (epilogue == EPI_BIAS_SS) epilogue = EPI_BIAS;
   const int bn = 32 * ng;
   const int tiles_m = (M + BM - 1) / BM, tiles_n = (N + bn - 1) / bn;
   const int nwg = tiles_m * tiles_n, kt = K / BK;
@@ -574,6 +583,7 @@
 extern "C" int ce_gemm256w4_reduce_launch(int epilogue, void* C, const float* bias, const float* gate, const void* res, int M, int N, int ldc,
                                           int ldres, int gate_rows, int tiles_m, int tiles_n, int t_full, int split, const float* ws, int tail,
                                           hipStream_t stream) {
+  if (epilogue == EPI_BIAS) gate = nullptr;
   static bool done_[CE_MAX_DEVICES][8] = {};
   bool* done = done_[ce_device_slot()];
 #define CE_RED(E)                                                                                                            \
diff --git a/chronoedit_amd/csrc/ce_gemm384.hip b/chronoedit_amd/csrc/ce_gemm384.hip
--- a/chronoedit_amd/csrc/ce_gemm384.hip
+++ b/chronoedit_amd/csrc/ce_gemm384.hip
@@ -334,6 +334,11 @@
         y[q] = pack_bf16(av[2 * q][jj] + b0, av[2 * q + 1][jj] + b1);
       }
       u32x4 o = y;
+      if (EPI == EPI_BIAS && gate != nullptr) {
+        const float ss = strip_sum16(col_ok ? sumsq8_bf16(y) : 0.f);
+        const int n_strip = n0 + wn * 128;
+        if (fr == 0 && m < M && n_strip < N) const_cast<float*>(gate)[(size_t)m * ((N + 127) >> 7) + (n_strip >> 7)] = ss;
+      }
       if (EPI == EPI_BIAS_GELU) {
 #pragma unroll
         for (int q = 0; q < 4; ++q) o[q] = pack_bf16(gelu_tanh(bf16lo(y[q])), gelu_tanh(bf16hi(y[q])));
@@ -392,6 +397,7 @@
   __syncthreads();
   epi_chunks<EPI, NF>(smem, QROW, [&](int tt, int& rl, int& cc, int& mr) { const int c = tid + 256 * tt; rl = mr = c >> 4; cc = c & 15; }, m0, n0,
                       C, gate, res, M, N, ldc, ldres, gate_rows);
+  if (EPI == EPI_BIAS && gate != nullptr) epi_strip_sums<NF>(smem, QROW, m0, n0, const_cast<float*>(gate), M, N);
 }
 
 }
@@ -408,11 +414,15 @@
   constexpr int BM = T384<NF>::BM, STAGE = T384<NF>::STAGE;
   if (epilogue == EPI_BIAS_T) {
     if ((M & 7) || (long long)N * ldc * 2 >= (1ll << 32) || !bias) return CE_ERR_SHAPE;
+  } else if (epilogue == EPI_BIAS_SS) {
+    if (!gate || (long long)M * ldc * 2 >= (1ll << 32)) return CE_ERR_SHAPE;
   } else
   if ((epilogue == EPI_GATE_RES && gate != nullptr && gate_rows > 0 && gate_rows < BM) || (long long)M * ldc * 2 >= (1ll << 32) ||
       (epilogue == EPI_BIAS_ROW && (M & 3)))
     return ce_gemm256_launch(A, W, C, bias, epilogue, gate, res, M, N, K, lda, ldw, ldc, ldres, gate_rows, a_seg_k, a_seg_stride, w_seg_k,
                              w_seg_stride, ws, ws_bytes, stream);
+  if (epilogue == EPI_BIAS) gate = nullptr;
+  if (epilogue == EPI_BIAS_SS) epilogue = EPI_BIAS;
   const int tiles_m = (M + BM - 1) / BM, tiles_n = (N + BN - 1) / BN;
   const int nwg = tiles_m * tiles_n, kt = K / BK;
   uint32_t a_seg_magic = 0, a_seg_extra = 0, w_seg_magic = 0, w_seg_extra = 0;
diff --git a/chronoedit_amd/csrc/ce_gemm_epi.h b/chronoedit_amd/csrc/ce_gemm_epi.h
--- a/chronoedit_amd/csrc/ce_gemm_epi.h
+++ b/chronoedit_amd/csrc/ce_gemm_epi.h
@@ -13,8 +13,38 @@
 #ifndef EPI_BIAS_T
 #define EPI_BIAS_T 7
 #endif
+#ifndef EPI_BIAS_SS
+#define EPI_BIAS_SS 8
+#endif
 
 namespace {
+
+__device__ __forceinline__ float sumsq8_bf16(const u32x4 v) {
+  float s = 0.f;
+#pragma unroll
+  for (int q = 0; q < 4; ++q) {
+    const float a = bf16lo(v[q]), b = bf16hi(v[q]);
+    s = __builtin_fmaf(a, a, s);
+    s = __builtin_fmaf(b, b, s);
+  }
+  return s;
+}
+__device__ __forceinline__ float strip_sum16(float s) {
+#pragma unroll
+  for (int o = 1; o < 16; o <<= 1) s += __shfl_xor(s, o, 64);
+  return s;
+}
+template <int NCH>
+__device__ __forceinline__ void epi_strip_sums(const unsigned char* smem, int row_bytes, int m0, int n0, float* __restrict__ sums, int M, int N) {
+  const int tid = threadIdx.x, nstrips = (N + 127) >> 7;
+#pragma unroll
+  for (int t = 0; t < NCH; ++t) {
+    const int c = tid + 256 * t, rl = c >> 4, cc = c & 15;
+    const u32x4 v = *reinterpret_cast<const u32x4*>(smem + rl * row_bytes + cc * 16);
+    const float s = strip_sum16(n0 + cc * 8 < N ? sumsq8_bf16(v) : 0.f);
+    if (cc == 0 && m0 + rl < M && n0 < N) sums[(size_t)(m0 + rl) * nstrips + (n0 >> 7)] = s;
+  }
+}
 
 template <int EPI, int NCH, bool HAS_GATE, typename RowCol>
 __device__ __forceinline__ void epi_chunks_impl(const unsigned char* smem, int row_bytes, RowCol rowcol, int m0, int n0,
diff --git a/chronoedit_amd/hiplib.py b/chronoedit_amd/hiplib.py
--- a/chronoedit_amd/hiplib.py
+++ b/chronoedit_amd/hiplib.py
@@ -57,6 +57,8 @@
     "ce_attention_batched_bf16": [_P, _P, _P, _I, _I, _I, _P, _P, _I, _I, _I, _P, _I, _I, _I, _I, _I, _F, _I, _P],
     "ce_attention_vt_bf16": [_P, _P, _P, _I, _I, _I, _P, _I, _I, _I, _I, _I, _F, _I, _P],
     "ce_attention_2seg_vt_bf16": [_P, _P, _P, _I, _I, _I, _I, _P, _P, _I, _I, _I, _I, _P, _I, _I, _I, _I, _I, _F, _I, _P],
+    "ce_attention_vt_qnorm_bf16": [_P, _P, _P, _I, _I, _I, _P, _I, _I, _I, _I, _I, _F, _I, _P, _I, _P, _P, _I, _F, _P],
+    "ce_attention_2seg_vt_qnorm_bf16": [_P, _P, _P, _I, _I, _I, _I, _P, _P, _I, _I, _I, _I, _P, _I, _I, _I, _I, _I, _F, _I, _P, _I, _P, _P, _I, _F, _P],
     "ce_attention_2seg_vt_quant_bf16": [_P, _P, _P, _I, _I, _I, _I, _P, _P, _I, _I, _I, _I, _P, _P, _I, _I, _I, _I, _I, _F, _I, _P],
     "ce_v_transpose_bf16": [_P, _I, _P, _I, _I, _I, _P],
     "ce_attention_vt_blocked_bf16": [_P, _P, _P, _I, _I, _I, _P, _I, _I, _I, _I, _I, _F, _I, _I, _I, _I, _P],
diff --git a/chronoedit_amd/ops.py b/chronoedit_amd/ops.py
--- a/chronoedit_amd/ops.py
+++ b/chronoedit_amd/ops.py
@@ -9,6 +9,7 @@
 
 EPI_BIAS, EPI_BIAS_GELU, EPI_GATE_RES, EPI_BIAS_GELU_ERF = 0, 1, 2, 3
 EPI_F32, EPI_MUL, EPI_BIAS_ROW, EPI_BIAS_T = 4, 5, 6, 7
+EPI_BIAS_SS = 8
 
 _lib = None
 _product = None
@@ -169,7 +170,8 @@
 
 
 def gemm(a: torch.Tensor, w: torch.Tensor, bias: Optional[torch.Tensor], out: Optional[torch.Tensor] = None,
-         epilogue: int = EPI_BIAS, gate: Optional[torch.Tensor] = None, res: Optional[torch.Tensor] = None, gate_rows: int = 0):
+         epilogue: int = EPI_BIAS, gate: Optional[torch.Tensor] = None, res: Optional[torch.Tensor] = None, gate_rows: int = 0,
+         sums: Optional[torch.Tensor] = None):
     _dev(a, torch.bfloat16, "a"), _dev(w, torch.bfloat16, "w")
     a_seg_k, a_seg_stride = 0, 0
     if a.dim() == 3:
@@ -200,6 +202,12 @@
         if gate is not None:
             _dev(gate, torch.float32, "gate")
             assert gate.is_contiguous() and gate.numel() == (N if gate_rows <= 0 else (M + gate_rows - 1) // gate_rows * N)
+    if (epilogue == EPI_BIAS_SS) != (sums is not None):
+        raise ValueError("gemm: sums goes with EPI_BIAS_SS, and only with it")
+    if sums is not None:
+        _dev(sums, torch.float32, "sums")
+        assert sums.is_contiguous() and sums.numel() >= M * ((N + 127) // 128) and gate is None
+        gate = sums
     ws, ws_bytes = _gemm_scratch(a.device)
     st = _prof_begin()
     _check(lib().ce_gemm_bf16(_ptr(a), _ptr(w), _ptr(out), _ptr(bias), epilogue, _ptr(gate), _ptr(res), M, N, K, lda, ldw, ldc, ldres,
@@ -336,8 +344,21 @@
     return out
 
 
+def _q_norm_args(q_norm, Nq: int, heads: int):
+    sums, w, cos_sin, eps = q_norm
+    _dev(sums, torch.float32, "q_norm sums"), _dev(w, torch.float32, "q_norm weight")
+    assert sums.dim() == 2 and sums.shape[0] == Nq and sums.shape[1] >= heads and sums.stride(1) == 1, (sums.shape, Nq, heads)
+    assert w.is_contiguous() and w.numel() == heads * 128
+    rope_rows = 0
+    if cos_sin is not None:
+        _dev(cos_sin, torch.float32, "cos_sin")
+        assert cos_sin.is_contiguous() and cos_sin.shape[1:] == (64, 2) and Nq % cos_sin.shape[0] == 0, (cos_sin.shape, Nq)
+        rope_rows = cos_sin.shape[0]
+    return sums, sums.stride(0), w, cos_sin, rope_rows, float(eps)
+
+
 def attention_vt(q: torch.Tensor, k: torch.Tensor, vt: torch.Tensor, heads: int, out: Optional[torch.Tensor] = None,
-                 scale: Optional[float] = None, batch: int = 1):
+                 scale: Optional[float] = None, batch: int = 1, q_norm=None):
     for n, t in (("q", q), ("k", k), ("vt", vt)):
         _dev(t, torch.bfloat16, n)
     Nq, Dq, ldq = _rows(q, "q")
@@ -352,8 +373,14 @@
         scale = 128 ** -0.5
     st = _prof_begin()
     nq, l1 = Nq // batch, L1 // batch
-    _check(lib().ce_attention_vt_bf16(_ptr(q), _ptr(k), _ptr(vt), l1, ldk, vt.stride(0), _ptr(out), nq, heads, 128, ldq, ldo, float(scale),
-                                      batch, _stream()), "ce_attention_vt_bf16")
+    if q_norm is not None:
+        sums, ld_sums, w, cos_sin, rope_rows, eps = _q_norm_args(q_norm, Nq, heads)
+        _check(lib().ce_attention_vt_qnorm_bf16(_ptr(q), _ptr(k), _ptr(vt), l1, ldk, vt.stride(0), _ptr(out), nq, heads, 128, ldq, ldo,
+                                                float(scale), batch, _ptr(sums), ld_sums, _ptr(w), _ptr(cos_sin), rope_rows, eps, _stream()),
+               "ce_attention_vt_qnorm_bf16")
+    else:
+        _check(lib().ce_attention_vt_bf16(_ptr(q), _ptr(k), _ptr(vt), l1, ldk, vt.stride(0), _ptr(out), nq, heads, 128, ldq, ldo, float(scale),
+                                          batch, _stream()), "ce_attention_vt_bf16")
     _prof_end(st, f"attention_{nq}x{l1}+0_h{heads}" + (f"_b{batch}" if batch > 1 else ""), 4.0 * nq * l1 * 128 * heads * batch)
     return out
 
@@ -361,7 +388,7 @@
 def attention_2seg_vt(q: torch.Tensor, k1: torch.Tensor, v1t: torch.Tensor, len1: int, k2: torch.Tensor, v2t: torch.Tensor, len2: int,
                       heads: int, out: Optional[torch.Tensor] = None, scale: Optional[float] = None, batch: int = 1,
                       cols1: Optional[int] = None, cols2: Optional[int] = None, out8: Optional[torch.Tensor] = None,
-                      scale8: Optional[torch.Tensor] = None):
+                      scale8: Optional[torch.Tensor] = None, q_norm=None):
     for n, t in (("q", q), ("k1", k1), ("v1t", v1t), ("k2", k2), ("v2t", v2t)):
         _dev(t, torch.bfloat16, n)
     Nq, Dq, ldq = _rows(q, "q")
@@ -378,6 +405,8 @@
     if scale is None:
         scale = 128 ** -0.5
     nq = Nq // batch
+    if q_norm is not None and out8 is not None:
+        raise ValueError("attention_2seg_vt: the query norm at Q load exists for the bf16 output form only")
     if out8 is not None:
         _dev(out8, torch.uint8, "out8"), _dev(scale8, torch.uint8, "scale8")
         _, D8, ld8 = _rows(out8, "out8")
@@ -393,9 +422,16 @@
         out = torch.empty((Nq, Dq), dtype=torch.bfloat16, device=q.device)
     _, _, ldo = _rows(out, "out")
     st = _prof_begin()
-    _check(lib().ce_attention_2seg_vt_bf16(_ptr(q), _ptr(k1), _ptr(v1t), len1, ldk1, v1t.stride(0), int(cols1), _ptr(k2), _ptr(v2t),
-                                           len2, ldk2, v2t.stride(0), int(cols2), _ptr(out), nq, heads, 128, ldq, ldo,
-                                           float(scale), batch, _stream()), "ce_attention_2seg_vt_bf16")
+    if q_norm is not None:
+        sums, ld_sums, w, cos_sin, rope_rows, eps = _q_norm_args(q_norm, Nq, heads)
+        _check(lib().ce_attention_2seg_vt_qnorm_bf16(_ptr(q), _ptr(k1), _ptr(v1t), len1, ldk1, v1t.stride(0), int(cols1), _ptr(k2), _ptr(v2t),
+                                                     len2, ldk2, v2t.stride(0), int(cols2), _ptr(out), nq, heads, 128, ldq, ldo,
+                                                     float(scale), batch, _ptr(sums), ld_sums, _ptr(w), _ptr(cos_sin), rope_rows, eps,
+                                                     _stream()), "ce_attention_2seg_vt_qnorm_bf16")
+    else:
+        _check(lib().ce_attention_2seg_vt_bf16(_ptr(q), _ptr(k1), _ptr(v1t), len1, ldk1, v1t.stride(0), int(cols1), _ptr(k2), _ptr(v2t),
+                                               len2, ldk2, v2t.stride(0), int(cols2), _ptr(out), nq, heads, 128, ldq, ldo,
+                                               float(scale), batch, _stream()), "ce_attention_2seg_vt_bf16")
     _prof_end(st, f"attention_{nq}x{len1}+{len2}_h{heads}" + (f"_b{batch}" if batch > 1 else ""), 4.0 * nq * (len1 + len2) * 128 * heads * batch)
     return out
 
diff --git a/chronoedit_amd/transformer.py b/chronoedit_amd/transformer.py
--- a/chronoedit_amd/transformer.py
+++ b/chronoedit_amd/transformer.py
@@ -15,6 +15,7 @@
 
 
 _VT_GEMM_SWAPPED = __import__("os").environ.get("CE_VT_GEMM") == "row"
+_QNORM_PASS = __import__("os").environ.get("CE_QNORM") == "pass"
 
 
 @dataclass
@@ -182,6 +183,7 @@
         self.fp8_linears = self.FP8_LINEARS
         self.attn_dtype = "bf16"
         self.v_transposed = True
+        self.q_norm_in_attention = not _QNORM_PASS
         self.sp_batch_cfg = True
         self.fp8_fuse_quant = True
         self.fp8_fuse_attn_quant = True
@@ -293,6 +295,12 @@
             self._engine.v_transposed = self.v_transposed
             self._engine._ws = {}
             self._engine.ws_generation += 1
+        return self
+
+    def enable_q_norm_in_attention(self, on: bool = True):
+        self.q_norm_in_attention = bool(on)
+        if self._engine is not None:
+            self._engine.q_norm_fused = self.q_norm_in_attention
         return self
 
     def enable_cross_vt(self, on: bool = True):
@@ -391,7 +399,7 @@
         eng = self._engine
         sp = self._sp
         return (self._gen, None if eng is None else eng.ws_generation, self.gemm_dtype, self.fp8_linears, self.attn_dtype, self.v_transposed, self.cross_vt,
-                self.sp_batch_cfg, bool(getattr(self, "rope_plain_temporal", False)), self.cache_context,
+                self.q_norm_in_attention, self.sp_batch_cfg, bool(getattr(self, "rope_plain_temporal", False)), self.cache_context,
                 None if sp is None else (sp.world, sp.rank), self._cfgp is not None)
 
     @torch.no_grad()
@@ -529,6 +537,7 @@
         self.fuse_quant = bool(getattr(model, "fp8_fuse_quant", True)) and self.F % 128 == 0
         self.fuse_attn_quant = self.fuse_quant and bool(getattr(model, "fp8_fuse_attn_quant", True))
         self.v_transposed = bool(getattr(model, "v_transposed", True))
+        self.q_norm_fused = bool(getattr(model, "q_norm_in_attention", True))
         if self.fp8:
             if self.D % 256 or self.F % 256:
                 raise NotImplementedError("fp8 GEMMs need inner and ffn dims that are multiples of 256")
@@ -648,6 +657,9 @@
             e = lambda *s: torch.empty(s, dtype=torch.bfloat16, device=dev)
             ws = SimpleNamespace(x=e(N, D), h=e(N, D), qkv=e(N, 3 * D), att=e(N, D), q2=e(N, D), ffn=e(N, F),
                                  cols=e(N, self.kpatch), head=e(N, self.w_out.shape[0]))
+            if D % 128 == 0:
+                ws.qsum = torch.empty((N, 2 * D // 128), dtype=torch.float32, device=dev)
+                ws.qsum2 = ws.qsum.view(-1)[: N * (D // 128)].view(N, D // 128)
             if self.fp8:
                 ws.a8 = torch.empty((N, max(D, F)), dtype=torch.uint8, device=dev)
                 ws.s8 = (torch.empty((ops.mx_scale_bytes(N, max(D, F)),), dtype=torch.uint8, device=dev) if self.mx else
@@ -912,13 +924,21 @@
                 if getattr(ws, "vt", None) is None:
                     ws.vt = torch.zeros((D, ops.vt_columns(B * Nl)), dtype=torch.bfloat16, device=self.dev)
                 ops.ln_affine(x, mod[li, 0, 1], mod[li, 0, 0], eps, out=ws.h, ab_rows=Nl, ab_stride=6 * D)
-                ops.gemm(ws.h, p.w_qkv[: 2 * D], p.b_qkv[: 2 * D], out=ws.qkv[:, : 2 * D])
+                q_fused = self.q_norm_fused and hd == 128 and D % 512 == 0
+                if q_fused:
+                    ops.gemm(ws.h, p.w_qkv[: 2 * D], p.b_qkv[: 2 * D], out=ws.qkv[:, : 2 * D], epilogue=ops.EPI_BIAS_SS, sums=ws.qsum)
+                else:
+                    ops.gemm(ws.h, p.w_qkv[: 2 * D], p.b_qkv[: 2 * D], out=ws.qkv[:, : 2 * D])
                 if _VT_GEMM_SWAPPED:
                     ops.gemm(p.w_qkv[2 * D :], ws.h, p.b_qkv[2 * D :], out=ws.vt[:, : B * Nl], epilogue=ops.EPI_BIAS_ROW)
                 else:
                     ops.gemm(ws.h, p.w_qkv[2 * D :], p.b_qkv[2 * D :], out=ws.vt[:, : B * Nl], epilogue=ops.EPI_BIAS_T)
-                ops.rmsnorm_rope_(ws.qkv[:, :D], p.nq1, cs, hd, eps, x2=ws.qkv[:, D : 2 * D], w2=p.nk1)
-                ops.attention_vt(ws.qkv[:, :D], ws.qkv[:, D : 2 * D], ws.vt, H, out=ws.att, batch=B)
+                if q_fused:
+                    ops.rmsnorm_rope_(ws.qkv[:, D : 2 * D], p.nk1, cs, hd, eps)
+                    ops.attention_vt(ws.qkv[:, :D], ws.qkv[:, D : 2 * D], ws.vt, H, out=ws.att, batch=B, q_norm=(ws.qsum, p.nq1, cs, eps))
+                else:
+                    ops.rmsnorm_rope_(ws.qkv[:, :D], p.nq1, cs, hd, eps, x2=ws.qkv[:, D : 2 * D], w2=p.nk1)
+                    ops.attention_vt(ws.qkv[:, :D], ws.qkv[:, D : 2 * D], ws.vt, H, out=ws.att, batch=B)
                 att = ws.att
             elif sp is None:
                 self._ln_linear(ws, x, mod[li, 0, 1], mod[li, 0, 0], p, "qkv", ws.qkv, ab_rows=Nl, ab_stride=6 * D)
@@ -929,10 +949,13 @@
                 att = self._self_attention_ulysses(ws, sp, x, mod[li, 0, 1], mod[li, 0, 0], p, cs, N, Nl, B)
             self._linear(ws, att, p, "o1", x, quantised=q_o1, epilogue=ops.EPI_GATE_RES, gate=gate_msa[li] if B > 1 else mods[0][li, 2],
                          res=x, gate_rows=grow)
+            q2_fused = (self.q_norm_fused and sp is None and ctx.vt and not ctx.f8 and not fuse_o2 and "q2" not in self.fp8_set and hd == 128
+                        and D % 512 == 0)
+            kw_q2 = dict(epilogue=ops.EPI_BIAS_SS, sums=ws.qsum2) if q2_fused else {}
             if p.n2w is not None:
-                self._ln_linear(ws, x, p.n2w, p.n2b, p, "q2", ws.q2)
+                self._ln_linear(ws, x, p.n2w, p.n2b, p, "q2", ws.q2, **kw_q2)
             else:
-                self._linear(ws, x, p, "q2", ws.q2)
+                self._linear(ws, x, p, "q2", ws.q2, **kw_q2)
             q_o2 = bool(ctx.vt and fuse_o2)
             if ctx.f8:
                 seg_t, seg_i = ctx.kv[li]
@@ -949,14 +972,16 @@
                 self._linear(ws, ws.att, p, "o2", x, quantised=q_o2, epilogue=ops.EPI_GATE_RES, gate=None, res=x)
                 k_t = None
             else:
-                ops.rmsnorm_rope_(ws.q2, p.nq2, None, hd, eps)
+                if not q2_fused:
+                    ops.rmsnorm_rope_(ws.q2, p.nq2, None, hd, eps)
                 k_t, v_t, k_i, v_i = ctx.kv[li]
             if k_t is None:
                 pass
             elif ctx.vt and fuse_o2:
                 ops.attention_2seg_vt(ws.q2, k_t, v_t, Tt, k_i, v_i, Ti, H, batch=B, cols1=ctx.c1, cols2=ctx.c2, out8=ws.a8[:, :D], scale8=ws.s8)
             elif ctx.vt:
-                ops.attention_2seg_vt(ws.q2, k_t, v_t, Tt, k_i, v_i, Ti, H, out=ws.att, batch=B, cols1=ctx.c1, cols2=ctx.c2)
+                ops.attention_2seg_vt(ws.q2, k_t, v_t, Tt, k_i, v_i, Ti, H, out=ws.att, batch=B, cols1=ctx.c1, cols2=ctx.c2,
+                                      q_norm=(ws.qsum2, p.nq2, None, eps) if q2_fused else None)
             elif k_i is not None:
                 ops.attention(ws.q2, k_t, v_t, H, out=ws.att, k2=k_i, v2=v_i, batch=B)
             else:
diff --git a/include/chronoedit_hip.h b/include/chronoedit_hip.h
--- a/include/chronoedit_hip.h
+++ b/include/chronoedit_hip.h
@@ -24,6 +24,7 @@
 #define CE_EPI_BIAS_ROW 6
 #define CE_EPI_BIAS_T 7
 #define CE_EPI_F32 4
+#define CE_EPI_BIAS_SS 8
 
 int ce_ln_affine_bf16(const void* x, void* y, const float* a, const float* b, int M, int D, int ldx, int ldy, float eps,
                       int ab_rows, int ab_stride, hipStream_t stream);
@@ -50,9 +51,18 @@
 int ce_attention_vt_bf16(const void* Q, const void* K, const void* Vt, int len, int ldk, int ldvt, void* O, int Nq, int H, int head_dim,
                          int ldq, int ldo, float softmax_scale, int batch, hipStream_t stream);
 
+int ce_attention_vt_qnorm_bf16(const void* Q, const void* K, const void* Vt, int len, int ldk, int ldvt, void* O, int Nq, int H, int head_dim,
+                               int ldq, int ldo, float softmax_scale, int batch, const float* q_sums, int ld_sums, const float* q_weight,
+                               const float* cos_sin, int rope_rows, float eps, hipStream_t stream);
+
 int ce_attention_2seg_vt_bf16(const void* Q, const void* K1, const void* V1t, int len1, int ldk1, int ldv1t, int vt_cols1, const void* K2,
                               const void* V2t, int len2, int ldk2, int ldv2t, int vt_cols2, void* O, int Nq, int H, int head_dim, int ldq,
                               int ldo, float softmax_scale, int batch, hipStream_t stream);
+
+int ce_attention_2seg_vt_qnorm_bf16(const void* Q, const void* K1, const void* V1t, int len1, int ldk1, int ldv1t, int vt_cols1, const void* K2,
+                                    const void* V2t, int len2, int ldk2, int ldv2t, int vt_cols2, void* O, int Nq, int H, int head_dim, int ldq,
+                                    int ldo, float softmax_scale, int batch, const float* q_sums, int ld_sums, const float* q_weight,
+                                    const float* cos_sin, int rope_rows, float eps, hipStream_t stream);
 
 int ce_attention_2seg_vt_quant_bf16(const void* Q, const void* K1, const void* V1t, int len1, int ldk1, int ldv1t, int vt_cols1, const void* K2,
                                     const void* V2t, int len2, int ldk2, int ldv2t, int vt_cols2, void* o8, void* scale8, int Nq, int H,
```
